# homenc/HElib

Measured on AMD Instinct MI355X. Metric: ctxt_x_ctxt_mults_per_sec_incl_relinearize, higher is better.
Workload: dtype u64; 1 GPU; BGV m=32768 p=65537 bits=950 (L=16x60b, K=6x56b, 6 small primes, D=3): Ctxt::multiplyBy on FRESH ciphertexts = multLowLvl (bringToSet x2 + tensorProduct) + reLinearize (dropSmallAndSpecialPrimes + key switch), benchmarks/bgv_basic.cpp:144-165; added noise MEASURED as in the reference (device canonical-embedding norms, read back lazily); the loop is driven by the C++17 host (libhelib_amd_host.so); ; batch_per_gpu=128, pairs_all_ranks=128

## Files before the change

### helib_amd/csrc/dev_common.h

```cpp
#pragma once
#include <hip/hip_runtime.h>
#include <stdint.h>

#include "ntt_core.h"

namespace hx {

constexpr int MAX_ROWS = 160;

struct PrimeDev {
  uint64_t q;
  uint64_t q2;
  uint64_t mu;
  uint64_t mu64;
  uint32_t k;
  uint32_t proth;
  uint64_t mu63;
  uint64_t tw_fwd_off;
  uint64_t tw_inv_off;
  uint64_t r2;
  uint64_t half_t1, half_t1p, half_t1m;
};

struct RowMap {
  uint16_t p[MAX_ROWS];
};
struct NttRows {
  uint16_t row[MAX_ROWS];
  uint16_t prime[MAX_ROWS];
};

struct ModDownPrep {
  uint64_t* xs;
  int64_t* S;
  uint64_t half;
  uint64_t ptxt;
  uint64_t ptxt_mu64, ptxt_mu, qd_mod_p, qdinv_mod_p;
  uint32_t ptxt_k, has_up;
  TW upS, upN;
  uint64_t qd;
  uint64_t poly_stride;
};
constexpr int MD_MAXDROP = 16;
struct PrepMulti {
  uint16_t row[MD_MAXDROP];
  uint16_t prime[MD_MAXDROP];
  TW up[2 * MD_MAXDROP];
};
struct ModDownRow {
  TW qdm;
  TW inv;
  TW cf;
  uint64_t cf_r2;
  uint32_t out_row;
  uint32_t mode;
};
struct ModDownApply {
  const uint64_t* xs;
  const int64_t* S;
  const ModDownRow* rows;
  const uint64_t* delta;
  uint64_t delta_poly_stride;
};
#if defined(__HIPCC__)
typedef unsigned long long hx_v2u64 __attribute__((ext_vector_type(2)));
__device__ __forceinline__ ulonglong2 ld_stream2(const uint64_t* p)
{
#ifdef HX_NO_NT
  return *reinterpret_cast<const ulonglong2*>(p);
#else
  const hx_v2u64 v = __builtin_nontemporal_load(reinterpret_cast<const hx_v2u64*>(p));
  return make_ulonglong2(v.x, v.y);
#endif
}
__device__ __forceinline__ uint64_t ld_stream1(const uint64_t* p)
{
#if defined(HX_NO_NT) || defined(HX_RNS_NO_NT)
  return *p;
#else
  return __builtin_nontemporal_load(p);
#endif
}
__device__ __forceinline__ void st_stream1(uint64_t* p, uint64_t v)
{
#if defined(HX_NO_NT) || defined(HX_RNS_NO_NT)
  *p = v;
#else
  __builtin_nontemporal_store(v, p);
#endif
}
__device__ __forceinline__ void st_stream2(uint64_t* p, ulonglong2 v)
{
#ifdef HX_NO_NT
  *reinterpret_cast<ulonglong2*>(p) = v;
#else
  hx_v2u64 w;
  w.x = v.x;
  w.y = v.y;
  __builtin_nontemporal_store(w, reinterpret_cast<hx_v2u64*>(p));
#endif
}
#endif

struct TensorSrc {
  const uint64_t* a0;
  const uint64_t* a1;
  const uint64_t* b0;
  const uint64_t* b1;
};
constexpr int MD_MAXPOLY = 8;
struct PolyBases {
  uint64_t* d[MD_MAXPOLY];
  int n;
};
__host__ __device__ inline uint64_t* poly_base(const PolyBases& p, unsigned i)
{
  uint64_t* r = p.d[0];
  r = i == 1 ? p.d[1] : r;
  r = i == 2 ? p.d[2] : r;
  r = i == 3 ? p.d[3] : r;
  r = i == 4 ? p.d[4] : r;
  r = i == 5 ? p.d[5] : r;
  r = i == 6 ? p.d[6] : r;
  r = i == 7 ? p.d[7] : r;
  return r;
}
struct RowMap2 {
  uint16_t p[MAX_ROWS];
  uint16_t brow[MAX_ROWS];
};
struct RowScalars {
  uint64_t c[MAX_ROWS];
  uint64_t cp[MAX_ROWS];
};

constexpr int KS_MAXD = 8;
struct KsFix {
  int64_t owner;
  TW pinv[KS_MAXD];
  TW pscale;
};
struct KsLastPlan {
  uint16_t fd[MAX_ROWS];
};
struct KsLastArgs {
  const uint64_t* dig_in;
  const uint64_t* dig_ev;
  const uint64_t* kb;
  const uint64_t* ka;
  uint64_t* out0;
  uint64_t* out1;
  const uint64_t* own_src;
  const uint64_t* acc0;
  const uint64_t* acc1;
  const KsFix* fix;
  int nall, wrows, batch, scale_parts;
};

typedef unsigned __int128 u128;

#define HX_RO __attribute__((address_space(4)))
typedef const HX_RO uint64_t* ro_u64;
typedef const HX_RO uint32_t* ro_u32;
typedef const HX_RO double* ro_f64;
typedef const HX_RO TW* ro_tw;
template <class T>
__host__ __device__ inline const HX_RO T* as_ro(const T* p)
{
  return (const HX_RO T*)(uintptr_t)p;
}
__device__ __forceinline__ TW ld_tw(ro_tw p, size_t i)
{
  ro_u64 w = (ro_u64)p;
  TW t;
  t.w = w[2 * i];
  t.wp = w[2 * i + 1];
  return t;
}

__device__ __forceinline__ uint64_t add_mod(uint64_t a, uint64_t b, uint64_t q)
{
  uint64_t s = a + b;
  return s >= q ? s - q : s;
}
__device__ __forceinline__ uint64_t sub_mod(uint64_t a, uint64_t b, uint64_t q)
{
  return a >= b ? a - b : a + q - b;
}
__device__ __forceinline__ uint64_t neg_mod(uint64_t a, uint64_t q) { return a ? q - a : 0; }

__device__ __forceinline__ uint64_t mul_mod(uint64_t a, uint64_t b, uint64_t q, uint64_t mu,
                                            uint32_t k)
{
  u128 x = (u128)a * b;
// ... 32 lines not shown
```

### helib_amd/csrc/engine.hip

```cpp
#include <hip/hip_runtime.h>

#include <cstdarg>
#include <cstdio>
#include <cstdlib>
#include <cstring>
#include <algorithm>
#include <chrono>
#include <map>
#include <mutex>
#include <string>
#include <unordered_set>
#include <vector>

#include "../../include/helib_amd.h"
#include "arena.h"
#include "prof.h"
#include "switches.h"
#include "dev_common.h"
#include "hostmath.h"
#include "bluestein.h"
#include "pfa_dev.h"
#include "rns_kernels.h"
#include "mfma_ext.h"
#include "rns_mfma_dev.h"
// ... 29 lines not shown
hipError_t launch_moddown_apply_plain_tensor_pow2(int logn, const TensorSrc& T, const PolyBases& outs, const NttRows& keep,
                                                  int nkeep, int batch, const ModDownApply& A, const PrimeDev* primes,
                                                  const TW* tw_arena, hipStream_t st);
hipError_t launch_moddown_tensor_pow2(int logn, const TensorSrc& T, const PolyBases& outs, int drop_row, int drop_prime,
                                      const NttRows& keep, int nkeep, int batch, const ModDownPrep& P,
                                      const ModDownApply& A, const PrimeDev* primes, const TW* tw_arena, hipStream_t st);
hipError_t launch_ntt_inv_mul_pow2(int logn, const uint64_t* a, const uint64_t* b, uint64_t* out, const NttRows& rows,
                                   int nrows, int batch, const PrimeDev* primes, const TW* tw_arena, hipStream_t st);
hipError_t launch_conv_rows(int logn, const ConvRowArgs& A, const ConvRows& R, int nunits, const PrimeDev* cprimes,
                            const TW* tw_arena, hipStream_t st);
}

using hx::ExtArgs;
using hx::ExtPlanDev;
using hx::MAX_ROWS;
static constexpr int MAX_EXT_SRC = hx::EXT_MAXSRC;
using hx::ModDownApply;
using hx::ModDownPrep;
using hx::NttRows;
using hx::PolyBases;
using hx::PrimeDev;
using hx::RowMap;
using hx::RowMap2;
using hx::RowScalars;
using hx::TW;

static thread_local std::string g_err;
static int fail(int code, const char* fmt, ...)
{
  char buf[512];
  va_list ap;
  va_start(ap, fmt);
  vsnprintf(buf, sizeof buf, fmt, ap);
  va_end(ap);
  g_err = buf;
  return code;
}
#define HIPCHK(expr)                                                                     \
  do {                                                                                   \
    hipError_t _e = (expr);                                                              \
    if (_e != hipSuccess) {                                                              \
      (void)hipGetLastError();  \
      return fail(HX_ERR_DEVICE, "%s failed: %s (%s:%d)", #expr, hipGetErrorString(_e),  \
                  __FILE__, __LINE__);                                                   \
    }                                                                                    \
  } while (0)
#define CHK(expr)          \
  do {                     \
    int _rc = (expr);      \
    if (_rc != HX_OK)      \
      return _rc;          \
  } while (0)

extern "C" const char* hx_last_error(void) { return g_err.c_str(); }
extern "C" const char* hx_version(void) { return "helib_amd 0.1 (gfx950)"; }
extern "C" int hx_device_count(int* count)
{
  if (!count)
    return fail(HX_ERR_INVALID, "null argument");
  int n = 0;
  hipError_t e = hipGetDeviceCount(&n);
  if (e != hipSuccess) {
    *count = 0;
    return fail(HX_ERR_DEVICE, "hipGetDeviceCount: %s", hipGetErrorString(e));
  }
  *count = n;
  return HX_OK;
}

struct PrimeHost {
  uint64_t q, root, rinv;
  uint64_t last_s = 0, last_n = 0;
  uint64_t tw_fwd_off = 0, tw_inv_off = 0;
  bool proth = false;
  int half_pd = -1;
};
static inline uint64_t tw_companion(const PrimeHost& ph, uint64_t w)
{
  return ph.proth ? hx::tw_mont_form(w, ph.q) : hxh::shoup(w, ph.q);
}
static inline uint64_t tw_r2(const PrimeHost& ph, uint64_t w)
{
  return ph.proth ? hx::tw_mont_form(hx::tw_mont_form(w, ph.q), ph.q) : 0;
}

struct ExtPlan {
  ExtPlanDev dev;
  void* blob = nullptr;
  void* blob_mfma = nullptr;
};

struct ConvPlan {
  int logn = 0;
  int split = 0;
  int pd[16] = {0, 0, 0, 0, 0, 0, 0, 0, 0, 0, 0, 0, 0, 0, 0, 0};
  hx::ConvPrimeDev* dev = nullptr;
};
struct BluePrime {
  bool aux = false;
  ConvPlan aconv[3][3];
  uint64_t* d_ahat[3][4] = {{nullptr, nullptr, nullptr, nullptr}, {nullptr, nullptr, nullptr, nullptr},
                            {nullptr, nullptr, nullptr, nullptr}};
  hx::Crt3Dev crt;
  hx::BluePrimeDev* dev = nullptr;
  TW* d_powers = nullptr;
  TW* d_ipowers = nullptr;
  uint64_t* d_hat[5] = {nullptr, nullptr, nullptr, nullptr, nullptr};
  TW* d_hatw[5] = {nullptr, nullptr, nullptr, nullptr, nullptr};
  ConvPlan conv[4];
  uint64_t* d_pfa = nullptr;
};

struct hx_ctx {
  hxs::Switches sw;
  int device = 0;
  hipStream_t stream = nullptr;
  uint64_t m = 0;
  uint32_t phim = 0;
  int logn = 0;
  bool pow2 = false;
  std::vector<uint32_t> zms;
  uint32_t* d_zms = nullptr;
  int32_t* d_zms_index = nullptr;
  uint32_t* d_perm = nullptr;
  std::vector<PrimeHost> primes;
  PrimeDev* d_primes = nullptr;
  int primes_cap = 0;
  TW* d_tw = nullptr;
  size_t tw_cap = 0, tw_used = 0;
  uint64_t* scratch[11] = {nullptr, nullptr, nullptr, nullptr, nullptr, nullptr, nullptr, nullptr, nullptr, nullptr, nullptr};
  uint32_t* d_redo = nullptr;
  size_t redo_cap = 0;
  size_t scratch_words[11] = {0, 0, 0, 0, 0, 0, 0, 0, 0, 0, 0};
  uint64_t aux_q[3] = {0, 0, 0};
  int bk = 0, n1 = 0, n2 = 0, n3 = 0;
  uint32_t dq = 0, mpad = 0;
  PrimeDev* d_cprimes = nullptr;
  int ncprimes = 0, cprimes_cap = 0;
  std::vector<struct BluePrime*> blue;
  uint16_t* d_pfa_idx = nullptr;
  std::vector<ConvPlan> bigplan;
  std::vector<int64_t> psi_low, phi_coef;
  std::map<std::vector<uint64_t>, ExtPlan*> plans;
  hxa::SlabArena arena;
  std::unordered_set<struct hx_poly*> polys;
  int refs = 1;
  std::recursive_mutex mu;
  double* d_frac = nullptr;
  size_t frac_cap = 0, frac_pos = 0;
  bool want_frac = false;
  int xs_first = 0, xs_rows = 0;
  double xs_inv_qd = 0;
  bool want_fdelta = false;
  double2* d_wtab = nullptr;
  double2 *d_bn_v = nullptr, *d_bn_w = nullptr, *d_bn_chat = nullptr, *d_bn_Z = nullptr;
  size_t bn_rows_cap = 0;
  unsigned long long* d_norm2 = nullptr;
  size_t norm_cap = 0;
  double2* d_norm_park = nullptr;
  size_t norm_park_cap = 0;
  struct NormPending {
    hipEvent_t ev;
    unsigned long long* pinned;
    size_t cap;
    int rows;
    double* out;
    bool slab;
  };
  std::vector<void*> norm_slabs;
  bool defer_norms = false;
  std::vector<NormPending> norm_pending, norm_free;
  hipStream_t norm_stream = nullptr;
  hipEvent_t norm_in_ev = nullptr, norm_out_ev = nullptr;
  bool norm_reads_xs = false, norm_reads_frac = false;
  hipEvent_t timer[2] = {nullptr, nullptr};
  bool capturing = false;
  int graphs_alive = 0;
  hipStream_t own_stream = nullptr;
  std::vector<void*> graph_retired;
  void* ckks = nullptr;
  void (*ckks_free)(void*) = nullptr;
  void* linalg = nullptr;
  void (*linalg_free)(void*) = nullptr;
};

struct hx_poly {
  hx_ctx* ctx;
  int batch;
  int cap_rows;
  std::vector<int> prime_idx;
  uint64_t* d;
  bool owns;
  struct Share {
    int refs;
  };
  Share* share = nullptr;
  bool exposed = false;
  size_t row_words() const { return (size_t)batch * ctx->phim; }
  int nrows() const { return (int)prime_idx.size(); }
  bool shared() const { return share && share->refs > 1; }
};

struct hx_ksk {
  hx_ctx* ctx;
  int ndig;
  std::vector<int> row_idx;
  uint64_t* d_b;
  uint64_t* d_a;
};

static int use(hx_ctx* c)
{
  HIPCHK(hipSetDevice(c->device));
  return HX_OK;
}
#define CTX_ENTER(ctx)                                             \
  std::lock_guard<std::recursive_mutex> _ctx_lock((ctx)->mu);      \
  CHK(use(ctx))

#define NO_CAPTURE(ctx, what)                                                                      \
  do {                                                                                             \
    if ((ctx)->capturing)                                                                          \
      return fail(HX_ERR_INVALID, what " waits for the device and cannot be captured in a graph"); \
  } while (0)

static constexpr size_t POOL_LIMIT = (size_t)64 << 30;
template <bool TRACE>
static int arena_sys_alloc_t(size_t bytes, void** out)
{
  const bool trace = TRACE;
  const auto t0 = std::chrono::steady_clock::now();
  hipError_t e = hipMalloc(out, bytes);
  if (trace)
    fprintf(stderr, "[helib_amd arena] hipMalloc(%zu MiB) took %.2f ms\n", bytes >> 20,
            std::chrono::duration<double, std::milli>(std::chrono::steady_clock::now() - t0).count());
  if (e != hipSuccess)
    (void)hipGetLastError();
  return (int)e;
}
static void arena_sys_free(void* p) { hipFree(p); }
static hipError_t pool_alloc(hx_ctx* c, size_t bytes, void** out)
{
  if (!c->arena.sys_alloc) {
    c->arena.sys_alloc = c->sw.arena_trace ? arena_sys_alloc_t<true> : arena_sys_alloc_t<false>;
    c->arena.sys_free = arena_sys_free;
  }
  int rc = c->arena.alloc(bytes, c->capturing, out);
  if (rc != 0 && !c->capturing) {
    (void)hipGetLastError();
    hipStreamSynchronize(c->stream);
    if (c->arena.trim(0) > 0)
      rc = c->arena.alloc(bytes, false, out);
  }
  return (hipError_t)rc;
}
static void retire_or_free(hx_ctx* c, void* p, bool device_wide_sync = false)
{
  if (!p)
    return;
  if (c->norm_stream)
    hipStreamSynchronize(c->norm_stream);
  if (c->capturing || c->graphs_alive > 0) {
    c->graph_retired.push_back(p);
    return;
  }
  if (device_wide_sync)
    hipDeviceSynchronize();
  else
    hipStreamSynchronize(c->stream);
  hipFree(p);
}
static void pool_free(hx_ctx* c, void* p, size_t bytes)
{
  (void)bytes;
  if ((c->capturing || c->graphs_alive > 0) && c->arena.is_pinned(p)) {
    c->arena.defer(p);
    return;
  }
  c->arena.release(p);
  if (c->arena.cached() > POOL_LIMIT && !c->capturing) {
    hipStreamSynchronize(c->stream);
    c->arena.trim(POOL_LIMIT / 2);
  }
}

static int norm_join(hx_ctx* c, bool xs, bool frac)
{
  if ((xs && c->norm_reads_xs) || (frac && c->norm_reads_frac)) {
    HIPCHK(hipStreamWaitEvent(c->stream, c->norm_out_ev, 0));
    c->norm_reads_xs = c->norm_reads_frac = false;
  }
  return HX_OK;
}

static int ensure_scratch(hx_ctx* c, int slot, size_t words)
{
  if (slot <= 1)
    CHK(norm_join(c, true, false));
  if (c->scratch_words[slot] >= words)
    return HX_OK;
  if (c->scratch[slot]) {
    retire_or_free(c, c->scratch[slot]);
    c->scratch[slot] = nullptr;
    c->scratch_words[slot] = 0;
  }
  HIPCHK(hipMalloc((void**)&c->scratch[slot], words * 8));
  c->scratch_words[slot] = words;
  return HX_OK;
}

static int dcopy(hx_ctx* c, uint64_t* dst, const uint64_t* src, size_t words)
{
  if (words == 0 || dst == src)
    return HX_OK;
  if (((uintptr_t)dst | (uintptr_t)src) & 15) {
    HIPCHK(hipMemcpyAsync(dst, src, words * 8, hipMemcpyDeviceToDevice, c->stream));
    return HX_OK;
  }
  const size_t blocks = std::min<size_t>((words / 2 + 255) / 256, (size_t)256 * 16);
  HX_LAUNCH(hx::copy_words_kernel, dim3((unsigned)std::max<size_t>(blocks, 1)), dim3(256), 0, c->stream,
                     dst, src, words);
  HIPCHK(hipGetLastError());
  return HX_OK;
}
// ... 10 lines not shown
    }
    p->share = nullptr;
  } else {
    pool_free(p->ctx, p->d, bytes);
  }
  p->d = nullptr;
}
static int poly_own(hx_poly* p)
{
  if (!p->share)
    return HX_OK;
  if (p->share->refs == 1) {
    delete p->share;
    p->share = nullptr;
    return HX_OK;
  }
  hx_ctx* c = p->ctx;
  uint64_t* nd = nullptr;
  const size_t bytes = (size_t)p->cap_rows * p->row_words() * 8;
  hipError_t e = pool_alloc(c, bytes, (void**)&nd);
  if (e != hipSuccess)
    return fail(HX_ERR_NOMEM, "hipMalloc(%zu) failed: %s", bytes, hipGetErrorString(e));
  CHK(dcopy(c, nd, p->d, (size_t)p->nrows() * p->row_words()));
  p->share->refs--;
  p->share = nullptr;
  p->d = nd;
  return HX_OK;
}
#define OWN(p) CHK(poly_own(p))
static int poly_fresh(hx_poly* p, const uint64_t** old_rows)
{
  *old_rows = p->d;
  if (!p->share)
    return HX_OK;
  if (p->share->refs == 1) {
    delete p->share;
    p->share = nullptr;
    return HX_OK;
  }
  uint64_t* nd = nullptr;
  const size_t bytes = (size_t)p->cap_rows * p->row_words() * 8;
  hipError_t e = pool_alloc(p->ctx, bytes, (void**)&nd);
  if (e != hipSuccess)
    return fail(HX_ERR_NOMEM, "hipMalloc(%zu) failed: %s", bytes, hipGetErrorString(e));
  p->share->refs--;
  p->share = nullptr;
  p->d = nd;
  return HX_OK;
}

static void ctx_free(hx_ctx* c);
extern "C" int hx_ctx_create(hx_ctx** out, int device, uint64_t m)
{
  if (!out || m < 2 || m > (1ull << 24))
    return fail(HX_ERR_INVALID, "Bad Z_m^* modulus m (must be in [2, 2^24])");
  int ndev = 0;
  if (hipGetDeviceCount(&ndev) != hipSuccess || ndev <= 0)
    return fail(HX_ERR_DEVICE, "no HIP device available (this library has no CPU path)");
  if (device < 0 || device >= ndev)
    return fail(HX_ERR_INVALID, "device %d out of range [0,%d)", device, ndev);
  HIPCHK(hipSetDevice(device));
  hx_ctx* c = new hx_ctx();
  c->sw = hxs::read();
  struct Guard {
    hx_ctx* c;
    ~Guard()
    {
      if (c)
        ctx_free(c);
    }
  } guard{c};
  c->device = device;
  c->m = m;
  std::vector<int32_t> zidx((size_t)m, -1);
  for (uint64_t i = 1; i < m; i++)
    if (hxh::gcd(i, m) == 1) {
      zidx[i] = (int32_t)c->zms.size();
      c->zms.push_back((uint32_t)i);
    }
  c->phim = (uint32_t)c->zms.size();
  c->pow2 = (m & (m - 1)) == 0;
  if (c->pow2) {
    int l = 0;
    while ((1u << l) < c->phim)
      l++;
    c->logn = l;
  }
  HIPCHK(hipMalloc((void**)&c->d_zms, (size_t)c->phim * 4));
  HIPCHK(hipMalloc((void**)&c->d_zms_index, (size_t)m * 4));
  HIPCHK(hipMalloc((void**)&c->d_perm, (size_t)c->phim * 4));
  HIPCHK(hipMemcpy(c->d_zms, c->zms.data(), (size_t)c->phim * 4, hipMemcpyHostToDevice));
  HIPCHK(hipMemcpy(c->d_zms_index, zidx.data(), (size_t)m * 4, hipMemcpyHostToDevice));
  c->primes_cap = 1024;
  HIPCHK(hipMalloc((void**)&c->d_primes, sizeof(PrimeDev) * c->primes_cap));
  guard.c = nullptr;
  *out = c;
  return HX_OK;
}

static void ctx_release(hx_ctx* c)
{
  bool last;
  {
    std::lock_guard<std::recursive_mutex> lk(c->mu);
    last = --c->refs == 0;
  }
  if (last)
    ctx_free(c);
}
extern "C" int hx_ctx_destroy(hx_ctx* c)
{
  if (!c)
    return HX_OK;
  ctx_release(c);
  return HX_OK;
}
static void ctx_free(hx_ctx* c)
{
  hipSetDevice(c->device);
  hipDeviceSynchronize();
  if (c->ckks_free)
    c->ckks_free(c->ckks);
  if (c->linalg_free)
    c->linalg_free(c->linalg);
  if (c->d_tw)
    hipFree(c->d_tw);
  for (auto& kv : c->plans) {
    hipFree(kv.second->blob);
    hipFree(kv.second->blob_mfma);
    delete kv.second;
  }
  for (int i = 0; i < 11; i++)
    if (c->scratch[i])
      hipFree(c->scratch[i]);
  c->arena.destroy();
  if (c->norm_stream) {
    hipStreamDestroy(c->norm_stream);
    hipEventDestroy(c->norm_in_ev);
    hipEventDestroy(c->norm_out_ev);
  }
  if (c->own_stream)
    hipStreamDestroy(c->own_stream);
  for (void* q : c->graph_retired)
    hipFree(q);
  hipFree(c->d_redo);
  hipFree(c->d_frac);
  hipFree(c->d_wtab);
  hipFree(c->d_bn_v);
  hipFree(c->d_bn_w);
  hipFree(c->d_bn_chat);
  hipFree(c->d_bn_Z);
  hipFree(c->d_norm2);
  hipFree(c->d_norm_park);
  for (auto* v : {&c->norm_pending, &c->norm_free})
    for (auto& np : *v) {
      hipEventDestroy(np.ev);
      if (!np.slab)
        hipHostFree(np.pinned);
    }
  for (void* q : c->norm_slabs)
    hipHostFree(q);
  for (BluePrime* b : c->blue) {
    if (!b)
      continue;
    hipFree(b->dev);
    hipFree(b->d_powers);
    hipFree(b->d_ipowers);
    hipFree(b->d_pfa);
    for (int i = 0; i < 5; i++) {
      hipFree(b->d_hat[i]);
      hipFree(b->d_hatw[i]);
    }
    for (int i = 0; i < 4; i++)
      hipFree(b->conv[i].dev);
    for (int j = 0; j < 3; j++) {
      for (int i = 0; i < 4; i++)
        hipFree(b->d_ahat[j][i]);
      for (int i = 0; i < 3; i++)
        hipFree(b->aconv[j][i].dev);
    }
    delete b;
  }
  if (c->d_cprimes)
    hipFree(c->d_cprimes);
  for (hipEvent_t e : c->timer)
    if (e)
      hipEventDestroy(e);
  hipFree(c->d_pfa_idx);
  hipFree(c->d_zms);
  hipFree(c->d_zms_index);
  hipFree(c->d_perm);
  hipFree(c->d_primes);
  delete c;
}

extern "C" int hx_ctx_phim(const hx_ctx* c, uint64_t* phim)
{
  if (!c || !phim)
    return fail(HX_ERR_INVALID, "null argument");
  *phim = c->phim;
  return HX_OK;
}
extern "C" int hx_ctx_set_stream(hx_ctx* c, void* s)
{
  if (!c)
    return fail(HX_ERR_INVALID, "null context");
  std::lock_guard<std::recursive_mutex> lk(c->mu);
  if (c->capturing)
    return fail(HX_ERR_INVALID, "hx_ctx_set_stream while a graph is being captured");
  if (c->stream != (hipStream_t)s) {
    hipSetDevice(c->device);
    hipStreamSynchronize(c->stream);
    if (c->norm_stream)
      hipStreamSynchronize(c->norm_stream);
  }
  c->stream = (hipStream_t)s;
  return HX_OK;
}
extern "C" int hx_ctx_sync(hx_ctx* c)
{
  if (!c)
    return fail(HX_ERR_INVALID, "null context");
  CTX_ENTER(c);
  NO_CAPTURE(c, "hx_ctx_sync");
  HIPCHK(hipStreamSynchronize(c->stream));
  if (c->norm_stream)
    HIPCHK(hipStreamSynchronize(c->norm_stream));
  return HX_OK;
}
extern "C" int hx_ctx_reserve(hx_ctx* c, uint64_t bytes)
{
  if (!c)
    return fail(HX_ERR_INVALID, "null context");
  CTX_ENTER(c);
  if (!c->arena.sys_alloc) {
    c->arena.sys_alloc = c->sw.arena_trace ? arena_sys_alloc_t<true> : arena_sys_alloc_t<false>;
    c->arena.sys_free = arena_sys_free;
  }
  const int rc = c->arena.reserve((size_t)bytes);
  if (rc != 0)
    return fail(HX_ERR_NOMEM, "hipMalloc(%llu) failed: %s", (unsigned long long)bytes, hipGetErrorString((hipError_t)rc));
  return HX_OK;
}
extern "C" int hx_ctx_arena_stats(hx_ctx* c, uint64_t out[4])
{
  if (!c || !out)
    return fail(HX_ERR_INVALID, "null argument");
  std::lock_guard<std::recursive_mutex> lk(c->mu);
  out[0] = c->arena.reserved;
  out[1] = c->arena.in_use;
  out[2] = c->arena.sys_calls;
  out[3] = c->arena.deferred.size();
  return HX_OK;
}
extern "C" int hx_ctx_num_primes(const hx_ctx* c, int* n)
{
  if (!c || !n)
    return fail(HX_ERR_INVALID, "null argument");
  *n = (int)c->primes.size();
  return HX_OK;
}
extern "C" int hx_ctx_prime(const hx_ctx* c, int idx, uint64_t* q, uint64_t* root)
{
  if (!c)
    return fail(HX_ERR_INVALID, "prime index out of range");
  std::lock_guard<std::recursive_mutex> lk(const_cast<hx_ctx*>(c)->mu);
  if (idx < 0 || idx >= (int)c->primes.size())
    return fail(HX_ERR_INVALID, "prime index out of range");
  if (q)
    *q = c->primes[idx].q;
  if (root)
    *root = c->primes[idx].root;
  return HX_OK;
}

static int tw_reserve(hx_ctx* c, size_t extra)
{
  if (c->tw_used + extra <= c->tw_cap)
    return HX_OK;
  size_t ncap = c->tw_cap ? c->tw_cap * 2 : extra * 32;
  while (ncap < c->tw_used + extra)
    ncap *= 2;
  TW* nd = nullptr;
  HIPCHK(hipMalloc((void**)&nd, ncap * sizeof(TW)));
  if (c->d_tw) {
    HIPCHK(hipDeviceSynchronize());
    HIPCHK(hipMemcpy(nd, c->d_tw, c->tw_used * sizeof(TW), hipMemcpyDeviceToDevice));
    retire_or_free(c, c->d_tw, true);
  }
  c->d_tw = nd;
  c->tw_cap = ncap;
  return HX_OK;
}

template <int LOGN>
static int upload_tw(hx_ctx* c, PrimeHost& ph)
{
  using G = hx::Geo<LOGN>;
  std::vector<TW> f(G::TW_TOTAL), i(G::TW_TOTAL);
  uint64_t ninv = hxh::invmod((uint64_t)G::N % ph.q, ph.q);
  hx::build_tw_tables<LOGN>(ph.q, ph.root, ph.rinv, ninv, hxh::mulmod, f.data(), i.data());
  CHK(tw_reserve(c, 2 * (size_t)G::TW_TOTAL));
  ph.tw_fwd_off = c->tw_used;
  ph.tw_inv_off = c->tw_used + G::TW_TOTAL;
  ph.proth = hx::is_proth32(ph.q) && !c->sw.no_proth;
  if (ph.proth) {
// ... 1890 lines not shown
    pl->dev.mfma_a = nullptr;
    pl->dev.mfma_steps = 0;
    const bool oks = mfma_small && pl->dev.hps_ok;
    if ((okw || oks) && !c->sw.no_mfma_ext) {
      std::vector<uint8_t> tab;
      std::vector<uint64_t> tqs((size_t)nt);
      for (int t = 0; t < nt; t++)
        tqs[(size_t)t] = tq(t);
      hx::mfx::build_tables(n, nt, tqs.data(), mfma_w.data(), mfma_negp.data(), &h[o_upd], tab);
      uint8_t* dm = nullptr;
      HIPCHK(hipMalloc((void**)&dm, tab.size()));
      HIPCHK(hipMemcpy(dm, tab.data(), tab.size(), hipMemcpyHostToDevice));
      pl->blob_mfma = dm;
      pl->dev.mfma_a = dm;
      pl->dev.mfma_steps = (uint32_t)hx::mfx::steps_for(n);
    }
  }
  pl->dev.tgt_chunk7 = hx::as_ro(reinterpret_cast<const uint32_t*>(d + o_tchunk));
  {
    bool unit = scaled && ptxt > 1;
    for (int t = 0; t < nt && unit; t++)
      unit = ptxt <= tq(t);
    pl->dev.corr_unit = unit ? 1u : 0u;
  }
  c->plans[key] = pl;
  *out = pl;
  return HX_OK;
}

static int redo_prepare(hx_ctx* c, size_t row_words, uint32_t** out)
{
  const size_t need = row_words + 1;
  if (c->redo_cap < need) {
    uint32_t* nd = nullptr;
    HIPCHK(hipMalloc((void**)&nd, need * sizeof(uint32_t)));
    retire_or_free(c, c->d_redo);
    c->d_redo = nd;
    c->redo_cap = need;
  }
  HIPCHK(hipMemsetAsync(c->d_redo, 0, sizeof(uint32_t), c->stream));
  *out = c->d_redo;
  return HX_OK;
}
static int hps_min_n(const hx_ctx* c)
{
  return c->sw.hps_min_n;
}
static const dim3 REDO_GRID(64);

static int launch_extend(hx_ctx* c, const ExtPlan* pl, const ExtArgs& args_in, size_t row_words)
{
  dim3 grid((unsigned)((row_words + 255) / 256)), block(256);
  int n = pl->dev.n;
  ExtArgs args = args_in;
  args.redo = nullptr;
  if (pl->dev.fast16_ok) {
    const bool mfma = pl->dev.hps_ok && pl->dev.mfma_steps != 0 && args.upd == nullptr && row_words < ((size_t)1 << 32);
    const bool hps = mfma || (pl->dev.hps_ok && n >= hps_min_n(c) && args.upd == nullptr && row_words < ((size_t)1 << 32));
    if (hps)
      CHK(redo_prepare(c, row_words, &args.redo));
    if (mfma)
      HIPCHK(hx::launch_rns_extend_mfma(pl->dev, args, row_words, c->stream));
#define HX_EXT_FAST(NN)                                                                                            \
  case NN:                                                                                                         \
    if (hps) {                                                                                                     \
      if (!mfma)                                                                                                   \
        HX_LAUNCH((hx::rns_extend_fast_kernel<NN, true>), grid, block, 0, c->stream, pl->dev, args, row_words);    \
      HX_LAUNCH((hx::rns_extend_fast_kernel<NN, false>), REDO_GRID, block, 0, c->stream, pl->dev, args, row_words); \
    } else {                                                                                                       \
      HX_LAUNCH((hx::rns_extend_fast_kernel<NN, false>), grid, block, 0, c->stream, pl->dev, args, row_words);     \
    }                                                                                                              \
    break;
    switch (n) {
      HX_EXT_FAST(1) HX_EXT_FAST(2) HX_EXT_FAST(3) HX_EXT_FAST(4) HX_EXT_FAST(5) HX_EXT_FAST(6) HX_EXT_FAST(7) HX_EXT_FAST(8)
      HX_EXT_FAST(9) HX_EXT_FAST(10) HX_EXT_FAST(11) HX_EXT_FAST(12) HX_EXT_FAST(13) HX_EXT_FAST(14) HX_EXT_FAST(15)
      HX_EXT_FAST(16)
    }
#undef HX_EXT_FAST
    HIPCHK(hipGetLastError());
    return HX_OK;
  }
  const size_t wide_lds = (size_t)pl->dev.nt * (size_t)hx::wide_stride(n) * 8;
  if (pl->dev.wide_ok && row_words < ((size_t)1 << 32) && wide_lds <= 160 * 1024) {
    CHK(redo_prepare(c, row_words, &args.redo));
    if (pl->dev.mfma_steps) {
      HIPCHK(hx::launch_rns_extend_mfma(pl->dev, args, row_words, c->stream));
      HX_LAUNCH((hx::rns_extend_kernel<40>), REDO_GRID, block, 0, c->stream, pl->dev, args, row_words);
      HIPCHK(hipGetLastError());
      return HX_OK;
    }
    const dim3 wgrid((unsigned)((row_words + hx::WIDE_THREADS - 1) / hx::WIDE_THREADS)), wblock(hx::WIDE_THREADS);
    const size_t lds = wide_lds;
    static std::mutex wide_mu;
    static std::unordered_set<int> wide_attr;
    {
      std::lock_guard<std::mutex> lk(wide_mu);
      if (!wide_attr.count(c->device)) {
        for (const void* f : {(const void*)hx::rns_extend_wide_kernel<20>, (const void*)hx::rns_extend_wide_kernel<24>,
                              (const void*)hx::rns_extend_wide_kernel<28>, (const void*)hx::rns_extend_wide_kernel<32>,
                              (const void*)hx::rns_extend_wide_kernel<36>, (const void*)hx::rns_extend_wide_kernel<40>})
          HIPCHK(hxp::dyn_lds(f, 160 * 1024));
        wide_attr.insert(c->device);
      }
    }
    if (n <= 20)
      HX_LAUNCH((hx::rns_extend_wide_kernel<20>), wgrid, wblock, lds, c->stream, pl->dev, args, row_words);
    else if (n <= 24)
      HX_LAUNCH((hx::rns_extend_wide_kernel<24>), wgrid, wblock, lds, c->stream, pl->dev, args, row_words);
    else if (n <= 28)
      HX_LAUNCH((hx::rns_extend_wide_kernel<28>), wgrid, wblock, lds, c->stream, pl->dev, args, row_words);
    else if (n <= 32)
      HX_LAUNCH((hx::rns_extend_wide_kernel<32>), wgrid, wblock, lds, c->stream, pl->dev, args, row_words);
    else if (n <= 36)
      HX_LAUNCH((hx::rns_extend_wide_kernel<36>), wgrid, wblock, lds, c->stream, pl->dev, args, row_words);
    else
      HX_LAUNCH((hx::rns_extend_wide_kernel<40>), wgrid, wblock, lds, c->stream, pl->dev, args, row_words);
    HX_LAUNCH((hx::rns_extend_kernel<40>), REDO_GRID, block, 0, c->stream, pl->dev, args, row_words);
    HIPCHK(hipGetLastError());
    return HX_OK;
  }
  if (n <= 8)
    HX_LAUNCH((hx::rns_extend_kernel<8>), grid, block, 0, c->stream, pl->dev, args,
                       row_words);
  else if (n <= 16)
    HX_LAUNCH((hx::rns_extend_kernel<16>), grid, block, 0, c->stream, pl->dev, args,
                       row_words);
  else if (n <= 40)
    HX_LAUNCH((hx::rns_extend_kernel<40>), grid, block, 0, c->stream, pl->dev, args,
                       row_words);
  else if (n <= 64)
    HX_LAUNCH((hx::rns_extend_kernel<64>), grid, block, 0, c->stream, pl->dev, args,
                       row_words);
  else
    HX_LAUNCH((hx::rns_extend_kernel<MAX_EXT_SRC>), grid, block, 0, c->stream, pl->dev, args,
                       row_words);
  HIPCHK(hipGetLastError());
  return HX_OK;
}

static void clear_args(ExtArgs& a)
{
  memset(&a, 0xff, sizeof a);
  a.src = nullptr;
  a.dst = nullptr;
  a.upd = nullptr;
  a.nu = 0;
  a.frac = nullptr;
  a.redo = nullptr;
  a.lazy_out = 0;
}

static int bn_logp(const hx_ctx* c) { return next_pow2_exp(2 * c->m - 1); }

static int frac_begin(hx_ctx* c, size_t doubles)
{
  if (!c->pow2 && bn_logp(c) > 18)
    return fail(HX_ERR_UNSUPPORTED,
                "device embedding norms need m a power of two or m <= 131072 (otherwise the host keeps "
                "the reference's noiseBoundForUniform bound)");
  if (c->frac_cap < doubles) {
    CHK(norm_join(c, false, true));
    retire_or_free(c, c->d_frac);
    c->d_frac = nullptr;
    c->frac_cap = 0;
    HIPCHK(hipMalloc((void**)&c->d_frac, doubles * sizeof(double)));
    c->frac_cap = doubles;
  }
  CHK(norm_join(c, false, true));
  c->frac_pos = 0;
  c->want_frac = true;
  c->xs_rows = 0;
  return HX_OK;
}
static double* frac_take(hx_ctx* c, size_t doubles)
{
  if (!c->want_frac || c->frac_pos + doubles > c->frac_cap)
    return nullptr;
  double* p = c->d_frac + c->frac_pos;
  c->frac_pos += doubles;
  return p;
}

static int flush_xs(hx_ctx* c)
{
  if (c->xs_rows <= 0)
    return HX_OK;
  const size_t n = (size_t)c->xs_rows * c->phim;
  HX_LAUNCH(hx::frac_from_xs_kernel, dim3((unsigned)std::min<size_t>((n + 255) / 256, 4096)),
                     dim3(256), 0, c->stream, c->scratch[0],
                     reinterpret_cast<const int64_t*>(c->scratch[1]), c->xs_inv_qd,
                     c->d_frac + (size_t)c->xs_first * c->phim, n);
  HIPCHK(hipGetLastError());
  c->xs_rows = 0;
  return HX_OK;
}

static int bnorm_setup(hx_ctx* c)
{
  if (c->d_bn_chat)
    return HX_OK;
  const int bk = bn_logp(c);
  if (bk > 18)
    return fail(HX_ERR_UNSUPPORTED, "device embedding norms: m too large (2m-1 > 2^18)");
  const uint64_t m = c->m;
  const size_t P = (size_t)1 << bk;
  const long double pi = 3.141592653589793238462643383279502884L;
  std::vector<double> v(2 * m), cv(2 * P, 0.0), w(P);
  for (uint64_t k = 0; k < m; k++) {
    const uint64_t k2 = (uint64_t)(((hxh::u128)k * k) % (2 * m));
    const long double ang = pi * (long double)k2 / (long double)m;
    const double cr = (double)cosl(ang), si = (double)sinl(ang);
    v[2 * k] = cr;
    v[2 * k + 1] = si;
    cv[2 * k] = cr;
    cv[2 * k + 1] = -si;
    if (k) {
      cv[2 * (P - k)] = cr;
      cv[2 * (P - k) + 1] = -si;
    }
  }
  for (size_t k = 0; k < P / 2; k++) {
    const long double ang = 2 * pi * (long double)k / (long double)P;
    w[2 * k] = (double)cosl(ang);
    w[2 * k + 1] = (double)sinl(ang);
  }
  double2* d_cv = nullptr;
  HIPCHK(hipMalloc((void**)&c->d_bn_v, sizeof(double) * 2 * m));
  HIPCHK(hipMalloc((void**)&c->d_bn_w, sizeof(double) * P));
  HIPCHK(hipMalloc((void**)&c->d_bn_chat, sizeof(double) * 2 * P));
  HIPCHK(hipMalloc((void**)&d_cv, sizeof(double) * 2 * P));
  HIPCHK(hipMemcpy(c->d_bn_v, v.data(), sizeof(double) * 2 * m, hipMemcpyHostToDevice));
  HIPCHK(hipMemcpy(c->d_bn_w, w.data(), sizeof(double) * P, hipMemcpyHostToDevice));
  HIPCHK(hipMemcpy(d_cv, cv.data(), sizeof(double) * 2 * P, hipMemcpyHostToDevice));
  bool attr = false;
  if (!attr) {
    HIPCHK(hxp::dyn_lds((const void*)hx::bnorm_fwd_kernel, 16 << hx::NORM_MAX_LOGH));
    HIPCHK(hxp::dyn_lds((const void*)hx::bnorm_inv_kernel, 16 << hx::NORM_MAX_LOGH));
    attr = true;
  }
  const int logp = bk, logh = std::min(logp, hx::NORM_MAX_LOGH);
  const unsigned H = 1u << logh, S = (unsigned)(P >> logh);
  const unsigned threads = std::min<unsigned>(hx::NORM_THREADS, std::max<unsigned>(64u, H / 4));
  HX_LAUNCH(hx::bnorm_fwd_kernel, dim3(S), dim3(threads), std::max<size_t>(16 * (size_t)H, 256), c->stream,
                     (const double*)nullptr, (const double2*)nullptr, (const double2*)d_cv, c->d_bn_w,
                     (const double2*)nullptr, c->d_bn_chat, logp, logh, c->phim, 1);
  HIPCHK(hipGetLastError());
  HIPCHK(hipStreamSynchronize(c->stream));
  HIPCHK(hipFree(d_cv));
  return HX_OK;
}

static int embed_norms_general(hx_ctx* c, const double* d_f, int rows, hipStream_t ns)
{
  CHK(bnorm_setup(c));
  const int logp = bn_logp(c), logh = std::min(logp, hx::NORM_MAX_LOGH);
  const size_t P = (size_t)1 << logp;
  const unsigned H = 1u << logh, S = (unsigned)(P >> logh);
  const size_t cap = std::max<size_t>(1, ((size_t)1 << 28) / (16 * P));
  if (c->bn_rows_cap < std::min<size_t>(cap, (size_t)rows)) {
    retire_or_free(c, c->d_bn_Z);
    c->d_bn_Z = nullptr;
    c->bn_rows_cap = std::min<size_t>(cap, (size_t)rows);
    HIPCHK(hipMalloc((void**)&c->d_bn_Z, c->bn_rows_cap * P * 16));
  }
  const unsigned threads = std::min<unsigned>(hx::NORM_THREADS, std::max<unsigned>(64u, H / 4));
  const size_t lds = std::max<size_t>(16 * (size_t)H, 256);
  for (size_t r0 = 0; r0 < (size_t)rows; r0 += c->bn_rows_cap) {
    const unsigned nr = (unsigned)std::min<size_t>(c->bn_rows_cap, (size_t)rows - r0);
    HX_LAUNCH(hx::bnorm_fwd_kernel, dim3(nr * S), dim3(threads), lds, ns,
                       d_f + r0 * c->phim, (const double2*)c->d_bn_v, (const double2*)nullptr, c->d_bn_w,
                       (const double2*)c->d_bn_chat, c->d_bn_Z, logp, logh, c->phim, 0);
    HIPCHK(hipGetLastError());
    HX_LAUNCH(hx::bnorm_inv_kernel, dim3(nr * S), dim3(threads), lds, ns, c->d_bn_Z, c->d_bn_w,
                       logp, logh);
    HIPCHK(hipGetLastError());
    const unsigned gx = std::min<unsigned>(64u, (c->phim + 255u) / 256u);
    HX_LAUNCH(hx::bnorm_max_kernel, dim3(gx, nr), dim3(256), 0, ns, (const double2*)c->d_bn_Z,
                       c->d_bn_w, c->d_zms, c->phim, logp, logh, c->d_norm2 + r0);
    HIPCHK(hipGetLastError());
  }
  return HX_OK;
}

static int embed_norms(hx_ctx* c, const double* d_f, int rows, double* out_host)
{
  const uint32_t N = c->phim;
  const int logn = c->logn;
  if (c->pow2 && !c->d_wtab) {
    std::vector<double> h(2 * (size_t)N);
    const long double two_pi = 6.283185307179586476925286766559005768394L;
    for (uint32_t k = 0; k < N; k++) {
      long double ang = two_pi * (long double)k / (long double)c->m;
      h[2 * (size_t)k] = (double)cosl(ang);
      h[2 * (size_t)k + 1] = (double)sinl(ang);
    }
    HIPCHK(hipMalloc((void**)&c->d_wtab, sizeof(double) * 2 * (size_t)N));
    HIPCHK(hipMemcpy(c->d_wtab, h.data(), sizeof(double) * 2 * (size_t)N, hipMemcpyHostToDevice));
  }
  if (c->norm_cap < (size_t)rows) {
    retire_or_free(c, c->d_norm2);
    c->d_norm2 = nullptr;
    c->norm_cap = 0;
    HIPCHK(hipMalloc((void**)&c->d_norm2, sizeof(unsigned long long) * (size_t)rows));
    c->norm_cap = (size_t)rows;
  }
  const bool quarter_form = c->pow2 && logn >= 2 && logn - 1 <= hx::NORM_MAX_LOGH;
  const bool use_xs = quarter_form && c->xs_rows == rows && d_f == c->d_frac;
  if (!use_xs)
    CHK(flush_xs(c));
  hipStream_t ns = c->stream;
  const bool side_stream = c->sw.norm_async;
  if (side_stream && !c->capturing) {
    if (!c->norm_stream) {
      HIPCHK(hipStreamCreateWithFlags(&c->norm_stream, hipStreamNonBlocking));
      HIPCHK(hipEventCreateWithFlags(&c->norm_in_ev, hipEventDisableTiming));
      HIPCHK(hipEventCreateWithFlags(&c->norm_out_ev, hipEventDisableTiming));
    }
    HIPCHK(hipEventRecord(c->norm_in_ev, c->stream));
    HIPCHK(hipStreamWaitEvent(c->norm_stream, c->norm_in_ev, 0));
    ns = c->norm_stream;
  }
  hx_ctx::NormPending np{};
  bool have = false;
  for (size_t i = 0; i < c->norm_free.size(); i++)
    if (c->norm_free[i].cap >= (size_t)rows) {
      np = c->norm_free[i];
      c->norm_free.erase(c->norm_free.begin() + (long)i);
      have = true;
      break;
    }
  if (!have && rows <= 1024) {
    constexpr size_t PER = 64, CAP = 1024;
    unsigned long long* slab = nullptr;
    HIPCHK(hipHostMalloc((void**)&slab, PER * CAP * sizeof(unsigned long long), hipHostMallocDefault));
    c->norm_slabs.push_back(slab);
    for (size_t i = 0; i < PER; i++) {
      hx_ctx::NormPending f{};
      f.pinned = slab + i * CAP;
      f.cap = CAP;
      f.slab = true;
      HIPCHK(hipEventCreateWithFlags(&f.ev, hipEventDisableTiming));
      c->norm_free.push_back(f);
    }
    np = c->norm_free.back();
    c->norm_free.pop_back();
    have = true;
  }
  if (!have) {
    np.cap = (size_t)rows;
    np.slab = false;
    HIPCHK(hipHostMalloc((void**)&np.pinned, np.cap * sizeof(unsigned long long), hipHostMallocDefault));
    HIPCHK(hipEventCreateWithFlags(&np.ev, hipEventDisableTiming));
  }
  struct SlotGuard {
    hx_ctx* c;
    hx_ctx::NormPending* np;
    bool armed = true;
    ~SlotGuard()
    {
      if (armed)
        c->norm_free.push_back(*np);
    }
  } slot_guard{c, &np};
  const bool by_copy = c->sw.norm_memcpy;
  const bool r16_path = c->pow2 && !c->sw.norm_old && logn == 14;
  const bool x2_path = c->pow2 && logn == 15 && !c->sw.norm_old && !c->sw.norm_plain;
  const bool direct = !by_copy && (r16_path || x2_path);
  unsigned long long* const out2 = direct ? np.pinned : c->d_norm2;
  if (!direct)
    HIPCHK(hipMemsetAsync(c->d_norm2, 0, sizeof(unsigned long long) * (size_t)rows, ns));
  bool attr = false;
  if (!c->pow2) {
    CHK(flush_xs(c));
    CHK(embed_norms_general(c, d_f, rows, ns));
  } else if (!attr) {
    HIPCHK(hxp::dyn_lds((const void*)hx::embed_norm_kernel, 16 << hx::NORM_MAX_LOGH));
#define HX_NORM_ATTR(...)                                                                               \
  HIPCHK(hxp::dyn_lds((const void*)hx::embed_norm_quarter_kernel<__VA_ARGS__>,                   \
                             hipFuncAttributeMaxDynamicSharedMemorySize, 16 << hx::NORM_MAX_LOGH))
    HX_NORM_ATTR(hx::NormSrcF64, 0);
    HX_NORM_ATTR(hx::NormSrcF64, 13);
    HX_NORM_ATTR(hx::NormSrcF64, 14);
    HX_NORM_ATTR(hx::NormSrcXS, 0);
    HX_NORM_ATTR(hx::NormSrcXS, 13);
    HX_NORM_ATTR(hx::NormSrcXS, 14);
#undef HX_NORM_ATTR
    HIPCHK(hxp::dyn_lds((const void*)hx::embed_norm_quarter_split_kernel, 16 << hx::NORM_MAX_LOGH));
    attr = true;
  }
  if (!c->pow2) {
  } else if (logn >= 2 && logn - 1 <= hx::NORM_MAX_LOGH) {
    const unsigned M = N >> 1;
    const unsigned threads = std::min<unsigned>(hx::NORM_THREADS, std::max<unsigned>(64u, M / 4));
    const size_t lds = std::max<size_t>(16 * (size_t)M, 256);
    const bool full = threads == (unsigned)hx::NORM_THREADS;
#define HX_NORM_LAUNCH(SRCT, srcv)                                                                              \
  do {                                                                                                          \
    if (full && logn == 14)                                                                                     \
      HX_LAUNCH((hx::embed_norm_quarter_kernel<SRCT, 14>), dim3((unsigned)rows), dim3(threads), lds,   \
                         ns, srcv, c->d_wtab, logn, c->d_norm2);                                         \
    else if (full && logn == 13)                                                                                \
      HX_LAUNCH((hx::embed_norm_quarter_kernel<SRCT, 13>), dim3((unsigned)rows), dim3(threads), lds,   \
                         ns, srcv, c->d_wtab, logn, c->d_norm2);                                         \
    else                                                                                                        \
      HX_LAUNCH((hx::embed_norm_quarter_kernel<SRCT, 0>), dim3((unsigned)rows), dim3(threads), lds,    \
                         ns, srcv, c->d_wtab, logn, c->d_norm2);                                         \
  } while (0)
    const bool r16 = !c->sw.norm_old;
    constexpr size_t r16_lds = (size_t)hx::R16_LDS_DOUBLES * sizeof(double);
    if (r16 && logn == 14) {
      bool attr16 = false;
      if (!attr16) {
        HIPCHK(hxp::dyn_lds((const void*)hx::embed_norm_r16_kernel<hx::NormSrcXS>, (int)r16_lds));
        HIPCHK(hxp::dyn_lds((const void*)hx::embed_norm_r16_kernel<hx::NormSrcF64>, (int)r16_lds));
        attr16 = true;
      }
    }
    if (c->xs_rows == rows && d_f == c->d_frac) {
      hx::NormSrcXS src{c->scratch[0], reinterpret_cast<const int64_t*>(c->scratch[1]), c->xs_inv_qd};
      if (r16 && logn == 14)
        HX_LAUNCH((hx::embed_norm_r16_kernel<hx::NormSrcXS>), dim3((unsigned)rows), dim3(hx::R16_THREADS), r16_lds, ns, src,
                  c->d_wtab, out2, direct);
      else
        HX_NORM_LAUNCH(hx::NormSrcXS, src);
    } else {
      CHK(flush_xs(c));
      hx::NormSrcF64 src{d_f};
      if (r16 && logn == 14)
        HX_LAUNCH((hx::embed_norm_r16_kernel<hx::NormSrcF64>), dim3((unsigned)rows), dim3(hx::R16_THREADS), r16_lds, ns, src,
                  c->d_wtab, out2, direct);
      else
        HX_NORM_LAUNCH(hx::NormSrcF64, src);
    }
#undef HX_NORM_LAUNCH
    c->xs_rows = 0;
  } else if (logn - 1 > hx::NORM_MAX_LOGH && !c->sw.norm_plain) {
    CHK(flush_xs(c));
    const int logh = hx::NORM_MAX_LOGH;
    const unsigned H = 1u << logh, S = (N >> 1) >> logh;
    const size_t park_words = (size_t)rows * (S / 2) * H;
    const bool x2 = logn == 15 && !c->sw.norm_old;
    if (!x2 && c->norm_park_cap < park_words) {
      retire_or_free(c, c->d_norm_park);
      c->d_norm_park = nullptr;
      c->norm_park_cap = 0;
      HIPCHK(hipMalloc((void**)&c->d_norm_park, park_words * sizeof(double2)));
      c->norm_park_cap = park_words;
    }
    if (x2) {
      constexpr size_t x2_lds = 2 * (size_t)hx::R16_LDS_DOUBLES * sizeof(double);
      bool attrx2 = false;
      if (!attrx2) {
        HIPCHK(hxp::dyn_lds((const void*)hx::embed_norm_r16x2_kernel, (int)x2_lds));
        attrx2 = true;
      }
      HX_LAUNCH(hx::embed_norm_r16x2_kernel, dim3((unsigned)rows), dim3(2 * hx::R16_THREADS), x2_lds, ns, d_f, c->d_wtab,
                out2, direct);
    } else
    HX_LAUNCH(hx::embed_norm_quarter_split_kernel, dim3((unsigned)rows * (S / 2)), dim3(hx::NORM_THREADS),
                       16 * (size_t)H, ns, d_f, c->d_wtab, logn, logh, c->d_norm_park, c->d_norm2);
  } else {
    CHK(flush_xs(c));
    const int logh = std::min(logn, hx::NORM_MAX_LOGH);
    const unsigned H = 1u << logh, S = N >> logh;
    const unsigned threads = std::min<unsigned>(hx::NORM_THREADS, std::max<unsigned>(64u, H / 4));
    const size_t lds = std::max<size_t>(16 * (size_t)H, 256);
    HX_LAUNCH(hx::embed_norm_kernel, dim3((unsigned)rows * S), dim3(threads), lds, ns, d_f,
                       c->d_wtab, logn, logh, c->d_norm2);
  }
  HIPCHK(hipGetLastError());
  np.rows = rows;
  np.out = out_host;
  if (direct) {
  } else if (by_copy) {
    HIPCHK(hipMemcpyAsync(np.pinned, c->d_norm2, sizeof(unsigned long long) * (size_t)rows,
                          hipMemcpyDeviceToHost, ns));
  } else {
    HX_LAUNCH(hx::copy_words_kernel, dim3((unsigned)((rows + 255) / 256)), dim3(256), 0, ns,
              reinterpret_cast<uint64_t*>(np.pinned), reinterpret_cast<const uint64_t*>(c->d_norm2), (size_t)rows);
    HIPCHK(hipGetLastError());
  }
  HIPCHK(hipEventRecord(np.ev, ns));
  c->norm_pending.push_back(np);
  slot_guard.armed = false;
  if (ns != c->stream) {
    HIPCHK(hipEventRecord(c->norm_out_ev, ns));
    (use_xs ? c->norm_reads_xs : c->norm_reads_frac) = true;
  }
  if (c->defer_norms)
    return HX_OK;
  return hx_norms_flush(c);
}

static hipError_t wait_event(const hx_ctx* c, hipEvent_t ev)
{
  const auto t0 = std::chrono::steady_clock::now();
  for (;;) {
    for (int i = 0; i < 64; i++) {
      const hipError_t e = hipEventQuery(ev);
      if (e != hipErrorNotReady)
        return e;
    }
    if (std::chrono::steady_clock::now() - t0 > std::chrono::microseconds(c->sw.wait_poll_us))
      break;
  }
  return hipEventSynchronize(ev);
}

extern "C" int hx_norms_flush(hx_ctx* c)
{
  if (!c)
    return fail(HX_ERR_INVALID, "null context");
  CTX_ENTER(c);
  NO_CAPTURE(c, "hx_norms_flush");
  for (auto& np : c->norm_pending) {
    HIPCHK(wait_event(c, np.ev));
    for (int r = 0; r < np.rows; r++) {
      double v;
      memcpy(&v, &np.pinned[r], 8);
      np.out[r] = sqrt(v);
    }
    c->norm_free.push_back(np);
  }
  c->norm_pending.clear();
  return HX_OK;
}

extern "C" int hx_ctx_defer_norms(hx_ctx* c, int on)
{
  if (!c)
    return fail(HX_ERR_INVALID, "null context");
  c->defer_norms = on != 0;
  if (!on)
    return hx_norms_flush(c);
  return HX_OK;
}

extern "C" int hx_embedding_norm(hx_ctx* c, const double* f_host, int rows, double* norms_out)
{
  if (!c || !f_host || !norms_out || rows < 1)
    return fail(HX_ERR_INVALID, "bad argument");
  CTX_ENTER(c);
  NO_CAPTURE(c, "hx_embedding_norm");
  const size_t n = (size_t)rows * c->phim;
  CHK(frac_begin(c, n));
  c->want_frac = false;
  HIPCHK(hipMemcpyAsync(c->d_frac, f_host, n * sizeof(double), hipMemcpyHostToDevice, c->stream));
  CHK(embed_norms(c, c->d_frac, rows, norms_out));
  return hx_norms_flush(c);
}

static int scale_rows_by_primes(hx_poly* a, const int* add_idx, int nadd)
{
  hx_ctx* c = a->ctx;
  std::vector<uint64_t> f(a->nrows());
  for (int r = 0; r < a->nrows(); r++) {
    uint64_t q = c->primes[a->prime_idx[r]].q, v = 1;
    for (int i = 0; i < nadd; i++)
      v = hxh::mulmod(v, c->primes[add_idx[i]].q % q, q);
    f[r] = v;
  }
  return ew_scalar_rows<hx::EWS_MUL>(a, f.data());
}

extern "C" int hx_add_primes_and_scale(hx_poly* a, const int* add_idx, int nadd)
{
  if (!a)
    return fail(HX_ERR_INVALID, "null poly");
  if (nadd == 0)
    return HX_OK;
  hx_ctx* c = a->ctx;
  CTX_ENTER(c);
  CHK(check_rows(c, add_idx, nadd));
  for (int i = 0; i < nadd; i++)
    if (find_row(a->prime_idx, add_idx[i]) >= 0)
      return fail(HX_ERR_PRIMESET, "addPrimes can only be called on a disjoint set");
  int old = a->nrows();
  OWN(a);
  if (old > 0)
    CHK(scale_rows_by_primes(a, add_idx, nadd));
  CHK(poly_reserve(a, old + nadd));
  HIPCHK(hipMemsetAsync(a->d + (size_t)old * a->row_words(), 0,
                        (size_t)nadd * a->row_words() * 8, c->stream));
  for (int i = 0; i < nadd; i++)
    a->prime_idx.push_back(add_idx[i]);
  return HX_OK;
// ... 284 lines not shown
    ~PrimeRollback()
    {
      if (n > 0)
        a->prime_idx.resize(a->prime_idx.size() - (size_t)n);
    }
  } rollback{a};
  if (nadd > 0 && ndrop != 1) {
    std::vector<int> drop, keep;
    for (int r = 0; r < a->nrows(); r++) {
      bool d = false;
      for (int i = 0; i < ndrop; i++)
        d = d || drop_idx[i] == a->prime_idx[r];
      (d ? drop : keep).push_back(a->prime_idx[r]);
    }
    for (int i = 0; i < nadd; i++) {
      if (find_row(a->prime_idx, add_idx[i]) >= 0)
        return HX_ERR_UNSUPPORTED;
      for (int j = 0; j < ndrop; j++)
        if (drop_idx[j] == add_idx[i])
          return HX_ERR_UNSUPPORTED;
      keep.push_back(add_idx[i]);
    }
    if (drop.size() < 2 || (int)keep.size() == nadd)
      return HX_ERR_UNSUPPORTED;
    hx_poly* ps[hx::MD_MAXPOLY];
    if (1 + nother > hx::MD_MAXPOLY)
      return HX_ERR_UNSUPPORTED;
    ps[0] = a;
    for (int i = 0; i < nother; i++)
      ps[1 + i] = others[i];
    return scale_down_multi_fused(ps, 1 + nother, drop, keep, ptxt, add_idx, nadd, tsrc);
  }
  if (nadd > 0) {
    bool ok = ndrop == 1 && c->pow2 && c->logn >= 13 && c->logn <= 15 && find_row(a->prime_idx, drop_idx[0]) >= 0 &&
              a->nrows() + nadd - 1 <= MAX_ROWS && ptxt < ((uint64_t)1 << 62);
    for (int i = 0; i < nadd && ok; i++)
      if (find_row(a->prime_idx, add_idx[i]) >= 0 || add_idx[i] == drop_idx[0])
        ok = false;
    for (int i = 0; i < nadd && ok; i++)
      ok = ptxt / 2 + 2 < c->primes[add_idx[i]].q;
    for (int r = 0; r < a->nrows() && ok; r++)
      ok = a->prime_idx[r] == drop_idx[0] || ptxt / 2 + 2 < c->primes[a->prime_idx[r]].q;
    if (!ok)
      return HX_ERR_UNSUPPORTED;
    if (!a->shared())
      CHK(poly_reserve(a, a->nrows() + nadd));
    for (int i = 0; i < nother; i++)
      if (!others[i]->shared())
        CHK(poly_reserve(others[i], a->nrows() + nadd));
    for (int i = 0; i < nadd; i++)
      a->prime_idx.push_back(add_idx[i]);
    rollback.n = nadd;
  }
  const int nrows_old = a->nrows() - nadd;
  std::vector<int> drop, keep;
  for (int r = 0; r < a->nrows(); r++) {
    bool d = false;
    for (int i = 0; i < ndrop; i++)
      if (drop_idx[i] == a->prime_idx[r])
        d = true;
    (d ? drop : keep).push_back(a->prime_idx[r]);
  }
  if (drop.empty()) {
    if (tsrc)
      return HX_ERR_UNSUPPORTED;
    if (c->want_frac) {
      double* fr = frac_take(c, a->row_words() * (size_t)(1 + nother));
      if (fr)
        HIPCHK(hipMemsetAsync(fr, 0, a->row_words() * (size_t)(1 + nother) * sizeof(double), c->stream));
    }
    return HX_OK;
  }
  if (keep.empty())
    return fail(HX_ERR_PRIMESET, "s and the index set must have some intersection");
  if ((int)drop.size() > MAX_EXT_SRC)
    return fail(HX_ERR_UNSUPPORTED, "scaleDownToSet dropping more than %d primes", MAX_EXT_SRC);
  size_t rw = a->row_words();
  int nd = (int)drop.size(), nk = (int)keep.size();
  bool small_S = true;
  for (int pr : keep)
    small_S = small_S && ptxt / 2 + 2 < c->primes[pr].q;
  if (tsrc && nd >= 2) {
    hx_poly* ps[hx::MD_MAXPOLY];
    if (1 + nother > hx::MD_MAXPOLY)
      return HX_ERR_UNSUPPORTED;
    ps[0] = a;
    for (int i = 0; i < nother; i++)
      ps[1 + i] = others[i];
    return scale_down_multi_fused(ps, 1 + nother, drop, keep, ptxt, nullptr, 0, tsrc);
  }
  if (tsrc && !(nd == 1 && nk <= MAX_ROWS && small_S))
    return HX_ERR_UNSUPPORTED;
  if (nd == 1 && c->pow2 && c->logn >= 13 && c->logn <= 15 && nk <= MAX_ROWS && ptxt < ((uint64_t)1 << 62) && small_S) {
    const int dprime = drop[0], drow = find_row(a->prime_idx, dprime), last = a->nrows() - 1;
    const uint64_t qd = c->primes[dprime].q;
    PolyBases pb, pbo;
    memset(&pb, 0, sizeof pb);
    memset(&pbo, 0, sizeof pbo);
    pb.n = pbo.n = 1 + nother;
    hx_poly* ps[hx::MD_MAXPOLY];
    uint64_t* fresh[hx::MD_MAXPOLY] = {nullptr};
    ps[0] = a;
    for (int i = 0; i < nother; i++)
      ps[1 + i] = others[i];
    const int ncap = a->nrows() + 2;
    const size_t nbytes = (size_t)ncap * rw * 8;
    for (int i = 0; i < pb.n; i++)
      if (ps[i]->share && !ps[i]->shared())
        CHK(poly_own(ps[i]));
    auto drop_fresh = [&]() {
      for (int i = 0; i < pb.n; i++)
        if (fresh[i])
          pool_free(c, fresh[i], nbytes);
    };
    for (int i = 0; i < pb.n; i++) {
      pb.d[i] = pbo.d[i] = ps[i]->d;
      if (ps[i]->shared()) {
        hipError_t pe = pool_alloc(c, nbytes, (void**)&fresh[i]);
        if (pe != hipSuccess) {
          drop_fresh();
          return fail(HX_ERR_NOMEM, "hipMalloc(%zu) failed: %s", nbytes, hipGetErrorString(pe));
        }
        pbo.d[i] = fresh[i];
      }
    }
    struct FreshGuard {
      decltype(drop_fresh)& f;
      bool armed = true;
      ~FreshGuard()
      {
        if (armed)
          f();
      }
    } fresh_guard{drop_fresh};
    CHK(ensure_scratch(c, 0, rw * pb.n));
    CHK(ensure_scratch(c, 1, rw * pb.n));
    hx::ModDownPrep P;
    memset(&P, 0, sizeof P);
    P.xs = c->scratch[0];
    P.S = reinterpret_cast<int64_t*>(c->scratch[1]);
    P.half = (qd - 1) / 2;
    if (ptxt > 1) {
      P.ptxt = ptxt;
      P.ptxt_mu64 = (uint64_t)((((hxh::u128)1) << 64) / ptxt);
      int kb = hxh::bitlen(ptxt);
      P.ptxt_k = (uint32_t)kb;
      P.ptxt_mu = (uint64_t)((((hxh::u128)1) << (2 * kb)) / ptxt);
      P.qd_mod_p = qd % ptxt;
      P.qdinv_mod_p = hxh::invmod(qd % ptxt, ptxt);
      if (P.qdinv_mod_p == 0)
        return fail(HX_ERR_INVALID, "dropped primes are not invertible modulo ptxtSpace");
    }
    P.qd = qd;
    if (nadd > 0) {
      uint64_t F = 1;
      for (int i = 0; i < nadd; i++)
        F = hxh::mulmod(F, c->primes[add_idx[i]].q % qd, qd);
      P.has_up = 1;
      P.upS.w = hxh::mulmod(F, c->primes[dprime].last_s, qd);
      P.upS.wp = tw_companion(c->primes[dprime], P.upS.w);
      P.upN.w = hxh::mulmod(F, c->primes[dprime].last_n, qd);
      P.upN.wp = tw_companion(c->primes[dprime], P.upN.w);
    }
    std::vector<uint64_t> key;
    key.push_back(0xD0D0D0D0ull);
    key.push_back((uint64_t)dprime);
    for (int j = 0; j < nadd; j++)
      key.push_back(0xA000000ull | (uint64_t)add_idx[j]);
    NttRows kr;
    std::vector<hx::ModDownRow> hr(nk);
    int i = 0;
    for (int r = 0; r <= last; r++) {
      if (r == drow)
        continue;
      const int pr = a->prime_idx[r];
      const uint64_t q = c->primes[pr].q;
      kr.row[i] = (uint16_t)r;
      kr.prime[i] = (uint16_t)pr;
      uint64_t qdm = qd % q, inv = hxh::invmod(qdm, q);
      hr[i].qdm.w = qdm;
      hr[i].qdm.wp = hxh::shoup(qdm, q);
      hr[i].inv.w = inv;
      hr[i].inv.wp = tw_companion(c->primes[pr], inv);
      hr[i].out_row = (uint32_t)((r == last && drow != last) ? drow : r);
      hr[i].mode = 0;
      hr[i].cf = hr[i].inv;
      hr[i].cf_r2 = tw_r2(c->primes[pr], inv);
      if (nadd > 0) {
        if (r >= nrows_old) {
          hr[i].mode = 2;
          hr[i].cf.w = hr[i].cf.wp = 0;
          hr[i].cf_r2 = 0;
        } else {
          uint64_t F = 1;
          for (int j = 0; j < nadd; j++)
            F = hxh::mulmod(F, c->primes[add_idx[j]].q % q, q);
          uint64_t cf = hxh::mulmod(F, inv, q);
          hr[i].mode = 1;
          hr[i].cf.w = cf;
          hr[i].cf.wp = tw_companion(c->primes[pr], cf);
          hr[i].cf_r2 = tw_r2(c->primes[pr], cf);
        }
      }
      key.push_back(((uint64_t)pr << 28) | ((uint64_t)hr[i].out_row << 12) | hr[i].mode);
      i++;
    }
    auto it = c->plans.find(key);
    if (it == c->plans.end()) {
      ExtPlan* pl = new ExtPlan();
      memset(&pl->dev, 0, sizeof pl->dev);
      HIPCHK(hipMalloc(&pl->blob, sizeof(hx::ModDownRow) * nk));
      HIPCHK(hipMemcpy(pl->blob, hr.data(), sizeof(hx::ModDownRow) * nk, hipMemcpyHostToDevice));
      it = c->plans.emplace(key, pl).first;
    }
    hx::ModDownApply A;
    A.xs = c->scratch[0];
    A.S = reinterpret_cast<const int64_t*>(c->scratch[1]);
    A.rows = reinterpret_cast<const hx::ModDownRow*>(it->second->blob);
    hipError_t e = tsrc ? hx::launch_moddown_tensor_pow2(c->logn, *tsrc, pbo, drow, dprime, kr, nk, a->batch, P, A,
                                                         c->d_primes, c->d_tw, c->stream)
                        : hx::launch_moddown_pow2(c->logn, pb, pbo, drow, dprime, kr, nk, a->batch, P, A,
                                                  c->d_primes, c->d_tw, c->stream);
    if (e != hipSuccess)
      return fail(HX_ERR_DEVICE, "mod-down launch failed: %s", hipGetErrorString(e));
    fresh_guard.armed = false;
    for (int i = 0; i < pb.n; i++)
      if (fresh[i]) {
        storage_release(ps[i]);
        ps[i]->d = fresh[i];
        ps[i]->cap_rows = ncap;
      }
    if (c->want_frac) {
      const size_t n = rw * (size_t)pb.n;
      double* fr = frac_take(c, n);
      if (!fr)
        return fail(HX_ERR_INVALID, "internal: fraction buffer too small");
      if (c->xs_rows == 0 && c->frac_pos == n && !c->want_fdelta) {
        c->xs_first = 0;
        c->xs_rows = pb.n * a->batch;
        c->xs_inv_qd = 1.0 / (double)qd;
      } else {
        HX_LAUNCH(hx::frac_from_xs_kernel, dim3((unsigned)std::min<size_t>((n + 255) / 256, 4096)),
                           dim3(256), 0, c->stream, c->scratch[0],
                           reinterpret_cast<const int64_t*>(c->scratch[1]), 1.0 / (double)qd, fr, n);
        HIPCHK(hipGetLastError());
      }
    }
    rollback.n = 0;
    if (drow != last)
      a->prime_idx[drow] = a->prime_idx[last];
    a->prime_idx.pop_back();
    for (int i = 0; i < nother; i++)
      others[i]->prime_idx = a->prime_idx;
    return HX_OK;
  }
  if (nd >= 2 && 1 + nother <= hx::MD_MAXPOLY) {
    hx_poly* ps[hx::MD_MAXPOLY];
    ps[0] = a;
    for (int i = 0; i < nother; i++)
      ps[1 + i] = others[i];
    int rc = scale_down_multi_fused(ps, 1 + nother, drop, keep, ptxt, nullptr, 0);
    if (rc != HX_ERR_UNSUPPORTED)
      return rc;
  }
  if (nother > 0)
    return HX_ERR_UNSUPPORTED;
  CHK(ensure_scratch(c, 0, (size_t)a->nrows() * rw));
  std::vector<std::pair<int, int>> drows;
  for (int k = 0; k < nd; k++)
    drows.emplace_back(find_row(a->prime_idx, drop[k]), drop[k]);
  CHK(ntt_list(c, a->d, c->scratch[0], drows, a->batch, true));
  ExtPlan* pl;
  CHK(get_plan(c, drop, keep, ptxt > 1 ? ptxt : 0, &pl));
  uint64_t* nd_buf = nullptr;
  const int ncap = nk + 2;
  const size_t nbytes = (size_t)ncap * rw * 8;
  hipError_t pe = pool_alloc(c, nbytes, (void**)&nd_buf);
  if (pe != hipSuccess)
    return fail(HX_ERR_NOMEM, "hipMalloc(%zu) failed: %s", nbytes, hipGetErrorString(pe));
  ExtArgs args;
  clear_args(args);
  args.src = c->scratch[0];
  args.dst = nd_buf;
  for (int k = 0; k < nd; k++)
    args.src_row[k] = (uint16_t)drows[k].first;
  for (int t = 0; t < nk; t++)
    args.dst_row[t] = (uint16_t)t;
  int rc = HX_OK;
  if (c->want_frac) {
    args.frac = frac_take(c, rw);
    if (!args.frac)
      rc = fail(HX_ERR_INVALID, "internal: fraction buffer too small");
  }
  if (rc == HX_OK)
    rc = launch_extend(c, pl, args, rw);
  if (rc == HX_OK)
    rc = ntt_rows(c, nd_buf, keep, nk, 0, nk, a->batch, false);
  if (rc != HX_OK) {
    pool_free(c, nd_buf, nbytes);
    return rc;
  }
  RowMap2 map;
  RowScalars sc;
  for (int r = 0; r < nk; r++) {
    uint64_t q = c->primes[keep[r]].q, v = 1;
    for (int k = 0; k < nd; k++)
      v = hxh::mulmod(v, c->primes[drop[k]].q % q, q);
    uint64_t inv = hxh::invmod(v, q);
    map.p[r] = (uint16_t)keep[r];
    map.brow[r] = (uint16_t)find_row(a->prime_idx, keep[r]);
    sc.c[r] = inv;
    sc.cp[r] = hxh::shoup(inv, q);
  }
  HX_LAUNCH(hx::sub_scale_from_kernel, ew_grid(rw, nk), dim3(256), 0, c->stream, nd_buf,
                     a->d, map, sc, rw, c->d_primes);
  HIPCHK(hipGetLastError());
  if (a->owns) {
    storage_release(a);
    a->d = nd_buf;
    a->cap_rows = ncap;
  } else {
    CHK(dcopy(c, a->d, nd_buf, (size_t)nk * rw));
    pool_free(c, nd_buf, nbytes);
  }
  a->prime_idx = keep;
  return HX_OK;
}

extern "C" int hx_scale_down(hx_poly* a, const int* drop_idx, int ndrop, uint64_t ptxt)
{
  return scale_down_impl(a, nullptr, 0, drop_idx, ndrop, ptxt);
}

extern "C" int hx_scale_down_multi(hx_poly** polys, int npoly, const int* drop_idx, int ndrop,
                                   uint64_t ptxt)
{
  if (!polys || npoly < 1)
    return fail(HX_ERR_INVALID, "bad argument");
  bool same = npoly <= hx::MD_MAXPOLY;
  for (int i = 0; i < npoly; i++) {
    if (!polys[i])
      return fail(HX_ERR_INVALID, "null poly");
    if (polys[i]->ctx != polys[0]->ctx || polys[i]->batch != polys[0]->batch ||
        polys[i]->prime_idx != polys[0]->prime_idx)
      same = false;
    for (int j = 0; j < i; j++)
      if (polys[j] == polys[i])
        return fail(HX_ERR_INVALID, "the same poly listed twice");
  }
  if (same && npoly > 1) {
    int rc = scale_down_impl(polys[0], polys + 1, npoly - 1, drop_idx, ndrop, ptxt);
    if (rc != HX_ERR_UNSUPPORTED)
      return rc;
  }
  for (int i = 0; i < npoly; i++)
    CHK(scale_down_impl(polys[i], nullptr, 0, drop_idx, ndrop, ptxt));
  return HX_OK;
}

extern "C" int hx_bring_to_set_multi(hx_poly** polys, int npoly, const int* add_idx, int nadd,
                                     const int* drop_idx, int ndrop, uint64_t ptxt)
{
  if (!polys || npoly < 1 || (nadd > 0 && !add_idx) || (ndrop > 0 && !drop_idx))
    return fail(HX_ERR_INVALID, "bad argument");
  bool same = npoly <= hx::MD_MAXPOLY;
  for (int i = 0; i < npoly; i++) {
    if (!polys[i])
      return fail(HX_ERR_INVALID, "null poly");
    if (polys[i]->ctx != polys[0]->ctx || polys[i]->batch != polys[0]->batch ||
        polys[i]->prime_idx != polys[0]->prime_idx)
      same = false;
    for (int j = 0; j < i; j++)
      if (polys[j] == polys[i])
        return fail(HX_ERR_INVALID, "the same poly listed twice");
  }
  CHK(check_rows(polys[0]->ctx, add_idx, nadd));
  if (same && nadd > 0 && ndrop >= 1) {
// ... 970 lines not shown
```

### helib_amd/csrc/norm_kernels.h

```cpp
#pragma once
#include <hip/hip_runtime.h>
#include <stdint.h>

#include "fft_lds.h"
#include "norm_r16.h"

namespace hx {

__device__ __forceinline__ void block_max_to(double mx, double* sm, unsigned tid, unsigned nth,
                                             unsigned long long* dst, bool direct = false)
{
  for (int off = 32; off > 0; off >>= 1) {
    const double o = __shfl_down(mx, off, 64);
    mx = o > mx ? o : mx;
  }
  __syncthreads();
  if ((tid & 63u) == 0)
    sm[tid >> 6] = mx;
  __syncthreads();
  if (tid == 0) {
    const unsigned nw = (nth + 63) >> 6;
    for (unsigned w = 1; w < nw; w++)
      mx = sm[w] > mx ? sm[w] : mx;
    if (direct)
      *dst = (unsigned long long)__double_as_longlong(mx);
    else
      atomicMax(dst, (unsigned long long)__double_as_longlong(mx));
  }
}

__global__ void __launch_bounds__(NORM_THREADS)
embed_norm_kernel(const double* __restrict__ f, const double2* __restrict__ wtab, int logn, int logh,
                  unsigned long long* __restrict__ out2)
{
  extern __shared__ __attribute__((aligned(16))) double sm[];
  const unsigned N = 1u << logn, H = 1u << logh, S = N >> logh;
  double* re = sm;
  double* im = sm + H;
  const unsigned row = blockIdx.x / S, s = blockIdx.x % S;
  const unsigned tid = threadIdx.x, nth = blockDim.x;
  const double* fr = f + (size_t)row * N;
  const unsigned mmask = 2 * N - 1;
  for (unsigned i = tid; i < H; i += nth) {
    double ar = 0, ai = 0;
    for (unsigned t = 0; t < S; t++) {
      const unsigned idx = i + t * H;
      const unsigned e = (idx * (2 * s + 1)) & mmask;
      double2 w = wtab[e & (N - 1)];
      const double x = e >= N ? -fr[idx] : fr[idx];
      ar += x * w.x;
      ai += x * w.y;
    }
    re[i] = ar;
    im[i] = ai;
  }
  __syncthreads();
  dif_fft_lds(re, im, logh, N, wtab, tid, nth);
  double mx = 0;
  for (unsigned i = tid; i < H; i += nth) {
    const double n2 = re[i] * re[i] + im[i] * im[i];
    mx = n2 > mx ? n2 : mx;
  }
  block_max_to(mx, sm, tid, nth, out2 + row);
}

struct NormSrcF64 {
  const double* f;
  __device__ __forceinline__ double2 pair(unsigned row, unsigned N, unsigned i) const
  {
    return reinterpret_cast<const double2*>(f + (size_t)row * N)[i];
  }
};
struct NormSrcXS {
  const uint64_t* xs;
  const int64_t* S;
  double inv_qd;
  __device__ __forceinline__ double2 pair(unsigned row, unsigned N, unsigned i) const
  {
    const ulonglong2 x = reinterpret_cast<const ulonglong2*>(xs + (size_t)row * N)[i];
    const longlong2 s = reinterpret_cast<const longlong2*>(S + (size_t)row * N)[i];
    return make_double2((double)x.x * inv_qd - (double)s.x, (double)x.y * inv_qd - (double)s.y);
  }
};

template <class SRC, int CLOGN = 0>
__global__ void __launch_bounds__(NORM_THREADS)
embed_norm_quarter_kernel(SRC src, const double2* __restrict__ wtab, int logn_rt,
                          unsigned long long* __restrict__ out2)
{
  extern __shared__ __attribute__((aligned(16))) double sm[];
  const int logn = CLOGN ? CLOGN : logn_rt;
  const unsigned N = 1u << logn, M = N >> 1;
  const int logm = logn - 1;
  double* re = sm;
  double* im = sm + M;
  const unsigned row = blockIdx.x, tid = threadIdx.x, nth = CLOGN ? (unsigned)NORM_THREADS : blockDim.x;
#pragma unroll
  for (unsigned i = tid; i < M; i += nth) {
    const double2 v = src.pair(row, N, i);
    const double2 w = wtab[2 * i];
    re[i] = v.x * w.x - v.y * w.y;
    im[i] = v.x * w.y + v.y * w.x;
  }
  __syncthreads();
  dif_fft_lds<(CLOGN ? CLOGN - 1 : 0), (CLOGN ? NORM_THREADS : 0)>(re, im, logm, N, wtab, tid, nth);
  double mx = 0;
#pragma unroll
  for (unsigned p = tid; p < M; p += nth) {
    const unsigned j = __brev(p) >> (32 - logm);
    const double zr = re[p], zi = im[p], cr = re[M - 1 - p], ci = -im[M - 1 - p];
    const double er = 0.5 * (zr + cr), ei = 0.5 * (zi + ci);
    const double dr = zr - cr, di = zi - ci;
    const double orr = 0.5 * di, oi = -0.5 * dr;
    const double2 w = wtab[2 * j + 1];
    const double tr = orr * w.x - oi * w.y, ti = orr * w.y + oi * w.x;
    const double a = (er + tr) * (er + tr) + (ei + ti) * (ei + ti);
    const double b = (er - tr) * (er - tr) + (ei - ti) * (ei - ti);
    const double n2 = a > b ? a : b;
    mx = n2 > mx ? n2 : mx;
  }
  block_max_to(mx, sm, tid, nth, out2 + row);
}

__device__ __forceinline__ double lane_xor1(double v)
{
  int lo = __double2loint(v), hi = __double2hiint(v);
  lo = __builtin_amdgcn_mov_dpp(lo, 0xB1, 0xF, 0xF, true);
  hi = __builtin_amdgcn_mov_dpp(hi, 0xB1, 0xF, 0xF, true);
  return __hiloint2double(hi, lo);
}
template <unsigned (*FROM)(unsigned, unsigned), unsigned (*TO)(unsigned, unsigned)>
__device__ __forceinline__ void r16_transpose(cplx16 (&v)[16], double* sm, unsigned t)
{
#pragma unroll
  for (unsigned k = 0; k < 16; k++)
    sm[r16_pad(FROM(t, k))] = v[k].x;
  __syncthreads();
#pragma unroll
  for (unsigned k = 0; k < 16; k++)
    v[k].x = sm[r16_pad(TO(t, k))];
  __syncthreads();
#pragma unroll
  for (unsigned k = 0; k < 16; k++)
    sm[r16_pad(FROM(t, k))] = v[k].y;
  __syncthreads();
#pragma unroll
  for (unsigned k = 0; k < 16; k++)
    v[k].y = sm[r16_pad(TO(t, k))];
}
template <class SRC>
__global__ void __launch_bounds__(R16_THREADS)
embed_norm_r16_kernel(SRC src, const double2* __restrict__ wtab, unsigned long long* __restrict__ out2, bool direct)
{
  extern __shared__ __attribute__((aligned(16))) double sm[];
  const unsigned row = blockIdx.x, t = threadIdx.x;
  const tw16* wt = reinterpret_cast<const tw16*>(wtab);
  cplx16 v[16];
#pragma unroll
  for (unsigned k = 0; k < 16; k++) {
    const unsigned i = r16_pos_A(t, k);
    const double2 p = src.pair(row, R16_N, i);
    const tw16 w = k == 0 ? wt[2 * t] : r16_cmul(wt[2 * t], wt[1024u * k]);
    v[k].x = p.x * w.x - p.y * w.y;
    v[k].y = p.x * w.y + p.y * w.x;
  }
  r16_pass<9>(v, t, wt);
  r16_transpose<r16_pos_A, r16_pos_B>(v, sm, t);
  r16_pass<5>(v, t & 31u, wt);
  __syncthreads();
  r16_transpose<r16_pos_B, r16_pos_C>(v, sm, t);
  r16_pass<1>(v, t & 1u, wt);
#pragma unroll
  for (unsigned k = 0; k < 16; k++)
    v[k] = r16_last_lane(v[k], cplx16{lane_xor1(v[k].x), lane_xor1(v[k].y)}, t);
  __syncthreads();
#pragma unroll
  for (unsigned kk = 0; kk < 8; kk++) {
    sm[r16_xchg_idx(t, kk)] = v[8 + kk].x;
    sm[R16_XCHG_IM + r16_xchg_idx(t, kk)] = v[8 + kk].y;
  }
  __syncthreads();
  double mx = 0;
  const tw16 wth = wt[r16_pair_tw_thread(t)];
#pragma unroll
  for (unsigned k = 0; k < 8; k++) {
    const unsigned o = r16_xchg_idx(R16_THREADS - 1u - t, 7u - k);
    const cplx16 partner{sm[o], sm[R16_XCHG_IM + o]};
    const tw16 w = k == 0 ? wth : r16_cmul(wth, wt[r16_pair_tw_k(k)]);
    const double n2 = r16_pair_norm2(v[k], partner, w);
    mx = n2 > mx ? n2 : mx;
  }
  block_max_to(mx, sm, t, R16_THREADS, out2 + row, direct);
}

__global__ void __launch_bounds__(2 * R16_THREADS)
embed_norm_r16x2_kernel(const double* __restrict__ f, const double2* __restrict__ wtab, unsigned long long* __restrict__ out2,
                        bool direct)
{
  extern __shared__ __attribute__((aligned(16))) double sm[];
  const unsigned row = blockIdx.x, h = threadIdx.x >> 9, t = threadIdx.x & 511u;
  double* mine = sm + h * R16_LDS_DOUBLES;
  const double* theirs = sm + (1u - h) * R16_LDS_DOUBLES;
  const tw16* wt = reinterpret_cast<const tw16*>(wtab);
  const double* fr = f + (size_t)row * (1u << 15);
  cplx16 v[16];
#pragma unroll
  for (unsigned k = 0; k < 16; k++)
    v[k] = r16_split_input(fr, wt, r16_pos_A(t, k), h);
  r16_pass<9, 15>(v, t, wt);
  r16_transpose<r16_pos_A, r16_pos_B>(v, mine, t);
  r16_pass<5, 15>(v, t & 31u, wt);
  __syncthreads();
  r16_transpose<r16_pos_B, r16_pos_C>(v, mine, t);
  r16_pass<1, 15>(v, t & 1u, wt);
#pragma unroll
  for (unsigned k = 0; k < 16; k++)
    v[k] = r16_last_lane(v[k], cplx16{lane_xor1(v[k].x), lane_xor1(v[k].y)}, t);
  __syncthreads();
#pragma unroll
  for (unsigned kk = 0; kk < 8; kk++) {
    mine[r16_xchg_idx(t, kk)] = v[8 + kk].x;
    mine[R16_XCHG_IM + r16_xchg_idx(t, kk)] = v[8 + kk].y;
  }
  __syncthreads();
  double mx = 0;
  const tw16 wth = wt[r16x2_pair_tw_thread(h, t)];
#pragma unroll
  for (unsigned k = 0; k < 8; k++) {
    const unsigned o = r16_xchg_idx(R16_THREADS - 1u - t, 7u - k);
    const cplx16 other{theirs[o], theirs[R16_XCHG_IM + o]};
    const double n2 = r16x2_pair(h, v[k], other, wth, wt[r16x2_pair_tw_k(k)], k);
    mx = n2 > mx ? n2 : mx;
  }
  block_max_to(mx, sm, threadIdx.x, 2 * R16_THREADS, out2 + row, direct);
}

__global__ void __launch_bounds__(NORM_THREADS)
embed_norm_quarter_split_kernel(const double* __restrict__ f, const double2* __restrict__ wtab, int logn, int logh,
                                double2* __restrict__ park, unsigned long long* __restrict__ out2)
{
  extern __shared__ __attribute__((aligned(16))) double sm[];
  const unsigned N = 1u << logn, M = N >> 1, H = 1u << logh, S = M >> logh, half = S >> 1;
  double* re = sm;
  double* im = sm + H;
  const unsigned row = blockIdx.x / half, s = blockIdx.x % half;
  const unsigned tid = threadIdx.x, nth = blockDim.x;
  const double2* fp = reinterpret_cast<const double2*>(f + (size_t)row * N);
  double2* pk = park + ((size_t)row * half + s) * H;
  const unsigned mmask = 2 * N - 1;
  for (int pass = 0; pass < 2; pass++) {
    const unsigned sub = pass == 0 ? S - 1 - s : s;
    for (unsigned i = tid; i < H; i += nth) {
      double ar = 0, ai = 0;
      for (unsigned t = 0; t < S; t++) {
        const unsigned idx = i + t * H;
        const unsigned e = (2u * idx * (2u * sub + 1u)) & mmask;
        const double2 w = wtab[e & (N - 1)];
        const double2 v = fp[idx];
        const double zr = v.x * w.x - v.y * w.y, zi = v.x * w.y + v.y * w.x;
        ar += e >= N ? -zr : zr;
        ai += e >= N ? -zi : zi;
      }
      re[i] = ar;
      im[i] = ai;
    }
    __syncthreads();
    dif_fft_lds<NORM_MAX_LOGH, NORM_THREADS>(re, im, logh, N, wtab, tid, nth);
    if (pass == 0) {
      for (unsigned p = tid; p < H; p += nth)
        pk[p] = make_double2(re[p], im[p]);
      __syncthreads();
    }
  }
  double mx = 0;
  for (unsigned p = tid; p < H; p += nth) {
    const unsigned j = s + S * (__brev(p) >> (32 - logh));
    const double2 c = pk[H - 1 - p];
    const double zr = re[p], zi = im[p], cr = c.x, ci = -c.y;
    const double er = 0.5 * (zr + cr), ei = 0.5 * (zi + ci);
    const double dr = zr - cr, di = zi - ci;
    const double orr = 0.5 * di, oi = -0.5 * dr;
    const double2 w = wtab[2 * j + 1];
    const double tr = orr * w.x - oi * w.y, ti = orr * w.y + oi * w.x;
    const double a = (er + tr) * (er + tr) + (ei + ti) * (ei + ti);
    const double b = (er - tr) * (er - tr) + (ei - ti) * (ei - ti);
    const double n2 = a > b ? a : b;
    mx = n2 > mx ? n2 : mx;
  }
  block_max_to(mx, sm, tid, nth, out2 + row);
}

__device__ __forceinline__ void dit_ifft_lds(double* re, double* im, int logh, unsigned tw_half,
                                             const double2* __restrict__ wtab, unsigned tid, unsigned nth)
{
  const unsigned H = 1u << logh;
  for (unsigned len = 1; len < H; len <<= 1) {
    const unsigned s1 = tw_half / len;
    for (unsigned q = tid; q < (H >> 1); q += nth) {
      const unsigned j = q & (len - 1), k = ((q / len) * 2 * len) + j;
      const double2 T = wtab[j * s1];
      const double br = re[k + len] * T.x + im[k + len] * T.y;
      const double bi = im[k + len] * T.x - re[k + len] * T.y;
      const double ar = re[k], ai = im[k];
      re[k] = ar + br, im[k] = ai + bi;
      re[k + len] = ar - br, im[k + len] = ai - bi;
// ... 120 lines not shown
```

### helib_amd/csrc/norm_r16.h

```cpp
#pragma once
#include <stdint.h>

#ifndef HXD
#if defined(__HIPCC__)
#define HXD __host__ __device__ __forceinline__
#else
#define HXD inline
#endif
#endif

namespace hx {

struct cplx16 {
  double x, y;
};
struct tw16 {
  double x, y;
};
constexpr unsigned R16_LOGN = 14, R16_N = 1u << R16_LOGN, R16_M = R16_N >> 1, R16_THREADS = 512;
constexpr unsigned R16_LDS_DOUBLES = R16_M + (R16_M >> 5);
HXD unsigned r16_pad(unsigned i) { return i + (i >> 5); }

HXD tw16 r16_cmul(tw16 a, tw16 b) { return tw16{a.x * b.x - a.y * b.y, a.x * b.y + a.y * b.x}; }
template <int LOGS, int LOGTAB = 14>
HXD void r16_pass(cplx16 (&v)[16], unsigned j0, const tw16* wtab)
{
  constexpr unsigned S = 1u << LOGS;
  tw16 B = wtab[j0 * ((1u << LOGTAB) / (S * 8u))];
#pragma unroll
  for (unsigned h = 8; h >= 1; h >>= 1) {
#pragma unroll
    for (unsigned k = 0; k < 16; k++) {
      if (k & h)
        continue;
      const unsigned kp = k & (h - 1);
      const tw16 T = kp == 0 ? B : r16_cmul(B, wtab[kp * ((1u << LOGTAB) / h)]);
      const cplx16 a = v[k], b = v[k + h];
      const double dx = a.x - b.x, dy = a.y - b.y;
      v[k].x = a.x + b.x;
      v[k].y = a.y + b.y;
      v[k + h].x = dx * T.x - dy * T.y;
      v[k + h].y = dx * T.y + dy * T.x;
    }
    B = r16_cmul(B, B);
  }
}
HXD unsigned r16_pos_A(unsigned t, unsigned k) { return t + 512u * k; }
HXD unsigned r16_pos_B(unsigned t, unsigned k) { return 512u * (t >> 5) + (t & 31u) + 32u * k; }
HXD unsigned r16_pos_C(unsigned t, unsigned k) { return 32u * (t >> 1) + (t & 1u) + 2u * k; }

HXD double r16_pair_norm2(cplx16 z, cplx16 partner, tw16 w)
{
  const double cr = partner.x, ci = -partner.y;
  const double er = 0.5 * (z.x + cr), ei = 0.5 * (z.y + ci);
  const double dr = z.x - cr, di = z.y - ci;
  const double orr = 0.5 * di, oi = -0.5 * dr;
  const double tr = orr * w.x - oi * w.y, ti = orr * w.y + oi * w.x;
  const double a = (er + tr) * (er + tr) + (ei + ti) * (ei + ti);
  const double b = (er - tr) * (er - tr) + (ei - ti) * (ei - ti);
  return a > b ? a : b;
}
HXD unsigned r16_brev4(unsigned i) { return ((i & 1u) << 3) | ((i & 2u) << 1) | ((i & 4u) >> 1) | ((i & 8u) >> 3); }
HXD cplx16 r16_last_lane(cplx16 own, cplx16 other, unsigned t)
{
  return (t & 1u) ? cplx16{other.x - own.x, other.y - own.y} : cplx16{own.x + other.x, own.y + other.y};
}
constexpr unsigned R16_XCHG_IM = 4096;
HXD unsigned r16_xchg_idx(unsigned t, unsigned kk) { return kk * 512u + t; }
HXD unsigned r16_brev8(unsigned x)
{
  unsigned r = 0;
  for (int i = 0; i < 8; i++)
    r |= ((x >> i) & 1u) << (7 - i);
  return r;
}
HXD unsigned r16_pair_tw_thread(unsigned t) { return 8192u * (t & 1u) + 2u * r16_brev8(t >> 1) + 1u; }
HXD unsigned r16_pair_tw_k(unsigned k) { return 512u * r16_brev4(k); }

HXD cplx16 r16_split_input(const double* f, const tw16* wtab, unsigned i, unsigned sub)
{
  constexpr unsigned N = 1u << 15, H = 8192u, mmask = 2u * N - 1u;
  cplx16 acc{0.0, 0.0};
  for (unsigned t = 0; t < 2; t++) {
    const unsigned idx = i + t * H;
    const unsigned e = (2u * idx * (2u * sub + 1u)) & mmask;
    const tw16 w = wtab[e & (N - 1u)];
    const double vx = f[2 * idx], vy = f[2 * idx + 1];
    const double zr = vx * w.x - vy * w.y, zi = vx * w.y + vy * w.x;
    acc.x += e >= N ? -zr : zr;
    acc.y += e >= N ? -zi : zi;
  }
  return acc;
}
HXD unsigned r16x2_pair_tw_thread(unsigned h, unsigned t)
{
  const unsigned a = 16384u * (t & 1u) + 4u * r16_brev8(t >> 1);
  return h ? 32765u - a : a + 1u;
}
HXD unsigned r16x2_pair_tw_k(unsigned k) { return 1024u * r16_brev4(k); }
HXD double r16x2_pair(unsigned h, cplx16 own, cplx16 other, tw16 wth, tw16 wk, unsigned k)
{
  const tw16 u = h ? tw16{wk.x, -wk.y} : wk;
  const tw16 w = k == 0 ? wth : r16_cmul(wth, u);
  return h ? r16_pair_norm2(other, own, w) : r16_pair_norm2(own, other, w);
}

}
```

### helib_amd/csrc/ntt_core.h

```cpp
#pragma once
#include <stdint.h>
#include <utility>
#if defined(HX_CHECK_BOUNDS) && !defined(__HIP_DEVICE_COMPILE__)
#include <cstdio>
#include <cstdlib>
#include <type_traits>
#endif

#if defined(__HIPCC__)
#define HXD __host__ __device__ __forceinline__
#else
#define HXD inline
#endif

namespace hx {

struct TW {
  uint64_t w;
  uint64_t wp;
};

HXD uint64_t mulhi64(uint64_t a, uint64_t b)
{
#if defined(__HIP_DEVICE_COMPILE__)
// ... 559 lines not shown
    constexpr int rep = i / NGRUN, ii = i % NGRUN;
    constexpr int sp = grp_sp<S, INV>(ii), k = grp_k<S, INV>(ii);
    constexpr int half = (1 << (S - 1)) >> sp;
    constexpr int base = rep * (1 << S) + k * 2 * half;
    const typename AR::Tw t = tq[i % PF];
    static_for<0, half>([&](auto J) {
      constexpr int j = decltype(J)::value;
      if constexpr (INV) {
        constexpr int ex = S - 1 - sp;
        constexpr int bprev = AR::inv_after(BIN, ex - 1, k * 2 * half + j);
        AR::template gs<bprev>(v[base + j], v[base + j + half], t, c);
      } else {
        AR::template ct<BIN, sp>(v[base + j], v[base + j + half], t, c);
      }
    });
    if constexpr (i + PF < TOT) {
      constexpr int n = i + PF;
      constexpr int nrep = n / NGRUN, nsp = grp_sp<S, INV>(n % NGRUN), nk = grp_k<S, INV>(n % NGRUN);
      tq[i % PF] = fetch(nrep, nsp, nk, (uint32_t)v[base]);
    }
    if constexpr (HX_BF_FENCE > 0) {
      if constexpr (half >= HX_BF_FENCE)
        HX_SCHED_FENCE();
      else if constexpr ((k + 1) % (HX_BF_FENCE / half) == 0)
        HX_SCHED_FENCE();
    }
  });
}
template <int S, bool INV, int REP, int NGRUN, int BIN, class Fetch>
HXD void run_pass(uint64_t (&v)[32], const QC& c, Fetch fetch)
{
  run_pass<ArShoup, S, INV, REP, NGRUN, BIN>(v, c, fetch);
}

template <int LOGN>
HXD unsigned ab_addr_A(unsigned tid, int e) { return brev5((unsigned)e) + 33u * tid; }
template <int LOGN>
HXD unsigned ab_addr_B(unsigned tid, int eB)
{
  constexpr int LC = Geo<LOGN>::LC;
  return (tid & 31u) + 33u * (((unsigned)eB << LC) + (tid >> 5));
}
template <int LOGN>
HXD unsigned bc_addr_B(unsigned tid, int eB)
{
  return (tid & 31u) + 32u * brev5((unsigned)eB) + 1024u * (tid >> 5);
}
template <int LOGN>
HXD unsigned bc_addr_C(unsigned tid, int i)
{
  constexpr int LC = Geo<LOGN>::LC;
  constexpr int T = Geo<LOGN>::T;
  unsigned gi = (unsigned)i >> LC, ep = (unsigned)i & ((1u << LC) - 1u);
  return (tid + (unsigned)T * gi) + 1024u * ep;
}

template <class Cst, int E>
struct LdsOff {
  static constexpr unsigned bytes = Cst::at(E) * 4u;
  static constexpr unsigned chunk = bytes >> 16, imm = bytes & 0xffffu;
};
#if defined(__HIP_DEVICE_COMPILE__) && !defined(HX_LDS_RD_PLAIN)
template <int OFF>
__device__ __forceinline__ uint32_t ds_rd_b32(unsigned a)
{
  uint32_t x;
  asm volatile("ds_read_b32 %0, %1 offset:%2" : "=v"(x) : "v"(a), "n"(OFF) : "memory");
  return x;
}
template <class Cst>
HXD void lds_read32(const uint32_t* lds, unsigned base, uint32_t (&o)[32])
{
  const unsigned a0 = (unsigned)(uintptr_t)lds + base * 4u;
  const unsigned a1 = a0 + 0x10000u, a2 = a0 + 0x20000u;
  static_for<0, 32>([&](auto I) {
    constexpr int e = decltype(I)::value;
    using O = LdsOff<Cst, e>;
    static_assert(O::chunk <= 2, "LDS offset");
    o[e] = ds_rd_b32<(int)O::imm>(O::chunk == 0 ? a0 : (O::chunk == 1 ? a1 : a2));
  });
  asm volatile("s_waitcnt lgkmcnt(0)"
               : "+v"(o[0]), "+v"(o[1]), "+v"(o[2]), "+v"(o[3]), "+v"(o[4]), "+v"(o[5]), "+v"(o[6]),
                 "+v"(o[7]), "+v"(o[8]), "+v"(o[9]), "+v"(o[10]), "+v"(o[11]), "+v"(o[12]),
                 "+v"(o[13]), "+v"(o[14]), "+v"(o[15])
               :
               : "memory");
  asm volatile(""
               : "+v"(o[16]), "+v"(o[17]), "+v"(o[18]), "+v"(o[19]), "+v"(o[20]), "+v"(o[21]),
                 "+v"(o[22]), "+v"(o[23]), "+v"(o[24]), "+v"(o[25]), "+v"(o[26]), "+v"(o[27]),
                 "+v"(o[28]), "+v"(o[29]), "+v"(o[30]), "+v"(o[31])
               :
               : "memory");
}
#else
template <class Cst>
HXD void lds_read32(const uint32_t* lds, unsigned base, uint32_t (&o)[32])
{
  for (int e = 0; e < 32; e++)
    o[e] = lds[base + Cst::at(e)];
}
#endif
template <int LOGN>
struct CstAbB {
  static constexpr unsigned at(int e) { return 33u * ((unsigned)e << Geo<LOGN>::LC); }
};
template <int LOGN>
struct CstBcC {
  static constexpr unsigned at(int i)
  {
    return (unsigned)Geo<LOGN>::T * ((unsigned)i >> Geo<LOGN>::LC) + 1024u * ((unsigned)i & ((1u << Geo<LOGN>::LC) - 1u));
  }
};
template <int LOGN>
struct CstBcB {
  static constexpr unsigned at(int e) { return 32u * brev_bits((unsigned)e, 5); }
};
template <int LOGN>
struct CstAbA {
  static constexpr unsigned at(int e) { return brev_bits((unsigned)e, 5); }
};
HXD uint32_t half_of(uint64_t x, int half) { return half ? (uint32_t)(x >> 32) : (uint32_t)x; }
HXD void set_half(uint64_t& x, int half, uint32_t w)
{
  x = half ? ((x & 0xffffffffull) | ((uint64_t)w << 32)) : ((x & 0xffffffff00000000ull) | w);
}

template <int LOGN>
HXD unsigned coef_index(unsigned tid, int e) { return ((unsigned)e << (LOGN - 5)) + tid; }
template <int LOGN>
HXD unsigned eval_index(unsigned tid, int i)
{
  constexpr int LC = Geo<LOGN>::LC;
  constexpr int T = Geo<LOGN>::T;
  unsigned gi = (unsigned)i >> LC, ep = (unsigned)i & ((1u << LC) - 1u);
  return brev_bits(ep, LC) * 1024u + tid + (unsigned)T * gi;
}

template <int LOGN>
HXD unsigned coef_const(int e) { return (unsigned)e << (LOGN - 5); }
template <int LOGN>
HXD unsigned eval_const(int i)
{
  constexpr int LC = Geo<LOGN>::LC;
  constexpr int T = Geo<LOGN>::T;
  unsigned gi = (unsigned)i >> LC, ep = (unsigned)i & ((1u << LC) - 1u);
  return brev_bits(ep, LC) * 1024u + (unsigned)T * gi;
}

template <class IO, class = void>
struct io_skip_load : std::false_type {};
template <class IO>
struct io_skip_load<IO, std::void_t<decltype(IO::SKIP_LOAD)>> : std::integral_constant<bool, IO::SKIP_LOAD> {};

template <class IO, class AR, class = void>
struct io_load_bound : std::integral_constant<int, IO::LOAD_BOUND> {};
template <class IO, class AR>
struct io_load_bound<IO, AR, std::void_t<decltype(IO::template load_bound<AR>())>>
    : std::integral_constant<int, IO::template load_bound<AR>()> {};

template <class IO, class AR, class = void>
struct io_inv_load_bound : std::integral_constant<int, 1> {};
template <class IO, class AR>
struct io_inv_load_bound<IO, AR, std::void_t<decltype(IO::template inv_load_bound<AR>())>>
    : std::integral_constant<int, IO::template inv_load_bound<AR>()> {};

struct PtrIO {
  static constexpr int LOAD_BOUND = 1;
  static constexpr bool LAZY_STORE = false;
  static constexpr bool PIPELINED = false;
  struct StorePrefetch {};
  const uint64_t* in;
  uint64_t* out;
  HXD uint64_t load(unsigned tid, unsigned c) const { return in[tid + c]; }
  HXD void store(unsigned tid, unsigned c, uint64_t v) const { out[tid + c] = v; }
  HXD TW last_tw(TW def, int) const { return def; }
  HXD TWM last_tw(TWM def, int) const { return def; }
};

HXD uint64_t norm4(uint64_t x, uint64_t q, uint64_t q2)
{
  x = (x >= q2) ? x - q2 : x;
  return (x >= q) ? x - q : x;
}
HXD uint64_t norm2(uint64_t x, uint64_t q)
{
  return (x >= q) ? x - q : x;
}
template <int B, bool EST = false>
HXD uint64_t norm_from(uint64_t x, const QC& c)
{
  static_assert(B >= 1 && B <= 16, "bound");
  HX_BOUND(x, B, c.q);
  if constexpr (EST && B > 4) {
    const uint32_t xl = (uint32_t)x, xh = (uint32_t)(x >> 32);
    const uint64_t t = (uint64_t)xh * c.mu32 + mulhi32(xl, c.mu32);
    const uint32_t e = (uint32_t)(t >> 32);
    const uint32_t nl = (uint32_t)c.nq, nh = (uint32_t)(c.nq >> 32);
    uint64_t r = (uint64_t)e * nl + x;
    r += (uint64_t)(e * nh) << 32;
    HX_BOUND(r, 2, c.q);
    return csub(r, c.q);
  } else {
    if constexpr (B > 8)
      x = csub(x, c.q8);
    if constexpr (B > 4)
      x = csub(x, c.q4);
    if constexpr (B > 2)
      x = csub(x, c.q + c.q);
    if constexpr (B > 1)
      x = csub(x, c.q);
    return x;
  }
}

template <int LOGN, class AR = ArShoup>
struct RowNTT {
  using G = Geo<LOGN>;
  static constexpr int NPHASE = 8;


  template <int PH, class IO, class TWS>
  static HXD void fwd(unsigned tid, uint64_t (&v)[32], uint32_t (&nl)[32], uint32_t* lds,
                      const IO& io, const TWS& tw, const QC& c)
  {
    constexpr int LB = io_load_bound<IO, AR>::value;
    constexpr int L0 = LB * AR::U;
    constexpr int FA = pass_bound_out<AR, 5, false, 31, L0>();
    constexpr int FB = pass_bound_out<AR, 5, false, 31, FA>();
    constexpr int FCU = pass_bound_out<AR, G::LC, false, G::GC - 1, FB>();
    constexpr int FC = (FCU + AR::U - 1) / AR::U;
    static_assert(LB <= AR::FWD_LOAD_MAX && FA <= 16 * AR::U && FB <= 16 * AR::U && FCU <= 16 * AR::U, "lazy bounds");
    if constexpr (PH == 0) {
      if constexpr (IO::PIPELINED) {
        io.template load_all<LOGN, AR>(tid, v, c);
      } else {
#pragma unroll
        for (int e = 0; e < 32; e++) {
          v[e] = io.load(tid, coef_const<LOGN>(e));
          HX_IO_FENCE(e);
        }
      }
      run_pass<AR, 5, false, 1, 31, L0>(v, c, [&](int, int sp, int k, uint32_t) {
        return tw_uni(tw, (unsigned)((1 << sp) - 1 + k));
      });
#pragma unroll
      for (int e = 0; e < 32; e++)
        lds[ab_addr_A<LOGN>(tid, e)] = half_of(v[e], 0);
    } else if constexpr (PH == 1) {
      lds_read32<CstAbB<LOGN>>(lds, ab_addr_B<LOGN>(tid, 0), nl);
    } else if constexpr (PH == 2) {
#pragma unroll
      for (int e = 0; e < 32; e++)
        lds[ab_addr_A<LOGN>(tid, e)] = half_of(v[e], 1);
    } else if constexpr (PH == 3) {
      uint32_t nh[32];
      lds_read32<CstAbB<LOGN>>(lds, ab_addr_B<LOGN>(tid, 0), nh);
#pragma unroll
      for (int e = 0; e < 32; e++)
        v[e] = ((uint64_t)nh[e] << 32) | nl[e];
      run_pass<AR, 5, false, 1, 31, FA>(v, c, [&](int, int sp, int k, uint32_t dep) {
        return tw_vec(tw, G::TWB, tid & 31u, ((1u << sp) - 1u + (unsigned)k) * 32u, dep);
      });
    } else if constexpr (PH == 4) {
#pragma unroll
      for (int e = 0; e < 32; e++)
        lds[bc_addr_B<LOGN>(tid, e)] = half_of(v[e], 0);
    } else if constexpr (PH == 5) {
      lds_read32<CstBcC<LOGN>>(lds, bc_addr_C<LOGN>(tid, 0), nl);
    } else if constexpr (PH == 6) {
#pragma unroll
      for (int e = 0; e < 32; e++)
        lds[bc_addr_B<LOGN>(tid, e)] = half_of(v[e], 1);
    } else if constexpr (PH == 7) {
      uint32_t nh[32];
      lds_read32<CstBcC<LOGN>>(lds, bc_addr_C<LOGN>(tid, 0), nh);
#pragma unroll
      for (int i = 0; i < 32; i++)
        v[i] = ((uint64_t)nh[i] << 32) | nl[i];
      typename IO::StorePrefetch pre;
      if constexpr (IO::LAZY_STORE)
        io.template store_prefetch<LOGN>(tid, pre);
      run_pass<AR, G::LC, false, G::NGC, G::GC - 1, FB>(v, c, [&](int gi, int sp, int k, uint32_t dep) {
        return tw_vec(tw, G::TWC, tid, ((1u << sp) - 1u + (unsigned)k) * 1024u + (unsigned)(G::T * gi), dep);
      });
      if constexpr (IO::LAZY_STORE) {
        if (c.mu32)
          io.template store_all<LOGN, AR, FC, true>(tid, v, c, pre);
        else
          io.template store_all<LOGN, AR, FC, false>(tid, v, c, pre);
      } else if (c.mu32) {
#pragma unroll
        for (int i = 0; i < 32; i++) {
          io.store(tid, eval_const<LOGN>(i), norm_from<FC, true>(v[i], c));
          HX_IO_FENCE(i);
        }
      } else {
#pragma unroll
        for (int i = 0; i < 32; i++) {
          io.store(tid, eval_const<LOGN>(i), norm_from<FC, false>(v[i], c));
          HX_IO_FENCE(i);
        }
      }
    }
  }

  template <int PH, class IO, class TWS>
  static HXD void inv(unsigned tid, uint64_t (&v)[32], uint32_t (&nl)[32], uint32_t* lds,
                      const IO& io, const TWS& tw, const QC& c)
  {
    constexpr int I0 = io_inv_load_bound<IO, AR>::value;
    constexpr int IC_ = pass_bound_out<AR, G::LC, true, G::GC - 1, I0>();
    constexpr int IB = pass_bound_out<AR, 5, true, 31, IC_>();
    static_assert(I0 <= AR::inv_cap() && IC_ <= AR::inv_cap() && IB <= AR::inv_cap(), "lazy bounds");
    if constexpr (PH == 0) {
      if constexpr (!io_skip_load<IO>::value) {
#pragma unroll
        for (int i = 0; i < 32; i++)
          v[i] = io.load(tid, eval_const<LOGN>(i));
      }
      run_pass<AR, G::LC, true, G::NGC, G::GC - 1, I0>(v, c, [&](int gi, int sp, int k, uint32_t dep) {
        return tw_vec(tw, G::TWC, tid, ((1u << sp) - 1u + (unsigned)k) * 1024u + (unsigned)(G::T * gi), dep);
      });
#pragma unroll
      for (int i = 0; i < 32; i++)
        lds[bc_addr_C<LOGN>(tid, i)] = half_of(v[i], 0);
    } else if constexpr (PH == 1) {
      lds_read32<CstBcB<LOGN>>(lds, bc_addr_B<LOGN>(tid, 0), nl);
    } else if constexpr (PH == 2) {
#pragma unroll
      for (int i = 0; i < 32; i++)
        lds[bc_addr_C<LOGN>(tid, i)] = half_of(v[i], 1);
    } else if constexpr (PH == 3) {
      uint32_t nh[32];
      lds_read32<CstBcB<LOGN>>(lds, bc_addr_B<LOGN>(tid, 0), nh);
#pragma unroll
      for (int e = 0; e < 32; e++)
        v[e] = ((uint64_t)nh[e] << 32) | nl[e];
      run_pass<AR, 5, true, 1, 31, IC_>(v, c, [&](int, int sp, int k, uint32_t dep) {
        return tw_vec(tw, G::TWB, tid & 31u, ((1u << sp) - 1u + (unsigned)k) * 32u, dep);
      });
    } else if constexpr (PH == 4) {
#pragma unroll
      for (int e = 0; e < 32; e++)
        lds[ab_addr_B<LOGN>(tid, e)] = half_of(v[e], 0);
    } else if constexpr (PH == 5) {
      lds_read32<CstAbA<LOGN>>(lds, ab_addr_A<LOGN>(tid, 0), nl);
    } else if constexpr (PH == 6) {
#pragma unroll
      for (int e = 0; e < 32; e++)
        lds[ab_addr_B<LOGN>(tid, e)] = half_of(v[e], 1);
    } else if constexpr (PH == 7) {
      uint32_t nh[32];
      lds_read32<CstAbA<LOGN>>(lds, ab_addr_A<LOGN>(tid, 0), nh);
#pragma unroll
      for (int e = 0; e < 32; e++)
        v[e] = ((uint64_t)nh[e] << 32) | nl[e];
      run_pass<AR, 5, true, 1, 30, IB>(v, c, [&](int, int sp, int k, uint32_t) {
        return tw_uni(tw, (unsigned)((1 << sp) - 1 + k));
      });
      {
        const typename AR::Tw tS = io.last_tw(tw_uni(tw, 0), 0), tN = io.last_tw(tw_uni(tw, 31), 1);
        static_for<0, 16>([&](auto J) {
          constexpr int j = decltype(J)::value;
          AR::template gs_last<AR::inv_after(IB, 3, j)>(v[j], v[j + 16], tN, tS, c);
          if constexpr (HX_BF_FENCE > 0 && j % 2 == 1)
            HX_SCHED_FENCE();
        });
      }
#pragma unroll
      for (int e = 0; e < 32; e++) {
        io.store(tid, coef_const<LOGN>(e), norm_from<AR::INV_OUT>(v[e], c));
        HX_IO_FENCE(e);
      }
    }
  }
};

template <int LOGN, class MulMod>
inline void build_tw_tables_sub(uint64_t q, uint64_t psi, uint64_t psi_inv, uint64_t n_inv,
                                MulMod mulmod, int OUT, unsigned g, TW* fwd, TW* inv)
{
  using G = Geo<LOGN>;
  const int FULL = LOGN + OUT;
  const int NF = 1 << FULL;
  uint64_t* pw = new uint64_t[NF];
  uint64_t* ipw = new uint64_t[NF];
  pw[0] = ipw[0] = 1;
  for (int i = 1; i < NF; i++) {
    pw[i] = mulmod(pw[i - 1], psi, q);
    ipw[i] = mulmod(ipw[i - 1], psi_inv, q);
  }
  auto mk = [&](uint64_t w) {
    TW t;
    t.w = w;
    t.wp = (uint64_t)((((unsigned __int128)w) << 64) / q);
    return t;
  };
  auto src = [&](unsigned idx) {
    int sp = 31 - __builtin_clz(idx);
    unsigned j = idx - (1u << sp);
    unsigned full = (((1u << OUT) + g) << sp) + j;
    return brev_bits(full, FULL);
  };
  for (int i = 0; i < G::TW_TOTAL; i++) {
    fwd[i] = mk(0);
    inv[i] = mk(0);
  }
  for (int s = 0; s < 5; s++)
    for (int k = 0; k < (1 << s); k++) {
      unsigned e = src(twA_src<LOGN>(s, k));
      fwd[(1 << s) - 1 + k] = mk(pw[e]);
      inv[(1 << s) - 1 + k] = mk(ipw[e]);
    }
  inv[0] = mk(mulmod(ipw[src(1)], n_inv, q));
  inv[31] = mk(n_inv);
  for (int sp = 0; sp < 5; sp++)
    for (int k = 0; k < (1 << sp); k++)
      for (unsigned hip = 0; hip < 32; hip++) {
        unsigned e = src(twB_src<LOGN>(sp, k, hip));
        fwd[G::TWB + ((1 << sp) - 1 + k) * 32 + hip] = mk(pw[e]);
        inv[G::TWB + ((1 << sp) - 1 + k) * 32 + hip] = mk(ipw[e]);
      }
  for (int sp = 0; sp < G::LC; sp++)
    for (int k = 0; k < (1 << sp); k++)
      for (unsigned u = 0; u < 1024; u++) {
        unsigned e = src(twC_src<LOGN>(sp, k, u));
        fwd[G::TWC + ((1 << sp) - 1 + k) * 1024 + u] = mk(pw[e]);
        inv[G::TWC + ((1 << sp) - 1 + k) * 1024 + u] = mk(ipw[e]);
      }
  delete[] pw;
  delete[] ipw;
}

template <int LOGN, class MulMod>
inline void build_tw_tables(uint64_t q, uint64_t psi, uint64_t psi_inv, uint64_t n_inv,
                            MulMod mulmod, TW* fwd, TW* inv)
{
  build_tw_tables_sub<LOGN>(q, psi, psi_inv, n_inv, mulmod, 0, 0u, fwd, inv);
}
inline TWM tw_mont_form(uint64_t w, uint64_t q) { return (uint64_t)((((unsigned __int128)w) << 64) % q); }
inline void tw_tables_to_mont(const TW* t, int n, uint64_t q, TWM* out)
{
  for (int i = 0; i < n; i++)
    out[i] = tw_mont_form(t[i].w, q);
}

template <class MulMod>
inline void build_tw_small(int logn, uint64_t q, uint64_t psi, uint64_t psi_inv, uint64_t n_inv,
                           MulMod mulmod, TW* fwd, TW* inv)
{
  const int N = 1 << logn;
  uint64_t* pw = new uint64_t[N];
  uint64_t* ipw = new uint64_t[N];
  pw[0] = ipw[0] = 1;
  for (int i = 1; i < N; i++) {
    pw[i] = mulmod(pw[i - 1], psi, q);
    ipw[i] = mulmod(ipw[i - 1], psi_inv, q);
  }
  auto mk = [&](uint64_t w) {
    TW t;
    t.w = w;
    t.wp = (uint64_t)((((unsigned __int128)w) << 64) / q);
    return t;
  };
  fwd[0] = mk(0);
  inv[0] = mk(n_inv);
  for (int idx = 1; idx < N; idx++) {
    unsigned e = brev_bits((unsigned)idx, logn);
    fwd[idx] = mk(pw[e]);
    inv[idx] = mk(ipw[e]);
  }
  delete[] pw;
  delete[] ipw;
}

}
```

### helib_amd/csrc/ntt_kernels.hip

```cpp
#include <cstdlib>
#include "dev_common.h"
#include "prof.h"

#include "ntt_kernel_util.h"

#ifdef HX_NTT_ONLY
#define HX_SFX2(n, s) n##_L##s
#define HX_SFX1(n, s) HX_SFX2(n, s)
#define HX_ENTRY(n) HX_SFX1(n, HX_NTT_ONLY)
#else
#define HX_ENTRY(n) n
#endif
#if !defined(HX_NTT_ONLY) || HX_NTT_ONLY == 13
#define HX_SZ_13(...) case 13: return __VA_ARGS__;
#else
#define HX_SZ_13(...)
#endif
#if !defined(HX_NTT_ONLY) || HX_NTT_ONLY == 14
#define HX_SZ_14(...) case 14: return __VA_ARGS__;
#else
#define HX_SZ_14(...)
#endif
#if !defined(HX_NTT_ONLY) || HX_NTT_ONLY == 15
#define HX_SZ_15(...) case 15: return __VA_ARGS__;
#else
#define HX_SZ_15(...)
#endif
#define HX_SZ(N, ...) HX_SZ_##N(__VA_ARGS__)

namespace hx {

typedef int v4i32 __attribute__((ext_vector_type(4)));
typedef int v2i32 __attribute__((ext_vector_type(2)));
__device__ v2i32 hx_buffer_load_v2(v4i32 rsrc, int voffset, int soffset,
                                   int aux) __asm("llvm.amdgcn.raw.buffer.load.v2i32");
__device__ void hx_buffer_store_v2(v2i32 data, v4i32 rsrc, int voffset, int soffset,
                                   int aux) __asm("llvm.amdgcn.raw.buffer.store.v2i32");

#ifdef HX_NO_NT
#define HX_NT 0
#define HX_NT_ASM ""
#else
#define HX_NT 2
#define HX_NT_ASM " nt"
#endif

__device__ v4i32 hx_buffer_load_v4(v4i32 rsrc, int voffset, int soffset,
                                   int aux) __asm("llvm.amdgcn.raw.buffer.load.v4i32");

__device__ __forceinline__ v4i32 make_rsrc(const uint64_t* row, unsigned bytes)
{
  uint64_t a = (uint64_t)row;
  v4i32 r;
  r.x = __builtin_amdgcn_readfirstlane((int)(uint32_t)a);
  r.y = __builtin_amdgcn_readfirstlane((int)(uint32_t)(a >> 32));
  r.z = (int)bytes;
  r.w = 0x00020000;
  return r;
}
struct BufTw {
  v4i32 r;
  const TW* p;
  __device__ explicit BufTw(const TW* tw) : r(make_rsrc(reinterpret_cast<const uint64_t*>(tw), 0xfffffff0u)), p(tw) {}
};
__device__ __forceinline__ TW tw_uni(const BufTw& t, unsigned i) { return t.p[i]; }
__device__ __forceinline__ TW tw_vec(const BufTw& t, unsigned base, unsigned lane, unsigned off, uint32_t dep)
{
  int vo = (int)(lane * 16u);
  asm volatile("" : "+v"(vo) : "v"(dep));
  const v4i32 x = hx_buffer_load_v4(t.r, vo, (int)((base + off) * 16u), 0);
  TW w;
  w.w = ((uint64_t)(uint32_t)x.y << 32) | (uint32_t)x.x;
  w.wp = ((uint64_t)(uint32_t)x.w << 32) | (uint32_t)x.z;
  return w;
}

template <int LB>
struct BufIOT {
  static constexpr int LOAD_BOUND = LB;
#ifndef HX_DIGITS_LB8
  template <class AR>
  static constexpr int load_bound() { return (LB == 8 && AR::PROTH) ? 2 : LB; }
#endif
  static constexpr bool LAZY_STORE = false;
  static constexpr bool PIPELINED = false;
  struct StorePrefetch {};
  v4i32 rin, rout;
  __device__ BufIOT(const uint64_t* in_row, uint64_t* out_row, unsigned bytes)
      : rin(make_rsrc(in_row, bytes)), rout(make_rsrc(out_row, bytes))
  {
  }
  __device__ __forceinline__ uint64_t load(unsigned tid, unsigned c) const
  {
    v2i32 r = hx_buffer_load_v2(rin, (int)(tid * 8u), (int)(c * 8u), HX_NT);
    return ((uint64_t)(uint32_t)r.y << 32) | (uint32_t)r.x;
  }
  __device__ __forceinline__ void store(unsigned tid, unsigned c, uint64_t v) const
  {
    v2i32 d;
    d.x = (int)(uint32_t)v;
    d.y = (int)(uint32_t)(v >> 32);
    hx_buffer_store_v2(d, rout, (int)(tid * 8u), (int)(c * 8u), HX_NT);
  }
  __device__ __forceinline__ TW last_tw(TW def, int) const { return def; }
  __device__ __forceinline__ TWM last_tw(TWM def, int) const { return def; }
};

struct InvPrepIO {
  static constexpr int LOAD_BOUND = 1;
  static constexpr bool LAZY_STORE = false;
  static constexpr bool PIPELINED = false;
  struct StorePrefetch {};
  v4i32 rin, rx;
  TW upS, upN;
  uint32_t has_up;
  __device__ InvPrepIO(const uint64_t* in_row, const ModDownPrep& p, size_t boff, unsigned bytes)
      : rin(make_rsrc(in_row, bytes)), rx(make_rsrc(p.xs + boff, bytes)), upS(p.upS), upN(p.upN),
        has_up(p.has_up)
  {
  }
  __device__ __forceinline__ uint64_t load(unsigned tid, unsigned c) const
  {
    v2i32 r = hx_buffer_load_v2(rin, (int)(tid * 8u), (int)(c * 8u), HX_NT);
    return ((uint64_t)(uint32_t)r.y << 32) | (uint32_t)r.x;
  }
  __device__ __forceinline__ void store(unsigned tid, unsigned c, uint64_t x) const
  {
    v2i32 d;
    d.x = (int)(uint32_t)x;
    d.y = (int)(uint32_t)(x >> 32);
    hx_buffer_store_v2(d, rx, (int)(tid * 8u), (int)(c * 8u), 0);
  }
  __device__ __forceinline__ TW last_tw(TW def, int which) const
  {
    return has_up ? (which ? upN : upS) : def;
  }
  __device__ __forceinline__ TWM last_tw(TWM def, int which) const
  {
    return has_up ? (which ? upN.wp : upS.wp) : def;
  }
};

__device__ __forceinline__ int64_t moddown_S_of(const ModDownPrep& P, uint64_t x)
{
  const bool neg = x > P.half;
  int64_t S = neg ? 1 : 0;
  if (P.ptxt > 1) {
    const uint64_t p = P.ptxt;
    uint64_t r = red64(x, p, P.ptxt_mu64);
    if (neg)
      r = sub_mod(r, P.qd_mod_p, p);
    if (r != 0) {
      const uint64_t dm = (p >> 32) == 0 ? red64(r * P.qdinv_mod_p, p, P.ptxt_mu64)
                                         : mul_mod(r, P.qdinv_mod_p, p, P.ptxt_mu, P.ptxt_k);
      const uint64_t p2 = p >> 1;
      const bool sub_p = dm > p2 || (((p & 1) == 0) && dm == p2 && neg);
      S += sub_p ? (int64_t)dm - (int64_t)p : (int64_t)dm;
    }
  }
  return S;
}
template <int UNUSED = 0>
__global__ void __launch_bounds__(256)
moddown_S_kernel(ModDownPrep P, size_t n2)
{
  const ulonglong2* xs = reinterpret_cast<const ulonglong2*>(P.xs);
  longlong2* S = reinterpret_cast<longlong2*>(P.S);
  for (size_t i = (size_t)blockIdx.x * blockDim.x + threadIdx.x; i < n2; i += (size_t)gridDim.x * blockDim.x) {
    const ulonglong2 x = xs[i];
    longlong2 s;
    s.x = moddown_S_of(P, x.x);
    s.y = moddown_S_of(P, x.y);
    S[i] = s;
  }
}

template <bool PLAIN>
struct ModDownIO {
  static constexpr int LOAD_BOUND = PLAIN ? 8 : 6;
  template <class AR>
#ifndef HX_DIGITS_LB8
  static constexpr int load_bound() { return AR::PROTH ? 4 : (PLAIN ? 8 : 6); }
#else
  static constexpr int load_bound() { return PLAIN ? 8 : (AR::PROTH ? 4 : 6); }
#endif
  static constexpr bool LAZY_STORE = true;
  static constexpr bool PIPELINED = !PLAIN;
  static constexpr int IOG = 4;
  struct StorePrefetch {
    uint64_t c[IOG];
  };
  v4i32 rx, rS, rc, ro;
  TW inv, cf;
  uint64_t q;
  __device__ ModDownIO(const uint64_t* x_row, const int64_t* S_row, const ModDownRow& R, const uint64_t* c_row,
                       uint64_t* o_row, unsigned bytes, uint64_t q_)
      : rx(make_rsrc(x_row, bytes)), rS(make_rsrc((const uint64_t*)S_row, bytes)),
        rc(make_rsrc(c_row, bytes)), ro(make_rsrc(o_row, bytes)), inv(R.inv), cf(R.cf), q(q_)
  {
  }
  __device__ __forceinline__ uint64_t load(unsigned tid, unsigned c) const
  {
    v2i32 a = hx_buffer_load_v2(rx, (int)(tid * 8u), (int)(c * 8u), HX_NT);
    return ((uint64_t)(uint32_t)a.y << 32) | (uint32_t)a.x;
  }
  static __device__ __forceinline__ uint64_t ld(const v4i32& r, unsigned tid, unsigned c)
  {
    v2i32 a = hx_buffer_load_v2(r, (int)(tid * 8u), (int)(c * 8u), 0);
    return ((uint64_t)(uint32_t)a.y << 32) | (uint32_t)a.x;
  }
  template <int LOGN, class AR>
  __device__ __forceinline__ void load_all(unsigned tid, uint64_t (&v)[32], const QC& qc) const
  {
    static_for<0, 32>([&](auto E) {
      constexpr int e = decltype(E)::value;
      v[e] = ld(rx, tid, coef_const<LOGN>(e));
    });
    uint64_t sb[2][IOG];
    static_for<0, IOG>([&](auto J) {
      constexpr int j = decltype(J)::value;
      sb[0][j] = ld(rS, tid, coef_const<LOGN>(j));
    });
    HX_SCHED_FENCE();
    static_for<0, 32 / IOG>([&](auto GI) {
      constexpr int g = decltype(GI)::value;
      if constexpr (g + 1 < 32 / IOG)
        static_for<0, IOG>([&](auto J) {
          constexpr int j = decltype(J)::value;
          sb[(g + 1) & 1][j] = ld(rS, tid, coef_const<LOGN>((g + 1) * IOG + j));
        });
      static_for<0, IOG>([&](auto J) {
        constexpr int j = decltype(J)::value, e = g * IOG + j;
        if constexpr (AR::PROTH)
          v[e] = mont_acc(v[e], inv.wp, qc, q - sb[g & 1][j]);
        else
          v[e] = shoup4_acc(v[e], inv, qc.nq, q - sb[g & 1][j]);
      });
      HX_SCHED_FENCE();
    });
  }
  static __device__ __forceinline__ uint64_t ld_pinned(const v4i32& r, unsigned tid, unsigned c)
  {
    uint64_t x;
    asm volatile("buffer_load_dwordx2 %0, %1, %2, %3 offen" HX_NT_ASM
                 : "=v"(x)
                 : "v"((int)(tid * 8u)), "s"(r), "s"((int)(c * 8u))
                 : "memory");
    return x;
  }
  template <int N>
  static __device__ __forceinline__ void pinned_wait(uint64_t (&x)[IOG])
  {
    static_assert(IOG == 4, "operand list");
    asm volatile("s_waitcnt vmcnt(%4)" : "+v"(x[0]), "+v"(x[1]), "+v"(x[2]), "+v"(x[3]) : "n"(N) : "memory");
  }
  template <int LOGN>
  __device__ __forceinline__ void store_prefetch(unsigned tid, StorePrefetch& pre) const
  {
    static_for<0, IOG>([&](auto J) {
      constexpr int j = decltype(J)::value;
      pre.c[j] = ld_pinned(rc, tid, eval_const<LOGN>(j));
    });
  }
  template <int LOGN, class AR, int B, bool EST>
  __device__ __forceinline__ void store_all(unsigned tid, uint64_t (&v)[32], const QC& qc, StorePrefetch& pre) const
  {
    static_assert(!AR::PROTH || B <= 14, "B q - x + 2q must stay below 16q");
    const uint64_t Bq = (uint64_t)B * qc.q;
    uint64_t cb[2][IOG];
    static_for<0, IOG>([&](auto J) { cb[0][decltype(J)::value] = pre.c[decltype(J)::value]; });
    static_for<0, 32 / IOG>([&](auto GI) {
      constexpr int g = decltype(GI)::value;
      constexpr bool more = g + 1 < 32 / IOG;
      if constexpr (more)
        static_for<0, IOG>([&](auto J) {
          constexpr int j = decltype(J)::value;
          cb[(g + 1) & 1][j] = ld_pinned(rc, tid, eval_const<LOGN>((g + 1) * IOG + j));
        });
      pinned_wait<(g > 0 ? IOG : 0) + (more ? IOG : 0)>(cb[g & 1]);
      static_for<0, IOG>([&](auto J) {
        constexpr int j = decltype(J)::value, i = g * IOG + j;
        uint64_t x = v[i];
        if constexpr (AR::PROTH) {
          put(tid, eval_const<LOGN>(i), norm_from<B + 2, EST>(mont_acc(cb[g & 1][j], cf.wp, qc, Bq - x), qc));
        } else {
          if constexpr (B > 8)
            x = csub(x, qc.q8);
          put(tid, eval_const<LOGN>(i), norm_from<12, EST>(shoup4_acc(cb[g & 1][j], cf, qc.nq, qc.q8 - x), qc));
        }
      });
      HX_SCHED_FENCE();
    });
  }
  __device__ __forceinline__ void put(unsigned tid, unsigned c, uint64_t o) const
  {
    asm volatile("buffer_store_dwordx2 %0, %1, %2, %3 offen" HX_NT_ASM
                 :
                 : "v"(o), "v"((int)(tid * 8u)), "s"(ro), "s"((int)(c * 8u))
                 : "memory");
  }
  __device__ __forceinline__ TW last_tw(TW def, int) const { return def; }
  __device__ __forceinline__ TWM last_tw(TWM def, int) const { return def; }
};


template <int LOGN, bool INV, class AR, class IO>
__device__ __forceinline__ void ntt_body_ar(uint32_t* lds, const IO& io, const typename AR::Tw* tw, const QC& q)
{
  using R = RowNTT<LOGN, AR>;
  uint64_t v[32];
  uint32_t nl[32];
  const unsigned w = wave_index();
  if constexpr (!INV) {
    R::template fwd<0>(fresh_tid(w), v, nl, lds, io, tw, q);
    __syncthreads();
    R::template fwd<1>(fresh_tid(w), v, nl, lds, io, tw, q);
    __syncthreads();
    R::template fwd<2>(fresh_tid(w), v, nl, lds, io, tw, q);
    __syncthreads();
    R::template fwd<3>(fresh_tid(w), v, nl, lds, io, tw, q);
    __syncthreads();
    R::template fwd<4>(fresh_tid(w), v, nl, lds, io, tw, q);
    __syncthreads();
    R::template fwd<5>(fresh_tid(w), v, nl, lds, io, tw, q);
    __syncthreads();
    R::template fwd<6>(fresh_tid(w), v, nl, lds, io, tw, q);
    __syncthreads();
    R::template fwd<7>(fresh_tid(w), v, nl, lds, io, tw, q);
  } else {
    R::template inv<0>(fresh_tid(w), v, nl, lds, io, tw, q);
    __syncthreads();
    R::template inv<1>(fresh_tid(w), v, nl, lds, io, tw, q);
    __syncthreads();
    R::template inv<2>(fresh_tid(w), v, nl, lds, io, tw, q);
    __syncthreads();
    R::template inv<3>(fresh_tid(w), v, nl, lds, io, tw, q);
    __syncthreads();
    R::template inv<4>(fresh_tid(w), v, nl, lds, io, tw, q);
    __syncthreads();
    R::template inv<5>(fresh_tid(w), v, nl, lds, io, tw, q);
    __syncthreads();
    R::template inv<6>(fresh_tid(w), v, nl, lds, io, tw, q);
    __syncthreads();
    R::template inv<7>(fresh_tid(w), v, nl, lds, io, tw, q);
  }
}
template <int LOGN, bool INV, class IO>
__device__ __forceinline__ void ntt_body(uint32_t* lds, const IO& io, const TW* tw_ptr, const PrimeDev* pd)
{
  const QC q = make_qc(pd->q, pd->mu64);
#ifndef HX_NO_PROTH
  if (pd->proth) {
    ntt_body_ar<LOGN, INV, ArProth>(lds, io, reinterpret_cast<const TWM*>(tw_ptr), q);
    return;
  }
#endif
  ntt_body_ar<LOGN, INV, ArShoup>(lds, io, tw_ptr, q);
}

template <int LOGN>
__global__ void __launch_bounds__(Geo<LOGN>::T, HX_NTT_MINWAVES(LOGN))
ntt_moddown_prep_kernel(PolyBases polys, int row, int prime, int batch, ModDownPrep P,
                        const PrimeDev* __restrict__ primes, const TW* __restrict__ tw_arena)
{
  extern __shared__ __attribute__((aligned(16))) uint32_t lds[];
  const int b = (int)(blockIdx.x % (unsigned)batch), pi = (int)(blockIdx.x / (unsigned)batch);
  const PrimeDev* pd = primes + prime;
  const size_t N = Geo<LOGN>::N;
  const uint64_t* in = poly_base(polys, (unsigned)pi);
  const size_t pstride = P.poly_stride ? (size_t)P.poly_stride : (size_t)batch * N;
  const InvPrepIO io(in + ((size_t)row * batch + b) * N, P, (size_t)pi * pstride + (size_t)b * N,
                     (unsigned)N * 8u);
  ntt_body<LOGN, true>(lds, io, tw_arena + pd->tw_inv_off, pd);
}
template <int LOGN>
__global__ void __launch_bounds__(Geo<LOGN>::T, HX_NTT_MINWAVES(LOGN))
ntt_moddown_prep_multi_kernel(PolyBases polys, PrepMulti M, int batch, ModDownPrep P,
                              const PrimeDev* __restrict__ primes, const TW* __restrict__ tw_arena)
{
  extern __shared__ __attribute__((aligned(16))) uint32_t lds[];
  const unsigned per = (unsigned)polys.n * (unsigned)batch;
  const unsigned j = blockIdx.x / per, rem = blockIdx.x % per;
  const int b = (int)(rem % (unsigned)batch), pi = (int)(rem / (unsigned)batch);
  const PrimeDev* pd = primes + uniform_u16(M.prime, j);
  const int row = (int)uniform_u16(M.row, j);
  const size_t N = Geo<LOGN>::N;
  const uint64_t* in = poly_base(polys, (unsigned)pi);
  ModDownPrep Pj = P;
  Pj.xs = P.xs + (size_t)j * (size_t)batch * N;
  Pj.upS = M.up[2 * j];
  Pj.upN = M.up[2 * j + 1];
  const InvPrepIO io(in + ((size_t)row * batch + b) * N, Pj, (size_t)pi * (size_t)P.poly_stride + (size_t)b * N,
                     (unsigned)N * 8u);
  ntt_body<LOGN, true>(lds, io, tw_arena + pd->tw_inv_off, pd);
}
template <int LOGN, bool PLAIN>
__global__ void __launch_bounds__(Geo<LOGN>::T, HX_NTT_MINWAVES(LOGN))
ntt_moddown_apply_kernel(PolyBases polys, PolyBases outs, NttRows rows, int nkeep, int batch, ModDownApply A,
                         const PrimeDev* __restrict__ primes, const TW* __restrict__ tw_arena)
{
  extern __shared__ __attribute__((aligned(16))) uint32_t lds[];
#ifdef HX_MD_OLDMAP
  const unsigned wid = xcd_remap(blockIdx.x, gridDim.x);
  const int b = (int)(wid % (unsigned)batch);
  const unsigned rp = wid / (unsigned)batch;
  const unsigned pi = rp % (unsigned)polys.n, ri = rp / (unsigned)polys.n;
#else
  const MdWork Wk = md_work(blockIdx.x, (unsigned)nkeep, (unsigned)polys.n * (unsigned)batch);
  if (!Wk.active)
    return;
  const unsigned ri = Wk.ri, pb = Wk.pb;
  const int b = (int)(pb % (unsigned)batch);
  const unsigned pi = pb / (unsigned)batch;
#endif
  const PrimeDev* pd = primes + uniform_u16(rows.prime, ri);
  const size_t N = Geo<LOGN>::N;
  const ModDownRow R = A.rows[ri];
  uint64_t* odata = poly_base(outs, pi);
  const uint64_t* idata = R.mode == 2 ? odata : poly_base(polys, pi);
  const size_t eoff = ((size_t)pi * batch + b) * N;
  const uint64_t* xrow = PLAIN ? A.delta + (size_t)pi * (size_t)A.delta_poly_stride + ((size_t)ri * batch + b) * N
                               : A.xs + eoff;
  const ModDownIO<PLAIN> io(xrow, PLAIN ? nullptr : A.S + eoff, R,
                            idata + ((size_t)(R.mode == 2 ? R.out_row : uniform_u16(rows.row, ri)) * batch + b) * N,
                            odata + ((size_t)R.out_row * batch + b) * N, (unsigned)N * 8u, pd->q);
  ntt_body<LOGN, false>(lds, io, tw_arena + pd->tw_fwd_off, pd);
}

__device__ __forceinline__ uint64_t tensor_red128(u128 S, uint64_t q, uint64_t mu63, uint32_t k)
{
  const uint64_t xt = (uint64_t)(S >> (k - 1));
  const uint32_t xl = (uint32_t)xt, xh = (uint32_t)(xt >> 32);
  const uint32_t ml = (uint32_t)mu63, mh = (uint32_t)(mu63 >> 32);
  const uint64_t qh = (uint64_t)xh * mh + __umulhi(xh, ml) + __umulhi(xl, mh);
  uint64_t r = (uint64_t)S - qh * q;
  r = csub(r, q << 2);
  r = csub(r, q << 1);
  return csub(r, q);
}
__device__ __forceinline__ uint64_t tensor_value(unsigned part, uint64_t a0, uint64_t a1, uint64_t b0, uint64_t b1,
                                                 uint64_t q, uint64_t mu, uint32_t k)
{
  if (part == 1)
    return tensor_red128((u128)a0 * b1 + (u128)a1 * b0, q, mu, k);
  return tensor_red128((u128)a0 * b0, q, mu, k);
}
struct InvPrepTensorIO {
  static constexpr int LOAD_BOUND = 1;
  static constexpr bool LAZY_STORE = false;
  static constexpr bool PIPELINED = false;
  struct StorePrefetch {};
  v4i32 ra, rb, rc, rd, rx;
  TW upS, upN;
  uint32_t has_up, part, k;
  uint64_t q, mu;
  __device__ InvPrepTensorIO(const TensorSrc& T, unsigned part_, size_t roff, const ModDownPrep& p, size_t xoff,
                             unsigned bytes, const PrimeDev* pd)
      : ra(make_rsrc((part_ == 2 ? T.a1 : T.a0) + roff, bytes)),
        rb(make_rsrc((part_ == 0 ? T.b0 : T.b1) + roff, bytes)),
        rc(make_rsrc(T.a1 + roff, bytes)), rd(make_rsrc(T.b0 + roff, bytes)),
        rx(make_rsrc(p.xs + xoff, bytes)), upS(p.upS), upN(p.upN), has_up(p.has_up), part(part_), k(pd->k), q(pd->q),
        mu(pd->mu63)
  {
  }
  static __device__ __forceinline__ uint64_t ld(const v4i32& r, unsigned tid, unsigned c)
  {
    v2i32 a = hx_buffer_load_v2(r, (int)(tid * 8u), (int)(c * 8u), 0);
    return ((uint64_t)(uint32_t)a.y << 32) | (uint32_t)a.x;
  }
  __device__ __forceinline__ uint64_t load(unsigned tid, unsigned c) const
  {
    const uint64_t x = ld(ra, tid, c), y = ld(rb, tid, c);
    if (part == 1)
      return tensor_value(1, x, ld(rc, tid, c), ld(rd, tid, c), y, q, mu, k);
    return tensor_value(0, x, 0, y, 0, q, mu, k);
  }
  __device__ __forceinline__ void store(unsigned tid, unsigned c, uint64_t x) const
  {
    v2i32 d;
    d.x = (int)(uint32_t)x;
    d.y = (int)(uint32_t)(x >> 32);
    hx_buffer_store_v2(d, rx, (int)(tid * 8u), (int)(c * 8u), 0);
  }
  __device__ __forceinline__ TW last_tw(TW def, int which) const { return has_up ? (which ? upN : upS) : def; }
  __device__ __forceinline__ TWM last_tw(TWM def, int which) const { return has_up ? (which ? upN.wp : upS.wp) : def; }
};
template <int LOGN>
__global__ void __launch_bounds__(Geo<LOGN>::T, HX_NTT_MINWAVES(LOGN))
ntt_moddown_prep_tensor_kernel(TensorSrc T, int row, int prime, int batch, ModDownPrep P,
                               const PrimeDev* __restrict__ primes, const TW* __restrict__ tw_arena)
{
  extern __shared__ __attribute__((aligned(16))) uint32_t lds[];
  const int b = (int)(blockIdx.x % (unsigned)batch), pi = (int)(blockIdx.x / (unsigned)batch);
  const PrimeDev* pd = primes + prime;
  const size_t N = Geo<LOGN>::N;
  const InvPrepTensorIO io(T, (unsigned)pi, ((size_t)row * batch + b) * N, P, ((size_t)pi * batch + b) * N,
                           (unsigned)N * 8u, pd);
  ntt_body<LOGN, true>(lds, io, tw_arena + pd->tw_inv_off, pd);
}

template <int LOGN>
__global__ void __launch_bounds__(Geo<LOGN>::T, HX_NTT_MINWAVES(LOGN))
ntt_moddown_prep_multi_tensor_kernel(TensorSrc T, PrepMulti M, int batch, ModDownPrep P,
                                     const PrimeDev* __restrict__ primes, const TW* __restrict__ tw_arena)
{
  extern __shared__ __attribute__((aligned(16))) uint32_t lds[];
  const unsigned per = 3u * (unsigned)batch;
  const unsigned j = blockIdx.x / per, rem = blockIdx.x % per;
  const int b = (int)(rem % (unsigned)batch), pi = (int)(rem / (unsigned)batch);
  const PrimeDev* pd = primes + uniform_u16(M.prime, j);
  const int row = (int)uniform_u16(M.row, j);
  const size_t N = Geo<LOGN>::N;
  ModDownPrep Pj = P;
  Pj.xs = P.xs + (size_t)j * (size_t)batch * N;
  Pj.upS = M.up[2 * j];
  Pj.upN = M.up[2 * j + 1];
  const InvPrepTensorIO io(T, (unsigned)pi, ((size_t)row * batch + b) * N, Pj,
                           (size_t)pi * (size_t)P.poly_stride + (size_t)b * N, (unsigned)N * 8u, pd);
  ntt_body<LOGN, true>(lds, io, tw_arena + pd->tw_inv_off, pd);
}

template <bool PLAIN>
struct ModDownTensorIO {
  static constexpr int LOAD_BOUND = PLAIN ? 8 : 6;
  template <class AR>
#ifndef HX_DIGITS_LB8
  static constexpr int load_bound() { return AR::PROTH ? 4 : (PLAIN ? 8 : 6); }
#else
  static constexpr int load_bound() { return PLAIN ? 8 : (AR::PROTH ? 4 : 6); }
#endif
  static constexpr bool LAZY_STORE = true;
  static constexpr bool PIPELINED = !PLAIN;
  static constexpr int IOG = 4;
  struct StorePrefetch {};
  v4i32 rx, rS, ra, rb, rc, rd, ro;
  TW inv, cf;
  uint64_t cf_r2;
  uint64_t q, mu;
  uint32_t part, k;
  __device__ ModDownTensorIO(const uint64_t* x_row, const int64_t* S_row, const ModDownRow& R, const TensorSrc& T,
                             unsigned part_, size_t roff, bool has_row, uint64_t* o_row, unsigned bytes, const PrimeDev* pd)
      : rx(make_rsrc(x_row, bytes)), rS(make_rsrc((const uint64_t*)S_row, bytes)),
        ra(make_rsrc(has_row ? (part_ == 2 ? T.a1 : T.a0) + roff : o_row, bytes)),
        rb(make_rsrc(has_row ? (part_ == 0 ? T.b0 : T.b1) + roff : o_row, bytes)),
        rc(make_rsrc(has_row ? T.a1 + roff : o_row, bytes)), rd(make_rsrc(has_row ? T.b0 + roff : o_row, bytes)),
        ro(make_rsrc(o_row, bytes)), inv(R.inv), cf(R.cf), cf_r2(R.cf_r2), q(pd->q), mu(pd->mu63), part(part_), k(pd->k)
  {
  }
  static __device__ __forceinline__ uint64_t ld(const v4i32& r, unsigned tid, unsigned c)
  {
    v2i32 a = hx_buffer_load_v2(r, (int)(tid * 8u), (int)(c * 8u), 0);
    return ((uint64_t)(uint32_t)a.y << 32) | (uint32_t)a.x;
  }
  __device__ __forceinline__ uint64_t load(unsigned tid, unsigned c) const
  {
    v2i32 a = hx_buffer_load_v2(rx, (int)(tid * 8u), (int)(c * 8u), HX_NT);
    return ((uint64_t)(uint32_t)a.y << 32) | (uint32_t)a.x;
  }
  template <int LOGN, class AR>
  __device__ __forceinline__ void load_all(unsigned tid, uint64_t (&v)[32], const QC& qc) const
  {
    static_for<0, 32>([&](auto E) {
      constexpr int e = decltype(E)::value;
      v[e] = ld(rx, tid, coef_const<LOGN>(e));
    });
    uint64_t sb[2][IOG];
    static_for<0, IOG>([&](auto J) {
      constexpr int j = decltype(J)::value;
      sb[0][j] = ld(rS, tid, coef_const<LOGN>(j));
    });
    HX_SCHED_FENCE();
    static_for<0, 32 / IOG>([&](auto GI) {
      constexpr int g = decltype(GI)::value;
      if constexpr (g + 1 < 32 / IOG)
        static_for<0, IOG>([&](auto J) {
          constexpr int j = decltype(J)::value;
          sb[(g + 1) & 1][j] = ld(rS, tid, coef_const<LOGN>((g + 1) * IOG + j));
        });
      static_for<0, IOG>([&](auto J) {
        constexpr int j = decltype(J)::value, e = g * IOG + j;
        if constexpr (AR::PROTH)
          v[e] = mont_acc(v[e], inv.wp, qc, q - sb[g & 1][j]);
        else
          v[e] = shoup4_acc(v[e], inv, qc.nq, q - sb[g & 1][j]);
      });
      HX_SCHED_FENCE();
    });
  }
  static __device__ __forceinline__ uint64_t ld_pinned(const v4i32& r, unsigned tid, unsigned c)
  {
    uint64_t x;
    asm volatile("buffer_load_dwordx2 %0, %1, %2, %3 offen" : "=v"(x) : "v"((int)(tid * 8u)), "s"(r), "s"((int)(c * 8u)) : "memory");
    return x;
  }
  template <int N>
  static __device__ __forceinline__ void pinned_wait(uint64_t (&x)[8])
  {
    asm volatile("s_waitcnt vmcnt(%8)"
                 : "+v"(x[0]), "+v"(x[1]), "+v"(x[2]), "+v"(x[3]), "+v"(x[4]), "+v"(x[5]), "+v"(x[6]), "+v"(x[7])
                 : "n"(N)
                 : "memory");
  }
  template <int LOGN, bool P1, int g>
  __device__ __forceinline__ void request(unsigned tid, uint64_t (&w)[8]) const
  {
    if constexpr (P1) {
      static_for<0, 2>([&](auto J) {
        constexpr int j = decltype(J)::value;
        constexpr int i = 2 * g + j;
        const unsigned c = eval_const<LOGN>(i);
        w[4 * j + 0] = ld_pinned(ra, tid, c);
        w[4 * j + 1] = ld_pinned(rb, tid, c);
        w[4 * j + 2] = ld_pinned(rc, tid, c);
        w[4 * j + 3] = ld_pinned(rd, tid, c);
      });
    } else {
      static_for<0, 4>([&](auto J) {
        constexpr int j = decltype(J)::value;
        constexpr int i = 4 * g + j;
        const unsigned c = eval_const<LOGN>(i);
        w[2 * j + 0] = ld_pinned(ra, tid, c);
        w[2 * j + 1] = ld_pinned(rb, tid, c);
      });
    }
  }
  template <int LOGN>
  __device__ __forceinline__ void store_prefetch(unsigned, StorePrefetch&) const {}
  template <int LOGN, class AR, int B, bool EST, bool P1>
  __device__ __forceinline__ void store_part(unsigned tid, uint64_t (&v)[32], const QC& qc) const
  {
    constexpr int CPG = P1 ? 2 : 4, NG = 32 / CPG;
    static_assert(!AR::PROTH || B <= 14, "B q - x + 2q must stay below 16q");
    const uint64_t Bq = (uint64_t)B * qc.q;
    auto one = [&](auto I, uint64_t x0, uint64_t y0, uint64_t x1, uint64_t y1) {
      constexpr int i = decltype(I)::value;
      uint64_t x = v[i];
      if constexpr (AR::PROTH) {
        const u128 S = P1 ? (u128)x0 * y0 + (u128)x1 * y1 : (u128)x0 * y0;
        const uint64_t c2 = mont_redc128((uint64_t)S, (uint64_t)(S >> 64), qc);
        put(tid, eval_const<LOGN>(i), norm_from<B + 2, EST>(mont_acc(c2, cf_r2, qc, Bq - x), qc));
      } else {
        const uint64_t c = P1 ? tensor_value(1, x0, x1, y1, y0, q, mu, k) : tensor_value(0, x0, 0, y0, 0, q, mu, k);
        if constexpr (B > 8)
          x = csub(x, qc.q8);
        put(tid, eval_const<LOGN>(i), norm_from<12, EST>(shoup4_acc(c, cf, qc.nq, qc.q8 - x), qc));
      }
    };
    uint64_t wb[2][8];
    request<LOGN, P1, 0>(tid, wb[0]);
    static_for<0, NG>([&](auto GI) {
      constexpr int g = decltype(GI)::value;
// ... 287 lines not shown
  constexpr size_t lds_bytes = (size_t)Geo<LOGN>::LDS_WORDS * 4;
  hipError_t e = hxp::dyn_lds((const void*)ntt_keyswitch_last_kernel<LOGN, ND>, (int)lds_bytes, device);
  if (e != hipSuccess)
    return e;
  HX_LAUNCH((ntt_keyswitch_last_kernel<LOGN, ND>), dim3((unsigned)A.nall * (unsigned)A.batch), dim3(Geo<LOGN>::T), lds_bytes,
            st, A, map, plan, primes, tw_arena);
  return hipGetLastError();
}
template <int LOGN>
static hipError_t launch_ks_last_nd(int nd, const KsLastArgs& A, const RowMap2& map, const KsLastPlan& plan, int device,
                                    const PrimeDev* primes, const TW* tw_arena, hipStream_t st)
{
  switch (nd) {
    case 2: return launch_ks_last<LOGN, 2>(A, map, plan, device, primes, tw_arena, st);
    case 3: return launch_ks_last<LOGN, 3>(A, map, plan, device, primes, tw_arena, st);
    case 4: return launch_ks_last<LOGN, 4>(A, map, plan, device, primes, tw_arena, st);
  }
  return hipErrorInvalidValue;
}
hipError_t HX_ENTRY(launch_keyswitch_last_pow2)(int logn, int nd, const KsLastArgs& A, const RowMap2& map, const KsLastPlan& plan,
                                                int device, const PrimeDev* primes, const TW* tw_arena, hipStream_t st)
{
  switch (logn) {
    HX_SZ(13, launch_ks_last_nd<13>(nd, A, map, plan, device, primes, tw_arena, st))
    HX_SZ(14, launch_ks_last_nd<14>(nd, A, map, plan, device, primes, tw_arena, st))
    HX_SZ(15, launch_ks_last_nd<15>(nd, A, map, plan, device, primes, tw_arena, st))
  }
  return hipErrorInvalidValue;
}
#endif

#if !defined(HX_NTT_PART) || HX_NTT_PART == 1
template <bool PROTH>
struct MulLoadIO {
  static constexpr int LOAD_BOUND = 1;
  static constexpr bool LAZY_STORE = false;
  static constexpr bool PIPELINED = false;
  template <class AR>
  static constexpr int inv_load_bound() { return PROTH ? 2 : 1; }
  struct StorePrefetch {};
  v4i32 ra, rb, ro;
  uint64_t q, mu63, r2;
  uint32_t k;
  __device__ MulLoadIO(const uint64_t* a_row, const uint64_t* b_row, uint64_t* o_row, unsigned bytes, const PrimeDev* pd)
      : ra(make_rsrc(a_row, bytes)), rb(make_rsrc(b_row, bytes)), ro(make_rsrc(o_row, bytes)), q(pd->q), mu63(pd->mu63),
        r2(pd->r2), k(pd->k)
  {
  }
  __device__ __forceinline__ uint64_t load(unsigned tid, unsigned c) const
  {
    const v2i32 x = hx_buffer_load_v2(ra, (int)(tid * 8u), (int)(c * 8u), HX_NT);
    const v2i32 y = hx_buffer_load_v2(rb, (int)(tid * 8u), (int)(c * 8u), HX_NT);
    const uint64_t a = ((uint64_t)(uint32_t)x.y << 32) | (uint32_t)x.x, b = ((uint64_t)(uint32_t)y.y << 32) | (uint32_t)y.x;
    const u128 p = (u128)a * b;
    if constexpr (PROTH)
      return mont_redc128((uint64_t)p, (uint64_t)(p >> 64), make_qc(q, 0));
    else
      return tensor_red128(p, q, mu63, k);
  }
  __device__ __forceinline__ void store(unsigned tid, unsigned c, uint64_t v) const
  {
    v2i32 d;
    d.x = (int)(uint32_t)v;
    d.y = (int)(uint32_t)(v >> 32);
    hx_buffer_store_v2(d, ro, (int)(tid * 8u), (int)(c * 8u), HX_NT);
  }
  __device__ __forceinline__ TW last_tw(TW def, int) const { return def; }
  __device__ __forceinline__ TWM last_tw(TWM def, int) const
  {
    if constexpr (PROTH) {
      const QC qc = make_qc(q, 0);
      return csub(mont_mul(def, r2, qc), q);
    } else {
      return def;
    }
  }
};
template <int LOGN>
__global__ void __launch_bounds__(Geo<LOGN>::T, HX_NTT_MINWAVES(LOGN))
ntt_inv_mul_kernel(const uint64_t* a, const uint64_t* b, uint64_t* out, NttRows rows, int batch,
                   const PrimeDev* __restrict__ primes, const TW* __restrict__ tw_arena)
{
  extern __shared__ __attribute__((aligned(16))) uint32_t lds[];
  const unsigned wid = xcd_remap(blockIdx.x, gridDim.x);
  const unsigned ri = wid / (unsigned)batch;
  const int bb = (int)(wid % (unsigned)batch);
  const int row = (int)uniform_u16(rows.row, ri);
  const PrimeDev* pd = primes + uniform_u16(rows.prime, ri);
  const size_t N = Geo<LOGN>::N;
  const size_t roff = ((size_t)row * batch + bb) * N, ooff = ((size_t)ri * batch + bb) * N;
  const QC qc = make_qc(pd->q, pd->mu64);
  const TW* tw = tw_arena + pd->tw_inv_off;
#ifndef HX_NO_PROTH
  if (pd->proth) {
#ifndef HX_INVMUL_BARRETT
    const MulLoadIO<true> io(a + roff, b + roff, out + ooff, (unsigned)N * 8u, pd);
#else
    const MulLoadIO<false> io(a + roff, b + roff, out + ooff, (unsigned)N * 8u, pd);
#endif
    ntt_body_ar<LOGN, true, ArProth>(lds, io, reinterpret_cast<const TWM*>(tw), qc);
    return;
  }
#endif
  const MulLoadIO<false> io(a + roff, b + roff, out + ooff, (unsigned)N * 8u, pd);
  ntt_body_ar<LOGN, true, ArShoup>(lds, io, tw, qc);
}
template <int LOGN>
static hipError_t launch_inv_mul(const uint64_t* a, const uint64_t* b, uint64_t* out, const NttRows& rows, int nrows,
                                 int batch, const PrimeDev* primes, const TW* tw_arena, hipStream_t st)
{
  constexpr size_t lds_bytes = (size_t)Geo<LOGN>::LDS_WORDS * 4;
  hipError_t e = hxp::dyn_lds((const void*)ntt_inv_mul_kernel<LOGN>, (int)lds_bytes);
  if (e != hipSuccess)
    return e;
  HX_LAUNCH((ntt_inv_mul_kernel<LOGN>), dim3((unsigned)nrows * (unsigned)batch), dim3(Geo<LOGN>::T), lds_bytes, st, a, b,
            out, rows, batch, primes, tw_arena);
  return hipGetLastError();
}
hipError_t HX_ENTRY(launch_ntt_inv_mul_pow2)(int logn, const uint64_t* a, const uint64_t* b, uint64_t* out, const NttRows& rows,
                                   int nrows, int batch, const PrimeDev* primes, const TW* tw_arena, hipStream_t st)
{
  switch (logn) {
    HX_SZ(13, launch_inv_mul<13>(a, b, out, rows, nrows, batch, primes, tw_arena, st))
    HX_SZ(14, launch_inv_mul<14>(a, b, out, rows, nrows, batch, primes, tw_arena, st))
    HX_SZ(15, launch_inv_mul<15>(a, b, out, rows, nrows, batch, primes, tw_arena, st))
  }
  return hipErrorInvalidValue;
}

template <int LOGN, bool INV, int LB = 1>
static hipError_t launch_one(const uint64_t* in, uint64_t* out, const NttRows& rows, int nrows,
                             int batch, const PrimeDev* primes, const TW* tw_arena, hipStream_t st)
{
#ifdef HX_ROW_ONE_WG
  static const size_t lds_bytes = LOGN == 14 ? (size_t)90 * 1024 : (size_t)Geo<LOGN>::LDS_WORDS * 4;
#else
  static const size_t lds_bytes = (size_t)Geo<LOGN>::LDS_WORDS * 4;
#endif
  hipError_t e = hxp::dyn_lds((const void*)ntt_row_kernel<LOGN, INV, LB>, (int)lds_bytes);
  if (e != hipSuccess)
    return e;
  dim3 grid((unsigned)nrows * (unsigned)batch), block(Geo<LOGN>::T);
  HX_LAUNCH((ntt_row_kernel<LOGN, INV, LB>), grid, block, lds_bytes, st, in, out, rows, batch,
                     primes, tw_arena);
  return hipGetLastError();
}

template <int LOGN>
static hipError_t moddown_attrs()
{
  constexpr size_t lds_bytes = (size_t)Geo<LOGN>::LDS_WORDS * 4;
  hipError_t e = hxp::dyn_lds((const void*)ntt_moddown_prep_kernel<LOGN>, (int)lds_bytes);
  if (e == hipSuccess)
    e = hxp::dyn_lds((const void*)ntt_moddown_prep_multi_kernel<LOGN>, (int)lds_bytes);
  if (e == hipSuccess)
    e = hxp::dyn_lds((const void*)ntt_moddown_apply_kernel<LOGN, false>, (int)lds_bytes);
  if (e == hipSuccess)
    e = hxp::dyn_lds((const void*)ntt_moddown_apply_kernel<LOGN, true>, (int)lds_bytes);
  return e;
}
static unsigned moddown_apply_grid(unsigned npoly, unsigned nkeep, unsigned batch)
{
#ifdef HX_MD_OLDMAP
  return npoly * nkeep * batch;
#else
  return 8u * md_tile(nkeep, npoly * batch).per_xcd;
#endif
}

template <int LOGN>
static hipError_t launch_moddown(const PolyBases& polys, const PolyBases& outs, int drop_row, int drop_prime,
                                 const NttRows& keep, int nkeep, int batch, const ModDownPrep& P,
                                 const ModDownApply& A, const PrimeDev* primes, const TW* tw_arena,
                                 hipStream_t st)
{
  constexpr size_t lds_bytes = (size_t)Geo<LOGN>::LDS_WORDS * 4;
  hipError_t e = moddown_attrs<LOGN>();
  if (e != hipSuccess)
    return e;
  HX_LAUNCH((ntt_moddown_prep_kernel<LOGN>), dim3((unsigned)polys.n * (unsigned)batch),
                     dim3(Geo<LOGN>::T), lds_bytes, st, polys, drop_row, drop_prime, batch, P, primes,
                     tw_arena);
  {
    const size_t n = (size_t)polys.n * (size_t)batch * Geo<LOGN>::N;
    HX_LAUNCH((moddown_S_kernel<0>), dim3((unsigned)((n / 2 + 255) / 256 > 8192 ? 8192 : (n / 2 + 255) / 256)),
                       dim3(256), 0, st, P, n / 2);
  }
  HX_LAUNCH((ntt_moddown_apply_kernel<LOGN, false>),
                     dim3(moddown_apply_grid((unsigned)polys.n, (unsigned)nkeep, (unsigned)batch)),
                     dim3(Geo<LOGN>::T), lds_bytes, st, polys, outs, keep, nkeep, batch, A, primes, tw_arena);
  return hipGetLastError();
}

hipError_t HX_ENTRY(launch_moddown_pow2)(int logn, const PolyBases& data, const PolyBases& out, int drop_row,
                               int drop_prime, const NttRows& keep, int nkeep, int batch,
                               const ModDownPrep& P, const ModDownApply& A, const PrimeDev* primes,
                               const TW* tw_arena, hipStream_t st)
{
  switch (logn) {
    HX_SZ(13, launch_moddown<13>(data, out, drop_row, drop_prime, keep, nkeep, batch, P, A, primes, tw_arena, st))
    HX_SZ(14, launch_moddown<14>(data, out, drop_row, drop_prime, keep, nkeep, batch, P, A, primes, tw_arena, st))
    HX_SZ(15, launch_moddown<15>(data, out, drop_row, drop_prime, keep, nkeep, batch, P, A, primes, tw_arena, st))
  }
  return hipErrorInvalidValue;
}

template <int LOGN>
static hipError_t moddown_tensor_attrs()
{
  constexpr size_t lds_bytes = (size_t)Geo<LOGN>::LDS_WORDS * 4;
  hipError_t e = hxp::dyn_lds((const void*)ntt_moddown_prep_tensor_kernel<LOGN>, (int)lds_bytes);
  if (e == hipSuccess)
    e = hxp::dyn_lds((const void*)ntt_moddown_prep_multi_tensor_kernel<LOGN>, (int)lds_bytes);
  if (e == hipSuccess)
    e = hxp::dyn_lds((const void*)ntt_moddown_apply_tensor_kernel<LOGN, false>, (int)lds_bytes);
  if (e == hipSuccess)
    e = hxp::dyn_lds((const void*)ntt_moddown_apply_tensor_kernel<LOGN, true>, (int)lds_bytes);
  return e;
}
template <int LOGN>
static hipError_t launch_moddown_tensor(const TensorSrc& T, const PolyBases& outs, int drop_row, int drop_prime,
                                        const NttRows& keep, int nkeep, int batch, const ModDownPrep& P,
                                        const ModDownApply& A, const PrimeDev* primes, const TW* tw_arena, hipStream_t st)
{
  constexpr size_t lds_bytes = (size_t)Geo<LOGN>::LDS_WORDS * 4;
  hipError_t ea = moddown_tensor_attrs<LOGN>();
  if (ea != hipSuccess)
    return ea;
  HX_LAUNCH((ntt_moddown_prep_tensor_kernel<LOGN>), dim3(3u * (unsigned)batch), dim3(Geo<LOGN>::T), lds_bytes, st, T,
            drop_row, drop_prime, batch, P, primes, tw_arena);
  {
    const size_t n = (size_t)3 * (size_t)batch * Geo<LOGN>::N;
    HX_LAUNCH((moddown_S_kernel<0>), dim3((unsigned)((n / 2 + 255) / 256 > 8192 ? 8192 : (n / 2 + 255) / 256)), dim3(256), 0, st, P,
              n / 2);
  }
  HX_LAUNCH((ntt_moddown_apply_tensor_kernel<LOGN, false>), dim3(moddown_apply_grid(3u, (unsigned)nkeep, (unsigned)batch)),
            dim3(Geo<LOGN>::T), lds_bytes, st, T, outs, keep, nkeep, batch, A, primes, tw_arena);
  return hipGetLastError();
}
hipError_t HX_ENTRY(launch_moddown_tensor_pow2)(int logn, const TensorSrc& T, const PolyBases& outs, int drop_row, int drop_prime,
                                      const NttRows& keep, int nkeep, int batch, const ModDownPrep& P,
                                      const ModDownApply& A, const PrimeDev* primes, const TW* tw_arena, hipStream_t st)
{
  switch (logn) {
    HX_SZ(13, launch_moddown_tensor<13>(T, outs, drop_row, drop_prime, keep, nkeep, batch, P, A, primes, tw_arena, st))
    HX_SZ(14, launch_moddown_tensor<14>(T, outs, drop_row, drop_prime, keep, nkeep, batch, P, A, primes, tw_arena, st))
    HX_SZ(15, launch_moddown_tensor<15>(T, outs, drop_row, drop_prime, keep, nkeep, batch, P, A, primes, tw_arena, st))
  }
  return hipErrorInvalidValue;
}

template <int LOGN>
static hipError_t launch_prep_multi_tensor(const TensorSrc& T, const PrepMulti& M, int ndrop, int batch, const ModDownPrep& P,
                                           const PrimeDev* primes, const TW* tw_arena, hipStream_t st)
{
  constexpr size_t lds_bytes = (size_t)Geo<LOGN>::LDS_WORDS * 4;
  hipError_t e = moddown_tensor_attrs<LOGN>();
  if (e != hipSuccess)
    return e;
  HX_LAUNCH((ntt_moddown_prep_multi_tensor_kernel<LOGN>), dim3((unsigned)ndrop * 3u * (unsigned)batch), dim3(Geo<LOGN>::T),
            lds_bytes, st, T, M, batch, P, primes, tw_arena);
  return hipGetLastError();
}
template <int LOGN>
static hipError_t launch_apply_plain_tensor(const TensorSrc& T, const PolyBases& outs, const NttRows& keep, int nkeep,
                                            int batch, const ModDownApply& A, const PrimeDev* primes, const TW* tw_arena,
                                            hipStream_t st)
{
  constexpr size_t lds_bytes = (size_t)Geo<LOGN>::LDS_WORDS * 4;
  hipError_t e = moddown_tensor_attrs<LOGN>();
  if (e != hipSuccess)
    return e;
  HX_LAUNCH((ntt_moddown_apply_tensor_kernel<LOGN, true>), dim3(moddown_apply_grid(3u, (unsigned)nkeep, (unsigned)batch)),
            dim3(Geo<LOGN>::T), lds_bytes, st, T, outs, keep, nkeep, batch, A, primes, tw_arena);
  return hipGetLastError();
}
hipError_t HX_ENTRY(launch_moddown_prep_multi_tensor_pow2)(int logn, const TensorSrc& T, const PrepMulti& M, int ndrop, int batch,
                                                 const ModDownPrep& P, const PrimeDev* primes, const TW* tw_arena,
                                                 hipStream_t st)
{
  switch (logn) {
    HX_SZ(13, launch_prep_multi_tensor<13>(T, M, ndrop, batch, P, primes, tw_arena, st))
    HX_SZ(14, launch_prep_multi_tensor<14>(T, M, ndrop, batch, P, primes, tw_arena, st))
    HX_SZ(15, launch_prep_multi_tensor<15>(T, M, ndrop, batch, P, primes, tw_arena, st))
  }
  return hipErrorInvalidValue;
}
hipError_t HX_ENTRY(launch_moddown_apply_plain_tensor_pow2)(int logn, const TensorSrc& T, const PolyBases& outs, const NttRows& keep,
                                                  int nkeep, int batch, const ModDownApply& A, const PrimeDev* primes,
                                                  const TW* tw_arena, hipStream_t st)
{
  switch (logn) {
    HX_SZ(13, launch_apply_plain_tensor<13>(T, outs, keep, nkeep, batch, A, primes, tw_arena, st))
    HX_SZ(14, launch_apply_plain_tensor<14>(T, outs, keep, nkeep, batch, A, primes, tw_arena, st))
    HX_SZ(15, launch_apply_plain_tensor<15>(T, outs, keep, nkeep, batch, A, primes, tw_arena, st))
  }
  return hipErrorInvalidValue;
}

template <int LOGN>
static hipError_t launch_prep_one(const PolyBases& polys, int drop_row, int drop_prime, int batch,
                                  const ModDownPrep& P, const PrimeDev* primes, const TW* tw_arena, hipStream_t st)
{
  constexpr size_t lds_bytes = (size_t)Geo<LOGN>::LDS_WORDS * 4;
  hipError_t e = moddown_attrs<LOGN>();
  if (e != hipSuccess)
    return e;
  HX_LAUNCH((ntt_moddown_prep_kernel<LOGN>), dim3((unsigned)polys.n * (unsigned)batch),
                     dim3(Geo<LOGN>::T), lds_bytes, st, polys, drop_row, drop_prime, batch, P, primes,
                     tw_arena);
  return hipGetLastError();
}
template <int LOGN>
static hipError_t launch_apply_plain(const PolyBases& polys, const PolyBases& outs, const NttRows& keep,
                                     int nkeep, int batch, const ModDownApply& A, const PrimeDev* primes,
                                     const TW* tw_arena, hipStream_t st)
{
  constexpr size_t lds_bytes = (size_t)Geo<LOGN>::LDS_WORDS * 4;
  hipError_t e = moddown_attrs<LOGN>();
  if (e != hipSuccess)
    return e;
  HX_LAUNCH((ntt_moddown_apply_kernel<LOGN, true>),
                     dim3(moddown_apply_grid((unsigned)polys.n, (unsigned)nkeep, (unsigned)batch)),
                     dim3(Geo<LOGN>::T), lds_bytes, st, polys, outs, keep, nkeep, batch, A, primes, tw_arena);
  return hipGetLastError();
}
template <int LOGN>
static hipError_t launch_prep_multi(const PolyBases& polys, const PrepMulti& M, int ndrop, int batch,
                                    const ModDownPrep& P, const PrimeDev* primes, const TW* tw_arena, hipStream_t st)
{
  constexpr size_t lds_bytes = (size_t)Geo<LOGN>::LDS_WORDS * 4;
  hipError_t e = moddown_attrs<LOGN>();
  if (e != hipSuccess)
    return e;
  HX_LAUNCH((ntt_moddown_prep_multi_kernel<LOGN>), dim3((unsigned)ndrop * (unsigned)polys.n * (unsigned)batch),
                     dim3(Geo<LOGN>::T), lds_bytes, st, polys, M, batch, P, primes, tw_arena);
  return hipGetLastError();
}
hipError_t HX_ENTRY(launch_moddown_prep_multi_pow2)(int logn, const PolyBases& polys, const PrepMulti& M, int ndrop, int batch,
                                          const ModDownPrep& P, const PrimeDev* primes, const TW* tw_arena,
                                          hipStream_t st)
{
  switch (logn) {
    HX_SZ(13, launch_prep_multi<13>(polys, M, ndrop, batch, P, primes, tw_arena, st))
    HX_SZ(14, launch_prep_multi<14>(polys, M, ndrop, batch, P, primes, tw_arena, st))
    HX_SZ(15, launch_prep_multi<15>(polys, M, ndrop, batch, P, primes, tw_arena, st))
  }
  return hipErrorInvalidValue;
}
hipError_t HX_ENTRY(launch_moddown_prep_pow2)(int logn, const PolyBases& polys, int drop_row, int drop_prime, int batch,
                                    const ModDownPrep& P, const PrimeDev* primes, const TW* tw_arena,
                                    hipStream_t st)
{
  switch (logn) {
    HX_SZ(13, launch_prep_one<13>(polys, drop_row, drop_prime, batch, P, primes, tw_arena, st))
    HX_SZ(14, launch_prep_one<14>(polys, drop_row, drop_prime, batch, P, primes, tw_arena, st))
    HX_SZ(15, launch_prep_one<15>(polys, drop_row, drop_prime, batch, P, primes, tw_arena, st))
  }
  return hipErrorInvalidValue;
}
hipError_t HX_ENTRY(launch_moddown_apply_plain_pow2)(int logn, const PolyBases& polys, const PolyBases& outs,
                                           const NttRows& keep, int nkeep, int batch, const ModDownApply& A,
                                           const PrimeDev* primes, const TW* tw_arena, hipStream_t st)
{
  switch (logn) {
    HX_SZ(13, launch_apply_plain<13>(polys, outs, keep, nkeep, batch, A, primes, tw_arena, st))
    HX_SZ(14, launch_apply_plain<14>(polys, outs, keep, nkeep, batch, A, primes, tw_arena, st))
    HX_SZ(15, launch_apply_plain<15>(polys, outs, keep, nkeep, batch, A, primes, tw_arena, st))
  }
  return hipErrorInvalidValue;
}

template <bool INV>
__global__ void __launch_bounds__(256)
ntt_small_kernel(const uint64_t* in, uint64_t* out, NttRows rows, int batch, int logn,
                 const PrimeDev* __restrict__ primes, const TW* __restrict__ tw_arena)
{
  extern __shared__ __attribute__((aligned(16))) uint64_t sm[];
  const unsigned N = 1u << logn, tid = threadIdx.x, nth = blockDim.x;
  const unsigned ri = blockIdx.x / (unsigned)batch;
  const int b = (int)(blockIdx.x % (unsigned)batch);
  const PrimeDev* pd = primes + rows.prime[ri];
  const size_t roff = ((size_t)rows.row[ri] * batch + b) * (size_t)N;
  const TW* tw = tw_arena + (INV ? pd->tw_inv_off : pd->tw_fwd_off);
// ... 172 lines not shown
```

### helib_amd/csrc/switches.h

```cpp
#pragma once
#include <cstdlib>

namespace hxs {

struct Switches {
  bool no_hps = false;
  double hps_eps = 1.0 / (double)(1u << 30);
  int hps_min_n = 9;
  int brk_hps_min_n = 5;
  bool no_lazy_rns = false;
  bool no_fast_break = false;
  bool no_fast_extend = false;
  bool no_proth_rns = false;
  bool no_wide_extend = false;
  bool no_mfma_ext = false;
  int mfma_min_n = 9;
  bool no_mask_split = false;
  int brk_lds_pad_rows = 0;
  bool no_tensor_multi = false;
  bool no_mulrelin_fuse = false;
  bool no_ks_last_fuse = false;
  bool half15 = false;
  bool no_proth = false;
  bool blue_old = false;
  bool no_pfa = false;
  bool pfa_no_rem = false;
  bool norm_async = false;
  bool norm_old = false;
  bool norm_plain = false;
  bool norm_memcpy = false;
  int wait_poll_us = 2000;
  bool arena_trace = false;
};

inline Switches read()
{
  Switches s;
  auto on = [](const char* name) { return std::getenv(name) != nullptr; };
  s.no_hps = on("HX_NO_HPS");
  if (const char* e = std::getenv("HX_HPS_EPS"))
    s.hps_eps = std::atof(e);
  if (const char* e = std::getenv("HX_HPS_MIN_N"))
    s.hps_min_n = s.brk_hps_min_n = std::atoi(e);
  if (const char* e = std::getenv("HX_BRK_HPS_MIN_N"))
    s.brk_hps_min_n = std::atoi(e);
  s.no_lazy_rns = on("HX_NO_LAZY_RNS");
  s.no_fast_break = on("HX_NO_FAST_BREAK");
  s.no_fast_extend = on("HX_NO_FAST_EXTEND");
  s.no_proth_rns = on("HX_NO_PROTH_RNS");
  s.no_wide_extend = on("HX_NO_WIDE_EXTEND");
  s.no_mfma_ext = on("HX_NO_MFMA_EXT") || s.no_wide_extend;
  if (const char* e = std::getenv("HX_MFMA_MIN_N"))
    s.mfma_min_n = std::atoi(e);
  s.no_mask_split = on("HX_NO_MASK_SPLIT");
  if (const char* e = std::getenv("HX_BRK_LDS_PAD"))
    s.brk_lds_pad_rows = std::atoi(e);
  s.half15 = on("HX_HALF15");
  s.no_tensor_multi = on("HX_NO_TENSOR_MULTI");
  s.no_mulrelin_fuse = on("HX_NO_MULRELIN_FUSE");
  s.no_ks_last_fuse = on("HX_NO_KS_LAST_FUSE");
  s.no_proth = on("HX_NO_PROTH");
  s.blue_old = on("HX_BLUE_OLD");
  s.no_pfa = on("HX_NO_PFA") || s.blue_old;
  s.pfa_no_rem = on("HX_PFA_NO_REM");
  s.norm_async = on("HX_NORM_ASYNC");
  s.norm_old = on("HX_NORM_OLD");
  s.norm_plain = on("HX_NORM_PLAIN");
  s.norm_memcpy = on("HX_NORM_MEMCPY");
  if (const char* e = std::getenv("HX_WAIT_POLL_US"))
    s.wait_poll_us = std::atoi(e);
  s.arena_trace = on("HX_ARENA_TRACE");
  return s;
}

}
```

Baseline: 44590 mult/s.

## Fuse S computation and canonical-embedding norm into mod-down prep kernel

The mod-down prep kernel gains fused variants. FUSE=1 computes the S/xs values inside the inverse-NTT kernel instead of a separate moddown_S kernel. FUSE=2 (logN=14) additionally evaluates the r16 canonical-embedding norm while the row data is still in registers and LDS, writing maxima straight to a pinned slot. The separate norm pass therefore no longer rereads xs/S from memory. In exchange, prep-norm slot bookkeeping is added, the fused kernels get heavier with more register pressure, and a new direct-twist r16 norm kernel replaces the old one, with the paired version kept behind a switch.

```diff
diff --git a/helib_amd/csrc/dev_common.h b/helib_amd/csrc/dev_common.h
--- a/helib_amd/csrc/dev_common.h
+++ b/helib_amd/csrc/dev_common.h
@@ -40,6 +40,10 @@
   TW upS, upN;
   uint64_t qd;
   uint64_t poly_stride;
+  uint32_t fuse;
+  double inv_qd;
+  const double* wtab;
+  unsigned long long* norm_out;
 };
 constexpr int MD_MAXDROP = 16;
 struct PrepMulti {
diff --git a/helib_amd/csrc/engine.hip b/helib_amd/csrc/engine.hip
--- a/helib_amd/csrc/engine.hip
+++ b/helib_amd/csrc/engine.hip
@@ -205,6 +205,7 @@
   int xs_first = 0, xs_rows = 0;
   double xs_inv_qd = 0;
   bool want_fdelta = false;
+  bool prep_norm = false;
   double2* d_wtab = nullptr;
   double2 *d_bn_v = nullptr, *d_bn_w = nullptr, *d_bn_chat = nullptr, *d_bn_Z = nullptr;
   size_t bn_rows_cap = 0;
@@ -223,6 +224,7 @@
   std::vector<void*> norm_slabs;
   bool defer_norms = false;
   std::vector<NormPending> norm_pending, norm_free;
+  NormPending prep_np{};
   hipStream_t norm_stream = nullptr;
   hipEvent_t norm_in_ev = nullptr, norm_out_ev = nullptr;
   bool norm_reads_xs = false, norm_reads_frac = false;
@@ -539,6 +541,8 @@
   hipFree(c->d_bn_Z);
   hipFree(c->d_norm2);
   hipFree(c->d_norm_park);
+  if (c->prep_norm)
+    c->norm_free.push_back(c->prep_np);
   for (auto* v : {&c->norm_pending, &c->norm_free})
     for (auto& np : *v) {
       hipEventDestroy(np.ev);
@@ -2735,6 +2739,12 @@
 
 static int bn_logp(const hx_ctx* c) { return next_pow2_exp(2 * c->m - 1); }
 
+static void prep_norm_drop(hx_ctx* c)
+{
+  if (c->prep_norm)
+    c->norm_free.push_back(c->prep_np);
+  c->prep_norm = false;
+}
 static int frac_begin(hx_ctx* c, size_t doubles)
 {
   if (!c->pow2 && bn_logp(c) > 18)
@@ -2753,6 +2763,7 @@
   c->frac_pos = 0;
   c->want_frac = true;
   c->xs_rows = 0;
+  prep_norm_drop(c);
   return HX_OK;
 }
 static double* frac_take(hx_ctx* c, size_t doubles)
@@ -2768,6 +2779,7 @@
 {
   if (c->xs_rows <= 0)
     return HX_OK;
+  prep_norm_drop(c);
   const size_t n = (size_t)c->xs_rows * c->phim;
   HX_LAUNCH(hx::frac_from_xs_kernel, dim3((unsigned)std::min<size_t>((n + 255) / 256, 4096)),
                      dim3(256), 0, c->stream, c->scratch[0],
@@ -2865,44 +2877,24 @@
   return HX_OK;
 }
 
-static int embed_norms(hx_ctx* c, const double* d_f, int rows, double* out_host)
-{
+static int norm_wtab(hx_ctx* c)
+{
+  if (!c->pow2 || c->d_wtab)
+    return HX_OK;
   const uint32_t N = c->phim;
-  const int logn = c->logn;
-  if (c->pow2 && !c->d_wtab) {
-    std::vector<double> h(2 * (size_t)N);
-    const long double two_pi = 6.283185307179586476925286766559005768394L;
-    for (uint32_t k = 0; k < N; k++) {
-      long double ang = two_pi * (long double)k / (long double)c->m;
-      h[2 * (size_t)k] = (double)cosl(ang);
-      h[2 * (size_t)k + 1] = (double)sinl(ang);
-    }
-    HIPCHK(hipMalloc((void**)&c->d_wtab, sizeof(double) * 2 * (size_t)N));
-    HIPCHK(hipMemcpy(c->d_wtab, h.data(), sizeof(double) * 2 * (size_t)N, hipMemcpyHostToDevice));
-  }
-  if (c->norm_cap < (size_t)rows) {
-    retire_or_free(c, c->d_norm2);
-    c->d_norm2 = nullptr;
-    c->norm_cap = 0;
-    HIPCHK(hipMalloc((void**)&c->d_norm2, sizeof(unsigned long long) * (size_t)rows));
-    c->norm_cap = (size_t)rows;
-  }
-  const bool quarter_form = c->pow2 && logn >= 2 && logn - 1 <= hx::NORM_MAX_LOGH;
-  const bool use_xs = quarter_form && c->xs_rows == rows && d_f == c->d_frac;
-  if (!use_xs)
-    CHK(flush_xs(c));
-  hipStream_t ns = c->stream;
-  const bool side_stream = c->sw.norm_async;
-  if (side_stream && !c->capturing) {
-    if (!c->norm_stream) {
-      HIPCHK(hipStreamCreateWithFlags(&c->norm_stream, hipStreamNonBlocking));
-      HIPCHK(hipEventCreateWithFlags(&c->norm_in_ev, hipEventDisableTiming));
-      HIPCHK(hipEventCreateWithFlags(&c->norm_out_ev, hipEventDisableTiming));
-    }
-    HIPCHK(hipEventRecord(c->norm_in_ev, c->stream));
-    HIPCHK(hipStreamWaitEvent(c->norm_stream, c->norm_in_ev, 0));
-    ns = c->norm_stream;
-  }
+  std::vector<double> h(2 * (size_t)N);
+  const long double two_pi = 6.283185307179586476925286766559005768394L;
+  for (uint32_t k = 0; k < N; k++) {
+    long double ang = two_pi * (long double)k / (long double)c->m;
+    h[2 * (size_t)k] = (double)cosl(ang);
+    h[2 * (size_t)k + 1] = (double)sinl(ang);
+  }
+  HIPCHK(hipMalloc((void**)&c->d_wtab, sizeof(double) * 2 * (size_t)N));
+  HIPCHK(hipMemcpy(c->d_wtab, h.data(), sizeof(double) * 2 * (size_t)N, hipMemcpyHostToDevice));
+  return HX_OK;
+}
+static int norm_slot_take(hx_ctx* c, int rows, hx_ctx::NormPending* out)
+{
   hx_ctx::NormPending np{};
   bool have = false;
   for (size_t i = 0; i < c->norm_free.size(); i++)
@@ -2935,6 +2927,46 @@
     HIPCHK(hipHostMalloc((void**)&np.pinned, np.cap * sizeof(unsigned long long), hipHostMallocDefault));
     HIPCHK(hipEventCreateWithFlags(&np.ev, hipEventDisableTiming));
   }
+  *out = np;
+  return HX_OK;
+}
+
+static int embed_norms(hx_ctx* c, const double* d_f, int rows, double* out_host)
+{
+  const uint32_t N = c->phim;
+  const int logn = c->logn;
+  CHK(norm_wtab(c));
+  if (c->norm_cap < (size_t)rows) {
+    retire_or_free(c, c->d_norm2);
+    c->d_norm2 = nullptr;
+    c->norm_cap = 0;
+    HIPCHK(hipMalloc((void**)&c->d_norm2, sizeof(unsigned long long) * (size_t)rows));
+    c->norm_cap = (size_t)rows;
+  }
+  const bool quarter_form = c->pow2 && logn >= 2 && logn - 1 <= hx::NORM_MAX_LOGH;
+  const bool use_xs = quarter_form && c->xs_rows == rows && d_f == c->d_frac;
+  if (!use_xs)
+    CHK(flush_xs(c));
+  hipStream_t ns = c->stream;
+  const bool side_stream = c->sw.norm_async;
+  if (side_stream && !c->capturing) {
+    if (!c->norm_stream) {
+      HIPCHK(hipStreamCreateWithFlags(&c->norm_stream, hipStreamNonBlocking));
+      HIPCHK(hipEventCreateWithFlags(&c->norm_in_ev, hipEventDisableTiming));
+      HIPCHK(hipEventCreateWithFlags(&c->norm_out_ev, hipEventDisableTiming));
+    }
+    HIPCHK(hipEventRecord(c->norm_in_ev, c->stream));
+    HIPCHK(hipStreamWaitEvent(c->norm_stream, c->norm_in_ev, 0));
+    ns = c->norm_stream;
+  }
+  hx_ctx::NormPending np{};
+  const bool from_prep = c->prep_norm && use_xs;
+  if (from_prep) {
+    np = c->prep_np;
+    c->prep_norm = false;
+  } else {
+    CHK(norm_slot_take(c, rows, &np));
+  }
   struct SlotGuard {
     hx_ctx* c;
     hx_ctx::NormPending* np;
@@ -2952,11 +2984,10 @@
   unsigned long long* const out2 = direct ? np.pinned : c->d_norm2;
   if (!direct)
     HIPCHK(hipMemsetAsync(c->d_norm2, 0, sizeof(unsigned long long) * (size_t)rows, ns));
-  bool attr = false;
   if (!c->pow2) {
     CHK(flush_xs(c));
     CHK(embed_norms_general(c, d_f, rows, ns));
-  } else if (!attr) {
+  } else {
     HIPCHK(hxp::dyn_lds((const void*)hx::embed_norm_kernel, 16 << hx::NORM_MAX_LOGH));
 #define HX_NORM_ATTR(...)                                                                               \
   HIPCHK(hxp::dyn_lds((const void*)hx::embed_norm_quarter_kernel<__VA_ARGS__>,                   \
@@ -2969,9 +3000,10 @@
     HX_NORM_ATTR(hx::NormSrcXS, 14);
 #undef HX_NORM_ATTR
     HIPCHK(hxp::dyn_lds((const void*)hx::embed_norm_quarter_split_kernel, 16 << hx::NORM_MAX_LOGH));
-    attr = true;
   }
   if (!c->pow2) {
+  } else if (from_prep) {
+    c->xs_rows = 0;
   } else if (logn >= 2 && logn - 1 <= hx::NORM_MAX_LOGH) {
     const unsigned M = N >> 1;
     const unsigned threads = std::min<unsigned>(hx::NORM_THREADS, std::max<unsigned>(64u, M / 4));
@@ -2991,30 +3023,37 @@
   } while (0)
     const bool r16 = !c->sw.norm_old;
     constexpr size_t r16_lds = (size_t)hx::R16_LDS_DOUBLES * sizeof(double);
+    const bool paired = c->sw.no_prep_fuse;
     if (r16 && logn == 14) {
-      bool attr16 = false;
-      if (!attr16) {
-        HIPCHK(hxp::dyn_lds((const void*)hx::embed_norm_r16_kernel<hx::NormSrcXS>, (int)r16_lds));
-        HIPCHK(hxp::dyn_lds((const void*)hx::embed_norm_r16_kernel<hx::NormSrcF64>, (int)r16_lds));
-        attr16 = true;
-      }
-    }
+      HIPCHK(hxp::dyn_lds((const void*)hx::embed_norm_r16_kernel<hx::NormSrcXS>, (int)r16_lds));
+      HIPCHK(hxp::dyn_lds((const void*)hx::embed_norm_r16_kernel<hx::NormSrcF64>, (int)r16_lds));
+      HIPCHK(hxp::dyn_lds((const void*)hx::embed_norm_r16_paired_kernel<hx::NormSrcXS>, (int)r16_lds));
+      HIPCHK(hxp::dyn_lds((const void*)hx::embed_norm_r16_paired_kernel<hx::NormSrcF64>, (int)r16_lds));
+    }
+#define HX_R16_LAUNCH(SRCT, srcv)                                                                                       \
+  do {                                                                                                                  \
+    if (paired)                                                                                                         \
+      HX_LAUNCH((hx::embed_norm_r16_paired_kernel<SRCT>), dim3((unsigned)rows), dim3(hx::R16_THREADS), r16_lds, ns, srcv, \
+                c->d_wtab, out2, direct);                                                                               \
+    else                                                                                                                \
+      HX_LAUNCH((hx::embed_norm_r16_kernel<SRCT>), dim3((unsigned)rows), dim3(hx::R16_THREADS), r16_lds, ns, srcv,      \
+                c->d_wtab, out2, direct);                                                                               \
+  } while (0)
     if (c->xs_rows == rows && d_f == c->d_frac) {
       hx::NormSrcXS src{c->scratch[0], reinterpret_cast<const int64_t*>(c->scratch[1]), c->xs_inv_qd};
       if (r16 && logn == 14)
-        HX_LAUNCH((hx::embed_norm_r16_kernel<hx::NormSrcXS>), dim3((unsigned)rows), dim3(hx::R16_THREADS), r16_lds, ns, src,
-                  c->d_wtab, out2, direct);
+        HX_R16_LAUNCH(hx::NormSrcXS, src);
       else
         HX_NORM_LAUNCH(hx::NormSrcXS, src);
     } else {
       CHK(flush_xs(c));
       hx::NormSrcF64 src{d_f};
       if (r16 && logn == 14)
-        HX_LAUNCH((hx::embed_norm_r16_kernel<hx::NormSrcF64>), dim3((unsigned)rows), dim3(hx::R16_THREADS), r16_lds, ns, src,
-                  c->d_wtab, out2, direct);
+        HX_R16_LAUNCH(hx::NormSrcF64, src);
       else
         HX_NORM_LAUNCH(hx::NormSrcF64, src);
     }
+#undef HX_R16_LAUNCH
 #undef HX_NORM_LAUNCH
     c->xs_rows = 0;
   } else if (logn - 1 > hx::NORM_MAX_LOGH && !c->sw.norm_plain) {
@@ -3605,6 +3644,21 @@
         return fail(HX_ERR_INVALID, "dropped primes are not invertible modulo ptxtSpace");
     }
     P.qd = qd;
+    P.fuse = c->sw.no_prep_fuse ? 0u : 1u;
+    const size_t nfrac = rw * (size_t)pb.n;
+    const bool xs_in_place = c->want_frac && c->xs_rows == 0 && c->frac_pos == 0 && nfrac <= c->frac_cap && !c->want_fdelta;
+    const bool norm_in_prep = P.fuse && xs_in_place && c->logn == 14 && !c->sw.norm_old && !c->sw.norm_memcpy &&
+                              !c->sw.norm_async && !c->capturing && (ptxt >> 32) == 0;
+    if (norm_in_prep) {
+      prep_norm_drop(c);
+      CHK(norm_wtab(c));
+      CHK(norm_slot_take(c, pb.n * a->batch, &c->prep_np));
+      c->prep_norm = true;
+      P.fuse = 2;
+      P.inv_qd = 1.0 / (double)qd;
+      P.wtab = reinterpret_cast<const double*>(c->d_wtab);
+      P.norm_out = c->prep_np.pinned;
+    }
     if (nadd > 0) {
       uint64_t F = 1;
       for (int i = 0; i < nadd; i++)
@@ -3674,8 +3728,10 @@
                                                          c->d_primes, c->d_tw, c->stream)
                         : hx::launch_moddown_pow2(c->logn, pb, pbo, drow, dprime, kr, nk, a->batch, P, A,
                                                   c->d_primes, c->d_tw, c->stream);
-    if (e != hipSuccess)
+    if (e != hipSuccess) {
+      prep_norm_drop(c);
       return fail(HX_ERR_DEVICE, "mod-down launch failed: %s", hipGetErrorString(e));
+    }
     fresh_guard.armed = false;
     for (int i = 0; i < pb.n; i++)
       if (fresh[i]) {
diff --git a/helib_amd/csrc/norm_kernels.h b/helib_amd/csrc/norm_kernels.h
--- a/helib_amd/csrc/norm_kernels.h
+++ b/helib_amd/csrc/norm_kernels.h
@@ -7,27 +7,6 @@
 
 namespace hx {
 
-__device__ __forceinline__ void block_max_to(double mx, double* sm, unsigned tid, unsigned nth,
-                                             unsigned long long* dst, bool direct = false)
-{
-  for (int off = 32; off > 0; off >>= 1) {
-    const double o = __shfl_down(mx, off, 64);
-    mx = o > mx ? o : mx;
-  }
-  __syncthreads();
-  if ((tid & 63u) == 0)
-    sm[tid >> 6] = mx;
-  __syncthreads();
-  if (tid == 0) {
-    const unsigned nw = (nth + 63) >> 6;
-    for (unsigned w = 1; w < nw; w++)
-      mx = sm[w] > mx ? sm[w] : mx;
-    if (direct)
-      *dst = (unsigned long long)__double_as_longlong(mx);
-    else
-      atomicMax(dst, (unsigned long long)__double_as_longlong(mx));
-  }
-}
 
 __global__ void __launch_bounds__(NORM_THREADS)
 embed_norm_kernel(const double* __restrict__ f, const double2* __restrict__ wtab, int logn, int logh,
@@ -70,6 +49,7 @@
   {
     return reinterpret_cast<const double2*>(f + (size_t)row * N)[i];
   }
+  __device__ __forceinline__ double elem(unsigned row, unsigned N, unsigned i) const { return f[(size_t)row * N + i]; }
 };
 struct NormSrcXS {
   const uint64_t* xs;
@@ -80,6 +60,10 @@
     const ulonglong2 x = reinterpret_cast<const ulonglong2*>(xs + (size_t)row * N)[i];
     const longlong2 s = reinterpret_cast<const longlong2*>(S + (size_t)row * N)[i];
     return make_double2((double)x.x * inv_qd - (double)s.x, (double)x.y * inv_qd - (double)s.y);
+  }
+  __device__ __forceinline__ double elem(unsigned row, unsigned N, unsigned i) const
+  {
+    return (double)xs[(size_t)row * N + i] * inv_qd - (double)S[(size_t)row * N + i];
   }
 };
 
@@ -122,35 +106,26 @@
   block_max_to(mx, sm, tid, nth, out2 + row);
 }
 
-__device__ __forceinline__ double lane_xor1(double v)
-{
-  int lo = __double2loint(v), hi = __double2hiint(v);
-  lo = __builtin_amdgcn_mov_dpp(lo, 0xB1, 0xF, 0xF, true);
-  hi = __builtin_amdgcn_mov_dpp(hi, 0xB1, 0xF, 0xF, true);
-  return __hiloint2double(hi, lo);
-}
-template <unsigned (*FROM)(unsigned, unsigned), unsigned (*TO)(unsigned, unsigned)>
-__device__ __forceinline__ void r16_transpose(cplx16 (&v)[16], double* sm, unsigned t)
-{
-#pragma unroll
-  for (unsigned k = 0; k < 16; k++)
-    sm[r16_pad(FROM(t, k))] = v[k].x;
-  __syncthreads();
-#pragma unroll
-  for (unsigned k = 0; k < 16; k++)
-    v[k].x = sm[r16_pad(TO(t, k))];
-  __syncthreads();
-#pragma unroll
-  for (unsigned k = 0; k < 16; k++)
-    sm[r16_pad(FROM(t, k))] = v[k].y;
-  __syncthreads();
-#pragma unroll
-  for (unsigned k = 0; k < 16; k++)
-    v[k].y = sm[r16_pad(TO(t, k))];
-}
 template <class SRC>
 __global__ void __launch_bounds__(R16_THREADS)
 embed_norm_r16_kernel(SRC src, const double2* __restrict__ wtab, unsigned long long* __restrict__ out2, bool direct)
+{
+  extern __shared__ __attribute__((aligned(16))) double sm[];
+  const unsigned row = blockIdx.x, t = threadIdx.x;
+  const tw16* wt = reinterpret_cast<const tw16*>(wtab);
+  cplx16 v[16];
+  const tw16 wth = wt[t];
+#pragma unroll
+  for (unsigned k = 0; k < 16; k++) {
+    const unsigned p = r16_pos_A(t, k);
+    v[k] = r16_direct_twist(src.elem(row, R16_N, p), src.elem(row, R16_N, p + R16_M), wth, wt[r16_direct_tw_k(k)], k);
+  }
+  const double mx = r16_direct_max2(v, sm, t, wt);
+  block_max_to(mx, sm, t, R16_THREADS, out2 + row, direct);
+}
+template <class SRC>
+__global__ void __launch_bounds__(R16_THREADS)
+embed_norm_r16_paired_kernel(SRC src, const double2* __restrict__ wtab, unsigned long long* __restrict__ out2, bool direct)
 {
   extern __shared__ __attribute__((aligned(16))) double sm[];
   const unsigned row = blockIdx.x, t = threadIdx.x;
diff --git a/helib_amd/csrc/norm_r16.h b/helib_amd/csrc/norm_r16.h
--- a/helib_amd/csrc/norm_r16.h
+++ b/helib_amd/csrc/norm_r16.h
@@ -1,5 +1,8 @@
 #pragma once
 #include <stdint.h>
+#if defined(__HIPCC__)
+#include <hip/hip_runtime.h>
+#endif
 
 #ifndef HXD
 #if defined(__HIPCC__)
@@ -22,8 +25,8 @@
 HXD unsigned r16_pad(unsigned i) { return i + (i >> 5); }
 
 HXD tw16 r16_cmul(tw16 a, tw16 b) { return tw16{a.x * b.x - a.y * b.y, a.x * b.y + a.y * b.x}; }
-template <int LOGS, int LOGTAB = 14>
-HXD void r16_pass(cplx16 (&v)[16], unsigned j0, const tw16* wtab)
+template <int LOGS, int LOGTAB = 14, class TAB = const tw16*>
+HXD void r16_pass(cplx16 (&v)[16], unsigned j0, TAB wtab)
 {
   constexpr unsigned S = 1u << LOGS;
   tw16 B = wtab[j0 * ((1u << LOGTAB) / (S * 8u))];
@@ -77,6 +80,14 @@
 HXD unsigned r16_pair_tw_thread(unsigned t) { return 8192u * (t & 1u) + 2u * r16_brev8(t >> 1) + 1u; }
 HXD unsigned r16_pair_tw_k(unsigned k) { return 512u * r16_brev4(k); }
 
+HXD unsigned r16_direct_tw_k(unsigned k) { return 512u * k; }
+HXD cplx16 r16_direct_twist(double lo, double hi, tw16 wth, tw16 wk, unsigned k)
+{
+  const tw16 w = k == 0 ? wth : r16_cmul(wth, wk);
+  return cplx16{lo * w.x - hi * w.y, lo * w.y + hi * w.x};
+}
+HXD double r16_abs2(cplx16 z) { return z.x * z.x + z.y * z.y; }
+
 HXD cplx16 r16_split_input(const double* f, const tw16* wtab, unsigned i, unsigned sub)
 {
   constexpr unsigned N = 1u << 15, H = 8192u, mmask = 2u * N - 1u;
@@ -105,4 +116,76 @@
   return h ? r16_pair_norm2(other, own, w) : r16_pair_norm2(own, other, w);
 }
 
+#if defined(__HIPCC__)
+__device__ __forceinline__ void block_max_to(double mx, double* sm, unsigned tid, unsigned nth,
+                                             unsigned long long* dst, bool direct = false)
+{
+  for (int off = 32; off > 0; off >>= 1) {
+    const double o = __shfl_down(mx, off, 64);
+    mx = o > mx ? o : mx;
+  }
+  __syncthreads();
+  if ((tid & 63u) == 0)
+    sm[tid >> 6] = mx;
+  __syncthreads();
+  if (tid == 0) {
+    const unsigned nw = (nth + 63) >> 6;
+    for (unsigned w = 1; w < nw; w++)
+      mx = sm[w] > mx ? sm[w] : mx;
+    if (direct)
+      *dst = (unsigned long long)__double_as_longlong(mx);
+    else
+      atomicMax(dst, (unsigned long long)__double_as_longlong(mx));
+  }
 }
+__device__ __forceinline__ double lane_xor1(double v)
+{
+  int lo = __double2loint(v), hi = __double2hiint(v);
+  lo = __builtin_amdgcn_mov_dpp(lo, 0xB1, 0xF, 0xF, true);
+  hi = __builtin_amdgcn_mov_dpp(hi, 0xB1, 0xF, 0xF, true);
+  return __hiloint2double(hi, lo);
+}
+template <unsigned (*FROM)(unsigned, unsigned), unsigned (*TO)(unsigned, unsigned)>
+__device__ __forceinline__ void r16_transpose(cplx16 (&v)[16], double* sm, unsigned t)
+{
+#pragma unroll
+  for (unsigned k = 0; k < 16; k++)
+    sm[r16_pad(FROM(t, k))] = v[k].x;
+  __syncthreads();
+#pragma unroll
+  for (unsigned k = 0; k < 16; k++)
+    v[k].x = sm[r16_pad(TO(t, k))];
+  __syncthreads();
+#pragma unroll
+  for (unsigned k = 0; k < 16; k++)
+    sm[r16_pad(FROM(t, k))] = v[k].y;
+  __syncthreads();
+#pragma unroll
+  for (unsigned k = 0; k < 16; k++)
+    v[k].y = sm[r16_pad(TO(t, k))];
+}
+struct R16ConstTab {
+  const double __attribute__((address_space(4)))* p;
+  __device__ explicit R16ConstTab(const double* q) : p((const double __attribute__((address_space(4)))*)(uintptr_t)q) {}
+  __device__ __forceinline__ tw16 operator[](unsigned i) const { return tw16{p[2u * i], p[2u * i + 1u]}; }
+};
+template <class TAB>
+__device__ __forceinline__ double r16_direct_max2(cplx16 (&v)[16], double* sm, unsigned t, TAB wt)
+{
+  r16_pass<9>(v, t, wt);
+  r16_transpose<r16_pos_A, r16_pos_B>(v, sm, t);
+  r16_pass<5>(v, t & 31u, wt);
+  __syncthreads();
+  r16_transpose<r16_pos_B, r16_pos_C>(v, sm, t);
+  r16_pass<1>(v, t & 1u, wt);
+  double mx = 0;
+#pragma unroll
+  for (unsigned k = 0; k < 16; k++) {
+    const double n2 = r16_abs2(r16_last_lane(v[k], cplx16{lane_xor1(v[k].x), lane_xor1(v[k].y)}, t));
+    mx = n2 > mx ? n2 : mx;
+  }
+  return mx;
+}
+#endif
+
+}
diff --git a/helib_amd/csrc/ntt_core.h b/helib_amd/csrc/ntt_core.h
--- a/helib_amd/csrc/ntt_core.h
+++ b/helib_amd/csrc/ntt_core.h
@@ -735,6 +735,11 @@
 template <class IO>
 struct io_skip_load<IO, std::void_t<decltype(IO::SKIP_LOAD)>> : std::integral_constant<bool, IO::SKIP_LOAD> {};
 
+template <class IO, class = void>
+struct io_inv_store_all : std::false_type {};
+template <class IO>
+struct io_inv_store_all<IO, std::void_t<decltype(IO::INV_STORE_ALL)>> : std::integral_constant<bool, IO::INV_STORE_ALL> {};
+
 template <class IO, class AR, class = void>
 struct io_load_bound : std::integral_constant<int, IO::LOAD_BOUND> {};
 template <class IO, class AR>
@@ -950,10 +955,14 @@
             HX_SCHED_FENCE();
         });
       }
-#pragma unroll
-      for (int e = 0; e < 32; e++) {
-        io.store(tid, coef_const<LOGN>(e), norm_from<AR::INV_OUT>(v[e], c));
-        HX_IO_FENCE(e);
+      if constexpr (io_inv_store_all<IO>::value) {
+        io.template inv_store_all<LOGN, AR>(tid, v, lds, c);
+      } else {
+#pragma unroll
+        for (int e = 0; e < 32; e++) {
+          io.store(tid, coef_const<LOGN>(e), norm_from<AR::INV_OUT>(v[e], c));
+          HX_IO_FENCE(e);
+        }
       }
     }
   }
diff --git a/helib_amd/csrc/ntt_kernels.hip b/helib_amd/csrc/ntt_kernels.hip
--- a/helib_amd/csrc/ntt_kernels.hip
+++ b/helib_amd/csrc/ntt_kernels.hip
@@ -3,6 +3,7 @@
 #include "prof.h"
 
 #include "ntt_kernel_util.h"
+#include "norm_r16.h"
 
 #ifdef HX_NTT_ONLY
 #define HX_SFX2(n, s) n##_L##s
@@ -141,18 +142,22 @@
   }
 };
 
+enum class Known { No, Yes, RunTime };
+template <Known CORR = Known::RunTime, Known NARROW = Known::RunTime>
 __device__ __forceinline__ int64_t moddown_S_of(const ModDownPrep& P, uint64_t x)
 {
   const bool neg = x > P.half;
   int64_t S = neg ? 1 : 0;
-  if (P.ptxt > 1) {
+  const bool corr = CORR == Known::RunTime ? P.ptxt > 1 : CORR == Known::Yes;
+  if (corr) {
     const uint64_t p = P.ptxt;
     uint64_t r = red64(x, p, P.ptxt_mu64);
     if (neg)
       r = sub_mod(r, P.qd_mod_p, p);
-    if (r != 0) {
-      const uint64_t dm = (p >> 32) == 0 ? red64(r * P.qdinv_mod_p, p, P.ptxt_mu64)
-                                         : mul_mod(r, P.qdinv_mod_p, p, P.ptxt_mu, P.ptxt_k);
+    if (NARROW != Known::RunTime || r != 0) {
+      const bool narrow = NARROW == Known::RunTime ? (p >> 32) == 0 : NARROW == Known::Yes;
+      const uint64_t dm = narrow ? red64(r * P.qdinv_mod_p, p, P.ptxt_mu64)
+                                 : mul_mod(r, P.qdinv_mod_p, p, P.ptxt_mu, P.ptxt_k);
       const uint64_t p2 = p >> 1;
       const bool sub_p = dm > p2 || (((p & 1) == 0) && dm == p2 && neg);
       S += sub_p ? (int64_t)dm - (int64_t)p : (int64_t)dm;
@@ -169,11 +174,77 @@
   for (size_t i = (size_t)blockIdx.x * blockDim.x + threadIdx.x; i < n2; i += (size_t)gridDim.x * blockDim.x) {
     const ulonglong2 x = xs[i];
     longlong2 s;
-    s.x = moddown_S_of(P, x.x);
-    s.y = moddown_S_of(P, x.y);
+    s.x = moddown_S_of<>(P, x.x);
+    s.y = moddown_S_of<>(P, x.y);
     S[i] = s;
   }
 }
+
+template <class BASE, int FUSE>
+struct PrepFuseIO : BASE {
+  static constexpr bool INV_STORE_ALL = true;
+  const ModDownPrep& P;
+  v4i32 rS;
+  template <class... A>
+  __device__ PrepFuseIO(const ModDownPrep& p, size_t soff, unsigned bytes, A&&... base)
+      : BASE(base...), P(p), rS(make_rsrc(reinterpret_cast<const uint64_t*>(p.S) + soff, bytes))
+  {
+  }
+  template <int LOGN, class AR, Known CORR, Known NARROW>
+  __device__ __forceinline__ void store_xs(unsigned tid, uint64_t (&v)[32], const QC& c) const
+  {
+#pragma unroll
+    for (int e = 0; e < 32; e++) {
+      const uint64_t x = norm_from<AR::INV_OUT>(v[e], c);
+      BASE::store(tid, coef_const<LOGN>(e), x);
+      const int64_t S = moddown_S_of<CORR, NARROW>(P, x);
+      v2i32 sw;
+      sw.x = (int)(uint32_t)(uint64_t)S;
+      sw.y = (int)(uint32_t)((uint64_t)S >> 32);
+      hx_buffer_store_v2(sw, rS, (int)(tid * 8u), (int)(coef_const<LOGN>(e) * 8u), 0);
+      if constexpr (FUSE == 2) {
+        double d = (double)x * P.inv_qd - (double)S;
+        asm volatile("" : "+v"(d));
+        v[e] = (uint64_t)__double_as_longlong(d);
+        HX_SCHED_FENCE();
+      } else {
+        HX_IO_FENCE(e);
+      }
+    }
+  }
+  template <int LOGN, class AR>
+  __device__ __forceinline__ void inv_store_all(unsigned tid, uint64_t (&v)[32], uint32_t* lds, const QC& c) const
+  {
+    if constexpr (FUSE == 2)
+      store_xs<LOGN, AR, Known::RunTime, Known::Yes>(tid, v, c);
+    else if (P.ptxt <= 1)
+      store_xs<LOGN, AR, Known::No, Known::Yes>(tid, v, c);
+    else if ((P.ptxt >> 32) == 0)
+      store_xs<LOGN, AR, Known::Yes, Known::Yes>(tid, v, c);
+    else
+      store_xs<LOGN, AR, Known::Yes, Known::No>(tid, v, c);
+    if constexpr (FUSE == 2) {
+      static_assert(LOGN == (int)R16_LOGN && Geo<LOGN>::T == (int)R16_THREADS &&
+                        (size_t)Geo<LOGN>::LDS_WORDS * 4 == (size_t)R16_LDS_DOUBLES * 8,
+                    "the norm tail takes over the row transform's workgroup and array as they are");
+      __syncthreads();
+      const unsigned t = fresh_tid((unsigned)__builtin_amdgcn_readfirstlane((int)(tid >> 6)));
+      double* sm = reinterpret_cast<double*>(lds);
+      const R16ConstTab wt(P.wtab);
+      const tw16 wth = wt[t];
+      cplx16 z[16];
+#pragma unroll
+      for (unsigned k = 0; k < 16; k++) {
+        z[k] = r16_direct_twist(__longlong_as_double((long long)v[k]), __longlong_as_double((long long)v[k + 16]), wth,
+                                wt[r16_direct_tw_k(k)], k);
+        if (k % 4 == 3)
+          HX_SCHED_FENCE();
+      }
+      const double mx = r16_direct_max2(z, sm, t, wt);
+      block_max_to(mx, sm, t, R16_THREADS, P.norm_out + blockIdx.x, true);
+    }
+  }
+};
 
 template <bool PLAIN>
 struct ModDownIO {
@@ -358,7 +429,7 @@
   ntt_body_ar<LOGN, INV, ArShoup>(lds, io, tw_ptr, q);
 }
 
-template <int LOGN>
+template <int LOGN, int FUSE = 0>
 __global__ void __launch_bounds__(Geo<LOGN>::T, HX_NTT_MINWAVES(LOGN))
 ntt_moddown_prep_kernel(PolyBases polys, int row, int prime, int batch, ModDownPrep P,
                         const PrimeDev* __restrict__ primes, const TW* __restrict__ tw_arena)
@@ -369,9 +440,15 @@
   const size_t N = Geo<LOGN>::N;
   const uint64_t* in = poly_base(polys, (unsigned)pi);
   const size_t pstride = P.poly_stride ? (size_t)P.poly_stride : (size_t)batch * N;
-  const InvPrepIO io(in + ((size_t)row * batch + b) * N, P, (size_t)pi * pstride + (size_t)b * N,
-                     (unsigned)N * 8u);
-  ntt_body<LOGN, true>(lds, io, tw_arena + pd->tw_inv_off, pd);
+  const size_t boff = (size_t)pi * pstride + (size_t)b * N;
+  if constexpr (FUSE == 0) {
+    const InvPrepIO io(in + ((size_t)row * batch + b) * N, P, boff, (unsigned)N * 8u);
+    ntt_body<LOGN, true>(lds, io, tw_arena + pd->tw_inv_off, pd);
+  } else {
+    const PrepFuseIO<InvPrepIO, FUSE> io(P, boff, (unsigned)N * 8u, in + ((size_t)row * batch + b) * N, P, boff,
+                                         (unsigned)N * 8u);
+    ntt_body<LOGN, true>(lds, io, tw_arena + pd->tw_inv_off, pd);
+  }
 }
 template <int LOGN>
 __global__ void __launch_bounds__(Geo<LOGN>::T, HX_NTT_MINWAVES(LOGN))
@@ -485,7 +562,7 @@
   __device__ __forceinline__ TW last_tw(TW def, int which) const { return has_up ? (which ? upN : upS) : def; }
   __device__ __forceinline__ TWM last_tw(TWM def, int which) const { return has_up ? (which ? upN.wp : upS.wp) : def; }
 };
-template <int LOGN>
+template <int LOGN, int FUSE = 0>
 __global__ void __launch_bounds__(Geo<LOGN>::T, HX_NTT_MINWAVES(LOGN))
 ntt_moddown_prep_tensor_kernel(TensorSrc T, int row, int prime, int batch, ModDownPrep P,
                                const PrimeDev* __restrict__ primes, const TW* __restrict__ tw_arena)
@@ -494,9 +571,15 @@
   const int b = (int)(blockIdx.x % (unsigned)batch), pi = (int)(blockIdx.x / (unsigned)batch);
   const PrimeDev* pd = primes + prime;
   const size_t N = Geo<LOGN>::N;
-  const InvPrepTensorIO io(T, (unsigned)pi, ((size_t)row * batch + b) * N, P, ((size_t)pi * batch + b) * N,
-                           (unsigned)N * 8u, pd);
-  ntt_body<LOGN, true>(lds, io, tw_arena + pd->tw_inv_off, pd);
+  const size_t roff = ((size_t)row * batch + b) * N, xoff = ((size_t)pi * batch + b) * N;
+  if constexpr (FUSE == 0) {
+    const InvPrepTensorIO io(T, (unsigned)pi, roff, P, xoff, (unsigned)N * 8u, pd);
+    ntt_body<LOGN, true>(lds, io, tw_arena + pd->tw_inv_off, pd);
+  } else {
+    const PrepFuseIO<InvPrepTensorIO, FUSE> io(P, xoff, (unsigned)N * 8u, T, (unsigned)pi, roff, P, xoff, (unsigned)N * 8u,
+                                               pd);
+    ntt_body<LOGN, true>(lds, io, tw_arena + pd->tw_inv_off, pd);
+  }
 }
 
 template <int LOGN>
@@ -1090,6 +1173,11 @@
   constexpr size_t lds_bytes = (size_t)Geo<LOGN>::LDS_WORDS * 4;
   hipError_t e = hxp::dyn_lds((const void*)ntt_moddown_prep_kernel<LOGN>, (int)lds_bytes);
   if (e == hipSuccess)
+    e = hxp::dyn_lds((const void*)ntt_moddown_prep_kernel<LOGN, 1>, (int)lds_bytes);
+  if constexpr (LOGN == 14)
+    if (e == hipSuccess)
+      e = hxp::dyn_lds((const void*)ntt_moddown_prep_kernel<LOGN, 2>, (int)lds_bytes);
+  if (e == hipSuccess)
     e = hxp::dyn_lds((const void*)ntt_moddown_prep_multi_kernel<LOGN>, (int)lds_bytes);
   if (e == hipSuccess)
     e = hxp::dyn_lds((const void*)ntt_moddown_apply_kernel<LOGN, false>, (int)lds_bytes);
@@ -1116,10 +1204,19 @@
   hipError_t e = moddown_attrs<LOGN>();
   if (e != hipSuccess)
     return e;
-  HX_LAUNCH((ntt_moddown_prep_kernel<LOGN>), dim3((unsigned)polys.n * (unsigned)batch),
-                     dim3(Geo<LOGN>::T), lds_bytes, st, polys, drop_row, drop_prime, batch, P, primes,
-                     tw_arena);
-  {
+  const dim3 pgrid((unsigned)polys.n * (unsigned)batch), pblock(Geo<LOGN>::T);
+  if (P.fuse == 2) {
+    if constexpr (LOGN == 14)
+      HX_LAUNCH((ntt_moddown_prep_kernel<LOGN, 2>), pgrid, pblock, lds_bytes, st, polys, drop_row, drop_prime, batch, P,
+                primes, tw_arena);
+    else
+      return hipErrorInvalidValue;
+  } else if (P.fuse == 1) {
+    HX_LAUNCH((ntt_moddown_prep_kernel<LOGN, 1>), pgrid, pblock, lds_bytes, st, polys, drop_row, drop_prime, batch, P,
+              primes, tw_arena);
+  } else {
+    HX_LAUNCH((ntt_moddown_prep_kernel<LOGN>), pgrid, pblock, lds_bytes, st, polys, drop_row, drop_prime, batch, P, primes,
+              tw_arena);
     const size_t n = (size_t)polys.n * (size_t)batch * Geo<LOGN>::N;
     HX_LAUNCH((moddown_S_kernel<0>), dim3((unsigned)((n / 2 + 255) / 256 > 8192 ? 8192 : (n / 2 + 255) / 256)),
                        dim3(256), 0, st, P, n / 2);
@@ -1148,6 +1245,11 @@
 {
   constexpr size_t lds_bytes = (size_t)Geo<LOGN>::LDS_WORDS * 4;
   hipError_t e = hxp::dyn_lds((const void*)ntt_moddown_prep_tensor_kernel<LOGN>, (int)lds_bytes);
+  if (e == hipSuccess)
+    e = hxp::dyn_lds((const void*)ntt_moddown_prep_tensor_kernel<LOGN, 1>, (int)lds_bytes);
+  if constexpr (LOGN == 14)
+    if (e == hipSuccess)
+      e = hxp::dyn_lds((const void*)ntt_moddown_prep_tensor_kernel<LOGN, 2>, (int)lds_bytes);
   if (e == hipSuccess)
     e = hxp::dyn_lds((const void*)ntt_moddown_prep_multi_tensor_kernel<LOGN>, (int)lds_bytes);
   if (e == hipSuccess)
@@ -1165,9 +1267,19 @@
   hipError_t ea = moddown_tensor_attrs<LOGN>();
   if (ea != hipSuccess)
     return ea;
-  HX_LAUNCH((ntt_moddown_prep_tensor_kernel<LOGN>), dim3(3u * (unsigned)batch), dim3(Geo<LOGN>::T), lds_bytes, st, T,
-            drop_row, drop_prime, batch, P, primes, tw_arena);
-  {
+  const dim3 pgrid(3u * (unsigned)batch), pblock(Geo<LOGN>::T);
+  if (P.fuse == 2) {
+    if constexpr (LOGN == 14)
+      HX_LAUNCH((ntt_moddown_prep_tensor_kernel<LOGN, 2>), pgrid, pblock, lds_bytes, st, T, drop_row, drop_prime, batch, P,
+                primes, tw_arena);
+    else
+      return hipErrorInvalidValue;
+  } else if (P.fuse == 1) {
+    HX_LAUNCH((ntt_moddown_prep_tensor_kernel<LOGN, 1>), pgrid, pblock, lds_bytes, st, T, drop_row, drop_prime, batch, P,
+              primes, tw_arena);
+  } else {
+    HX_LAUNCH((ntt_moddown_prep_tensor_kernel<LOGN>), pgrid, pblock, lds_bytes, st, T, drop_row, drop_prime, batch, P, primes,
+              tw_arena);
     const size_t n = (size_t)3 * (size_t)batch * Geo<LOGN>::N;
     HX_LAUNCH((moddown_S_kernel<0>), dim3((unsigned)((n / 2 + 255) / 256 > 8192 ? 8192 : (n / 2 + 255) / 256)), dim3(256), 0, st, P,
               n / 2);
diff --git a/helib_amd/csrc/switches.h b/helib_amd/csrc/switches.h
--- a/helib_amd/csrc/switches.h
+++ b/helib_amd/csrc/switches.h
@@ -20,6 +20,7 @@
   bool no_tensor_multi = false;
   bool no_mulrelin_fuse = false;
   bool no_ks_last_fuse = false;
+  bool no_prep_fuse = false;
   bool half15 = false;
   bool no_proth = false;
   bool blue_old = false;
@@ -59,6 +60,7 @@
   s.no_tensor_multi = on("HX_NO_TENSOR_MULTI");
   s.no_mulrelin_fuse = on("HX_NO_MULRELIN_FUSE");
   s.no_ks_last_fuse = on("HX_NO_KS_LAST_FUSE");
+  s.no_prep_fuse = on("HX_NO_PREP_FUSE");
   s.no_proth = on("HX_NO_PROTH");
   s.blue_old = on("HX_BLUE_OLD");
   s.no_pfa = on("HX_NO_PFA") || s.blue_old;
```

Result: faster. 45250 mult/s (median of 6 runs) (+1.5%).
